# facebook/transform360

Measured on NVIDIA H100. Metric: Mpixels/s 8K equirect->cubemap bicubic (input-plane pixels consumed per second), higher is better.
Workload: dtype u8

## Files before the change

### include/transform360_b200.h

```cpp
#ifndef TRANSFORM360_B200_EXT_H
#define TRANSFORM360_B200_EXT_H

#include "Transform360/VideoFrameTransformHandler.h"

#ifdef __cplusplus
extern "C" {
#endif

typedef struct T360HostPlan T360HostPlan;

T360HostPlan* T360B200_hostPlanCreate(const FrameTransformContext* ctx, int inputWidth, int inputHeight,
                                      int outputWidth, int outputHeight);
void T360B200_hostPlanDestroy(T360HostPlan* plan);
int T360B200_hostPlanInfo(const T360HostPlan* plan, int info[6]);
const float* T360B200_hostPlanMap(const T360HostPlan* plan);
const int32_t* T360B200_hostPlanSamples(const T360HostPlan* plan);
int T360B200_hostPlanGather(T360HostPlan* plan, int info[10], const int32_t** jobs, const int32_t** records,
                            const uint32_t** compact);
int T360B200_dealLanes(int interpolationAlg, int n, const int32_t* phases, int32_t* laneOf, int32_t* copyOf);
int T360B200_weightImage(int interpolationAlg, const uint8_t** image);
int T360B200_hostPlanSegment(const T360HostPlan* plan, int i, int rect[4], int numTaps[2], const float** kx,
                             const float** ky);
int T360B200_remapTable(int interpolationAlg, const int16_t** table);

int T360B200_transformFramePlaneAsync(VideoFrameTransform* transform, const uint8_t* deviceInput,
                                      uint8_t* deviceOutput, int inputWidth, int inputHeight, int inputPitch,
                                      int outputWidth, int outputHeight, int outputPitch,
                                      int transformMatPlaneIndex, void* cudaStream);
int T360B200_transformFrameAsync(VideoFrameTransform* transform, int numPlanes, const uint8_t* const* deviceInputs,
                                 uint8_t* const* deviceOutputs, const int* inputWidths, const int* inputHeights,
                                 const int* inputPitches, const int* outputWidths, const int* outputHeights,
                                 const int* outputPitches, void* cudaStream);
int T360B200_lowPassPlaneAsync(VideoFrameTransform* transform, const uint8_t* deviceInput, uint8_t* deviceOutput,
                               int width, int height, int inputPitch, int outputPitch,
                               int transformMatPlaneIndex, void* cudaStream);
void T360B200_setPinHostPlanes(VideoFrameTransform* transform, int enable);
void T360B200_debugTrace(VideoFrameTransform* transform, int enable);
unsigned long long T360B200_debugTraceRead(VideoFrameTransform* transform, unsigned long long* out, unsigned long long maxWords);
int T360B200_synchronize(VideoFrameTransform* transform);
void* T360B200_stream(VideoFrameTransform* transform);

unsigned long long T360B200_kernelLaunchCount(void);
unsigned long long T360B200_planDeviceBytes(VideoFrameTransform* transform, int transformMatPlaneIndex);
int T360B200_planTileCounts(VideoFrameTransform* transform, int transformMatPlaneIndex, int counts[4]);
int T360B200_deviceCount(void);
const char* T360B200_version(void);

#ifdef __cplusplus
}
#endif
#endif
```

### profiles/trace_frame.py

```python
#!/usr/bin/env python
import sys
from pathlib import Path

import numpy as np
import torch

sys.path.insert(0, str(Path(__file__).resolve().parents[1]))
import transform360_b200 as t360
from bench import CONFIGS
from transform360_b200 import synth
from transform360_b200.stream import FrameTransformer, StreamSpec

KINDS = {0: "class0", 1: "class1", 2: "general", 3: "share-stay", 4: "share", 5: "nop", 7: "seam"}


def main():
    name = sys.argv[1] if len(sys.argv) > 1 else "cfg2"
    cfg = CONFIGS[name]
    dev = torch.device("cuda", 0)
    torch.cuda.set_device(0)
    ctx = t360.make_context(**dict(cfg["ov"], enable_low_pass_filter=0))
    spec = StreamSpec(cfg["inp"][0], cfg["inp"][1], cfg["out"][0], cfg["out"][1])
    ft = FrameTransformer(ctx, spec)
    pitch = lambda w: (w + 255) // 256 * 256
    ring = 5
    d_in = [[synth.noise_plane_torch(*spec.plane_dims(p)[:2], plane=p, frame=f, device=dev, pitch=pitch(spec.plane_dims(p)[0])) for p in range(3)]
            for f in range(ring)]
    d_out = [torch.zeros((spec.plane_dims(p)[3], pitch(spec.plane_dims(p)[2])), dtype=torch.uint8, device=dev) for p in range(3)]
    calls = [ft.frame_call([(t.data_ptr(), t.stride(0)) for t in fr], [(t.data_ptr(), t.stride(0)) for t in d_out]) for fr in d_in]
    stream = torch.cuda.Stream(device=dev)
    torch.cuda.synchronize()
    for i in range(6):
        calls[i % ring](stream.cuda_stream)
    torch.cuda.synchronize()
    ft.vft.debug_trace(True)
    calls[1](stream.cuda_stream)
    torch.cuda.synchronize()
    tr = ft.vft.read_trace().astype(np.int64)
    ft.vft.debug_trace(False)
    if len(sys.argv) > 2:
        np.save(sys.argv[2], tr)
    used = tr[..., 2] > 0
    t_start = tr[..., 0][used].min()
    end = np.where(used, tr[..., 2], 0).max(axis=1) - t_start
    begin = np.where(used, tr[..., 0], 1 << 62).min(axis=1) - t_start
    print(f"groups {tr.shape[0]}, jobs traced {int(used.sum())}, frame {end.max() / 1e3:.1f} us; groups finish at "
          f"min {end.min() / 1e3:.1f} / median {np.median(end) / 1e3:.1f} / max {end.max() / 1e3:.1f} us, start at median {np.median(begin) / 1e3:.1f} us")
    wait, comp, kind = (tr[..., 1] - tr[..., 0])[used], (tr[..., 2] - tr[..., 1])[used], tr[..., 3][used]
    print(f"all jobs: waiting {wait.sum() / 1e3:.0f} group-us, computing {comp.sum() / 1e3:.0f} group-us "
          f"({100 * wait.sum() / (wait.sum() + comp.sum()):.0f} % waiting)")
    for k in sorted(set(kind.tolist())):
        m = kind == k
        print(f"  {KINDS.get(k, k):10s} n={int(m.sum()):5d}  wait mean {wait[m].mean():7.0f} ns (p90 {np.percentile(wait[m], 90):6.0f})  "
              f"compute mean {comp[m].mean():7.0f} ns (p10 {np.percentile(comp[m], 10):6.0f} p90 {np.percentile(comp[m], 90):6.0f})")
    first = tr[:, 0, :]
    print(f"first job of a group: wait {np.mean(first[:, 1] - first[:, 0]) / 1e3:.2f} us")


if __name__ == "__main__":
    main()
```

### transform360_b200/csrc/gather_frame.cu

```cuda
#include "gather_common.cuh"

#include <cuda.h>

#include <algorithm>
#include <cstring>
#include <utility>

namespace t360 {

namespace {

template <class F, int... I>
__device__ __forceinline__ void staticForImpl(F&& f, std::integer_sequence<int, I...>) {
  (f(std::integral_constant<int, I>{}), ...);
}
template <int N, class F>
__device__ __forceinline__ void staticFor(F&& f) {
  staticForImpl(f, std::make_integer_sequence<int, N>{});
}

template <int IMM>
__device__ __forceinline__ uint32_t ldsWordImm(uint32_t addr) {
  uint32_t v;
  asm volatile("ld.shared.u32 %0, [%1+%2];" : "=r"(v) : "r"(addr), "n"(IMM));
  return v;
}
template <int IMM>
__device__ __forceinline__ uint4 ldsVecImm(uint32_t addr) {
  uint4 v;
  asm volatile("ld.shared.v4.u32 {%0, %1, %2, %3}, [%4+%5];" : "=r"(v.x), "=r"(v.y), "=r"(v.z), "=r"(v.w) : "r"(addr), "n"(IMM));
  return v;
}
template <int IMM>
__device__ __forceinline__ uint2 ldsVec2Imm(uint32_t addr) {
  uint2 v;
  asm volatile("ld.shared.v2.u32 {%0, %1}, [%2+%3];" : "=r"(v.x), "=r"(v.y) : "r"(addr), "n"(IMM));
  return v;
}

__device__ __forceinline__ uint32_t smemAddr(const void* p) { return (uint32_t)__cvta_generic_to_shared(p); }

__device__ __forceinline__ void mbarInit(uint64_t* bar, uint32_t arrivals) {
  asm volatile("mbarrier.init.shared::cta.b64 [%0], %1;" ::"r"(smemAddr(bar)), "r"(arrivals));
}
__device__ __forceinline__ void mbarExpectTx(uint64_t* bar, uint32_t bytes) {
  asm volatile("mbarrier.arrive.expect_tx.shared::cta.b64 _, [%0], %1;" ::"r"(smemAddr(bar)), "r"(bytes) : "memory");
}
__device__ __forceinline__ void mbarWait(uint64_t* bar, uint32_t parity) {
  asm volatile(
      "{\n\t.reg .pred p;\n\t"
      "WAIT_%=:\n\t"
      "mbarrier.try_wait.parity.shared::cta.b64 p, [%0], %1;\n\t"
      "@p bra DONE_%=;\n\t"
      "bra WAIT_%=;\n\t"
      "DONE_%=:\n\t}"
      ::"r"(smemAddr(bar)), "r"(parity) : "memory");
}
__device__ __forceinline__ void tmaLoadBox(void* dst, const CUtensorMap* map, int x, int y, uint64_t* bar) {
  asm volatile(
      "cp.async.bulk.tensor.2d.shared::cluster.global.mbarrier::complete_tx::bytes [%0], [%1, {%2, %3}], [%4];"
      ::"r"(smemAddr(dst)), "l"(reinterpret_cast<uint64_t>(map)), "r"(x), "r"(y), "r"(smemAddr(bar)) : "memory");
}
__device__ __forceinline__ void bulkCopyToShared(void* dst, const void* src, uint32_t bytes, uint64_t* bar) {
  asm volatile("cp.async.bulk.shared::cluster.global.mbarrier::complete_tx::bytes [%0], [%1], %2, [%3];"
               ::"r"(smemAddr(dst)), "l"(src), "r"(bytes), "r"(smemAddr(bar)) : "memory");
}
__device__ __forceinline__ void groupBarrier(int group) {
  asm volatile("bar.sync %0, %1;" ::"r"(group + 1), "n"(kGroupThreads) : "memory");
}

template <int K>
struct RowBytes {
  uint32_t b[K == 8 ? 2 : 1];
};

template <int K, int IMM>
__device__ __forceinline__ RowBytes<K> loadRow(uint32_t addr, int sh) {
  RowBytes<K> o;
  const uint32_t q0 = ldsWordImm<IMM>(addr), q1 = ldsWordImm<IMM + 4>(addr);
  o.b[0] = __funnelshift_r(q0, q1, sh);
  if constexpr (K == 8) o.b[1] = __funnelshift_r(q1, ldsWordImm<IMM + 8>(addr), sh);
  return o;
}

template <int K, int VS>
__device__ __forceinline__ int foldRows(const RowBytes<K> (&W)[K], uint32_t slotAddr) {
  int acc = 1 << 14;
  if constexpr (K == 2) {
    const uint2 w = ldsVec2Imm<0>(slotAddr);
    acc = dp2aLo(w.x, W[0].b[0], acc);
    acc = dp2aLo(w.y, W[1].b[0], acc);
  } else if constexpr (K == 4) {
    const uint4 wa = ldsVecImm<0>(slotAddr), wb = ldsVecImm<VS>(slotAddr);
    acc = dp2aLo(wa.x, W[0].b[0], acc); acc = dp2aHi(wa.y, W[0].b[0], acc);
    acc = dp2aLo(wa.z, W[1].b[0], acc); acc = dp2aHi(wa.w, W[1].b[0], acc);
    acc = dp2aLo(wb.x, W[2].b[0], acc); acc = dp2aHi(wb.y, W[2].b[0], acc);
    acc = dp2aLo(wb.z, W[3].b[0], acc); acc = dp2aHi(wb.w, W[3].b[0], acc);
  } else {
    staticFor<8>([&](auto R) {
      constexpr int r = decltype(R)::value;
      const uint4 wt = ldsVecImm<r * VS>(slotAddr);
      acc = dp2aLo(wt.x, W[r].b[0], acc); acc = dp2aHi(wt.y, W[r].b[0], acc);
      acc = dp2aLo(wt.z, W[r].b[1], acc); acc = dp2aHi(wt.w, W[r].b[1], acc);
    });
  }
  return acc;
}
template <int K>
__device__ __forceinline__ uint32_t slotOffset(uint32_t field) { return K == 2 ? field >> 1 : field; }

template <int VS>
__device__ __forceinline__ int foldRowsRotated(const RowBytes<8> (&W)[8], uint32_t wAddr, uint32_t field) {
  static_assert(VS == 16384, "one copy of the table");
  const uint32_t r = ((field >> 4) ^ threadIdx.x) & 7u;
  const uint32_t first = field ^ (r * (uint32_t)kDiagonalStep);
  const bool p0 = (r & 1u) != 0, p1 = (r & 2u) != 0, p2 = (r & 4u) != 0;
  RowBytes<8> A[8], B[8];
#pragma unroll
  for (int i = 0; i < 8; ++i)
#pragma unroll
    for (int h = 0; h < 2; ++h) A[i].b[h] = p0 ? W[i ^ 1].b[h] : W[i].b[h];
#pragma unroll
  for (int i = 0; i < 8; ++i)
#pragma unroll
    for (int h = 0; h < 2; ++h) B[i].b[h] = p1 ? A[i ^ 2].b[h] : A[i].b[h];
  int acc = 1 << 14;
  staticFor<8>([&](auto V) {
    constexpr int v = decltype(V)::value;
    const uint4 wt = ldsVecImm<0>(wAddr + (first ^ (uint32_t)(v * kDiagonalStep)));
    const uint32_t b0 = p2 ? B[v ^ 4].b[0] : B[v].b[0], b1 = p2 ? B[v ^ 4].b[1] : B[v].b[1];
    acc = dp2aLo(wt.x, b0, acc); acc = dp2aHi(wt.y, b0, acc);
    acc = dp2aLo(wt.z, b1, acc); acc = dp2aHi(wt.w, b1, acc);
  });
  return acc;
}
template <int K, int VS>
__device__ __forceinline__ int foldPixel(const RowBytes<K> (&W)[K], uint32_t wAddr, uint32_t field) {
  if constexpr (K == 8) return foldRowsRotated<VS>(W, wAddr, field);
  else return foldRows<K, VS>(W, wAddr + slotOffset<K>(field));
}
__device__ __forceinline__ int biasedToByte(int acc) { return min(max(acc >> 15, 0), 255); }


__device__ __forceinline__ uint32_t packBytes(int hi, int lo) {
  uint32_t r;
  asm("cvt.pack.sat.u8.s32.b32 %0, %1, %2, %3;" : "=r"(r) : "r"(hi), "r"(lo), "r"(0));
  return r;
}

template <int K, int PITCH, int VS, int ROWS, bool ZERO>
__device__ __forceinline__ void computeShareJob(uint8_t* dst, int dstPitch, uint32_t stageAddr, const uint4 (&rec)[ROWS / 8],
                                                uint32_t header, uint32_t wAddr) {
  static_assert(PITCH % 4 == 0 && (K == 4 || K == 8) && ROWS % 8 == 0, "");
  uint32_t base = stageAddr + (header & 0x7ffcu);
  const int sh = (int)(header << 3);
  RowBytes<K> W[K];
  staticFor<K>([&](auto R) { W[decltype(R)::value] = loadRow<K, decltype(R)::value * PITCH>(base, sh); });
  int accPrev = 0;
  staticFor<ROWS>([&](auto J) {
    constexpr int j = decltype(J)::value;
    const uint4& block = rec[j >> 3];
    const uint32_t word = ((j >> 1) & 3) == 0 ? block.x : (((j >> 1) & 3) == 1 ? block.y : (((j >> 1) & 3) == 2 ? block.z : block.w));
    const uint32_t r = (j & 1) ? word >> 16 : word;
    if constexpr (j > 0 && !ZERO) {
      const bool two = (r & 1u) != 0;
      const RowBytes<K> below = loadRow<K, (j - 1 + K) * PITCH>(base, sh);
      RowBytes<K> below2 = below;
      if (two) below2 = loadRow<K, (j + K) * PITCH>(base, sh);
#pragma unroll
      for (int q = 0; q + 2 < K; ++q)
#pragma unroll
        for (int i = 0; i < (K == 8 ? 2 : 1); ++i) W[q].b[i] = two ? W[q + 2].b[i] : W[q + 1].b[i];
#pragma unroll
      for (int i = 0; i < (K == 8 ? 2 : 1); ++i) W[K - 2].b[i] = two ? below.b[i] : W[K - 1].b[i];
      W[K - 1] = below2;
      if (two) base += PITCH;
    }
    if constexpr (j > 0 && ZERO) {
      const uint32_t d = r & 3u;
      RowBytes<K> below = W[K - 1], below2 = W[K - 1];
      if (d != 0) below = loadRow<K, K * PITCH>(base, sh);
      if (d == 2) below2 = loadRow<K, (K + 1) * PITCH>(base, sh);
#pragma unroll
      for (int q = 0; q + 2 < K; ++q)
#pragma unroll
        for (int i = 0; i < (K == 8 ? 2 : 1); ++i) W[q].b[i] = d == 0 ? W[q].b[i] : (d == 1 ? W[q + 1].b[i] : W[q + 2].b[i]);
#pragma unroll
      for (int i = 0; i < (K == 8 ? 2 : 1); ++i) {
        W[K - 2].b[i] = d == 0 ? W[K - 2].b[i] : (d == 1 ? W[K - 1].b[i] : below.b[i]);
        W[K - 1].b[i] = d == 0 ? W[K - 1].b[i] : (d == 1 ? below.b[i] : below2.b[i]);
      }
      base += d * PITCH;
    }
    const int acc = foldPixel<K, VS>(W, wAddr, r & kSlotFieldMask) >> 15;
    if constexpr (j & 1) {
      const uint32_t pair = packBytes(acc, accPrev);
      dst[(size_t)(j - 1) * dstPitch] = (uint8_t)pair;
      dst[(size_t)j * dstPitch] = (uint8_t)(pair >> 8);
    } else {
      accPrev = acc;
    }
  });
}

template <int K, int PITCH, int VS>
__device__ __forceinline__ void computeTileJob(const PlaneView& pv, uint32_t stageAddr, int outX, int outY, const uint4& rec,
                                               uint32_t wAddr, int warp) {
  static_assert(PITCH % 4 == 0, "");
  const int y0 = outY + warp * kTilePatchH;
  const int dstPitch = pv.dstPitch, dstW = pv.dstW, dstH = pv.dstH;
  uint8_t* const dstRow = pv.dst + (size_t)y0 * dstPitch + outX;
  const uint32_t words[4] = {rec.x, rec.y, rec.z, rec.w};
  staticFor<kRowsPerPatchStep>([&](auto J) {
    constexpr int j = decltype(J)::value;
    const uint32_t w = words[j];
    const int col = kTilePatchW * j + ((int)(w >> 16) & (kTilePatchW - 1)), row = (int)(w >> 19) & (kTilePatchH - 1);
    if (!(w & kRecordSkip) && outX + col < dstW && y0 + row < dstH) {
      const uint32_t rowAddr = stageAddr + (w & 0x7ffcu);
      const int sh = (int)(w << 3);
      RowBytes<K> W[K];
      staticFor<K>([&](auto R) { W[decltype(R)::value] = loadRow<K, decltype(R)::value * PITCH>(rowAddr, sh); });
      const int acc = foldPixel<K, VS>(W, wAddr, (w >> 17) & kSlotFieldMask);
      dstRow[(size_t)row * dstPitch + col] = (uint8_t)biasedToByte(acc);
    }
  });
}

template <int K, int VS>
__device__ __forceinline__ void computeGeneralJob(const PlaneView& pv, int outX, int outY, const unsigned char* wsmem, uint32_t wAddr,
                                                  int lane, int warp) {
  SrcView sv;
  sv.bytes = pv.src;
  sv.misalign = (int)(reinterpret_cast<uintptr_t>(pv.src) & 3);
  sv.words = reinterpret_cast<const uint32_t*>(pv.src - sv.misalign);
  sv.w = pv.srcW; sv.h = pv.srcH; sv.pitch = pv.srcPitch;
  const int y0 = outY + warp * kRowsPerThread;
  if (outX + lane >= pv.dstW) return;
  const int2* segment = pv.samples + ((size_t)(y0 / gatherTileH(K)) * pv.tilesPerRow + outX / kGatherTileW) * gatherTileH(K) * kGatherTileW +
                        (y0 % gatherTileH(K)) * kGatherTileW + lane;
  int2 full[kRowsPerThread];
#pragma unroll
  for (int j = 0; j < kRowsPerThread; ++j) full[j] = y0 + j < pv.dstH ? loadPlan(segment + j * kGatherTileW) : make_int2(0, 0);
  constexpr int kBatch = K == 8 ? 2 : 4;
#pragma unroll
  for (int jb = 0; jb < kRowsPerThread; jb += kBatch) {
    RowBytes<K> W[kBatch][K];
    bool interior[kBatch];
#pragma unroll
    for (int b = 0; b < kBatch; ++b) {
      const int col0 = recordCol0(full[jb + b].x), row0 = full[jb + b].y >> 10;
      interior[b] = y0 + jb + b < pv.dstH && col0 >= 0 && row0 >= 0 && col0 + (K == 2 ? 8 : K + 4) <= sv.w && row0 + K <= sv.h;
#pragma unroll
      for (int r = 0; r < K; ++r) {
        W[b][r].b[0] = 0;
        if constexpr (K == 8) W[b][r].b[1] = 0;
        if (interior[b]) {
          const int off = (row0 + r) * sv.pitch + col0 + sv.misalign;
          const uint32_t* q = sv.words + (off >> 2);
          const int sh = (off & 3) * 8;
          const uint32_t q0 = __ldg(q), q1 = __ldg(q + 1);
          W[b][r].b[0] = __funnelshift_r(q0, q1, sh);
          if constexpr (K == 8) W[b][r].b[1] = __funnelshift_r(q1, __ldg(q + 2), sh);
        }
      }
    }
#pragma unroll
    for (int b = 0; b < kBatch; ++b) {
      const int j = jb + b;
      if (y0 + j >= pv.dstH) continue;
      int v;
      if (interior[b]) v = biasedToByte(foldPixel<K, VS>(W[b], wAddr, (uint32_t)weightSlotOf(K, full[j].y & 1023) << 4));
      else v = gatherPixel<K, false, VS, weightDiagonal(K)>(sv, wsmem, recordCol0(full[j].x), full[j].y);
      pv.dst[(size_t)(y0 + j) * pv.dstPitch + outX + recordColumn(full[j].x)] = (uint8_t)v;
    }
  }
}

struct FrameTensorMaps {
  CUtensorMap map[kMaxFramePlanes][kNumBoxClasses][kBoxVariants];
};

__device__ __forceinline__ void mbarArrive(uint64_t* bar) {
  asm volatile("mbarrier.arrive.shared::cta.b64 _, [%0];" ::"r"(smemAddr(bar)) : "memory");
}
__device__ __forceinline__ uint4 ldsVec(uint32_t addr) {
  uint4 v;
  asm volatile("ld.shared.v4.u32 {%0, %1, %2, %3}, [%4];" : "=r"(v.x), "=r"(v.y), "=r"(v.z), "=r"(v.w) : "r"(addr));
  return v;
}
__device__ __forceinline__ uint32_t ldsWord(uint32_t addr) {
  uint32_t v;
  asm volatile("ld.shared.u32 %0, [%1];" : "=r"(v) : "r"(addr));
  return v;
}

template <int K, int COPIES, int GROUPS>
struct FrameLayout {
  static constexpr int kStages = gatherStages(K);
  static constexpr int kWeights = weightImageBytes(K, COPIES);
  static constexpr int kStage = stageBytesOf(K), kRec = stageRecordBytes(K);
  static constexpr int kGroupBytes = kStages * (kStage + kRec);
  static constexpr int kPlanes = kWeights + GROUPS * kGroupBytes;
  static constexpr int kBars = kPlanes + 256;
  static constexpr int kTotal = kBars + GROUPS * kStages * 16 + 16;
  static_assert(kTotal <= 232448, "227 KB of shared memory per CTA");
  static_assert(sizeof(PlaneView) * kMaxFramePlanes <= 256, "");
  static_assert(kStage % 128 == 0 && kRec % 128 == 0 && kWeights % 128 == 0, "TMA / bulk-copy destinations");
};

template <int K, int COPIES, int GROUPS>
__global__ void __launch_bounds__(GROUPS * (kGroupWarps + 1) * 32, 1)
gatherFrameKernel(const __grid_constant__ FrameGatherParams p, StagedParams jobs, const __grid_constant__ FrameTensorMaps maps) {
  using L = FrameLayout<K, COPIES, GROUPS>;
  constexpr int VS = weightVectorStride(K, COPIES), kStage = L::kStage, kRec = L::kRec, S = L::kStages;
  constexpr uint32_t kBox0 = stageBoxW(K, 0) * stageBoxH(K, 0), kBox1 = stageBoxW(K, 1) * stageBoxH(K, 1),
                     kBoxShare = stageBoxW(K, 2) * stageBoxH(K, 2);
  static_assert(kBox1 + 64 <= 2 * kStage && kBox0 + 64 <= kStage && kBoxShare + 64 <= kStage, "boxes must fit their stage buffers");
  static_assert(boxVariantRows(K, 0, kBoxVariants - 1) > 0 && boxVariantRows(K, 2, kBoxVariants - 1) > 0, "");
  extern __shared__ __align__(128) unsigned char smem[];
  unsigned char* wsmem = smem;
  PlaneView* planes = reinterpret_cast<PlaneView*>(smem + L::kPlanes);
  uint64_t* barBase = reinterpret_cast<uint64_t*>(smem + L::kBars);
  uint64_t* weightBar = barBase + GROUPS * 2 * S;
  const int warpId = threadIdx.x >> 5, lane = threadIdx.x & 31;
  constexpr int kProducerWarp = GROUPS * kGroupWarps;

  asm volatile("griddepcontrol.launch_dependents;" ::: "memory");
  if (threadIdx.x == 0) {
    for (int g = 0; g < GROUPS; ++g)
      for (int st = 0; st < S; ++st) {
        mbarInit(barBase + g * 2 * S + st, 1);
        mbarInit(barBase + g * 2 * S + S + st, kGroupWarps);
      }
    mbarInit(weightBar, 1);
    asm volatile("fence.mbarrier_init.release.cluster;" ::: "memory");
  }
  if (threadIdx.x < kMaxFramePlanes * (int)(sizeof(PlaneView) / 4))
    reinterpret_cast<uint32_t*>(planes)[threadIdx.x] = reinterpret_cast<const uint32_t*>(p.plane)[threadIdx.x];
  __syncthreads();

  if (warpId >= kProducerWarp) {
    const int g = warpId - kProducerWarp;
    if (g == 0 && lane == 0) {
      mbarExpectTx(weightBar, L::kWeights);
      constexpr int kChunk = L::kWeights / 4;
      for (int i = 0; i < 4; ++i)
        bulkCopyToShared(wsmem + i * kChunk, reinterpret_cast<const unsigned char*>(p.weightImage) + i * kChunk, kChunk, weightBar);
    }
    const int producer = blockIdx.x * GROUPS + g, dynamicBase = gridDim.x * GROUPS * 2 * kClaimBatch;
    auto loadBatch = [&](int base) {
      int4 h = make_int4(0, kJobExit << kJobKindShift, 0, 0);
      if (lane < kClaimBatch && base + lane < jobs.numTiles) h = __ldg(reinterpret_cast<const int4*>(jobs.tiles) + base + lane);
      return h;
    };
    int4 batch = loadBatch(producer * 2 * kClaimBatch);
    int4 batchNext = loadBatch((producer * 2 + 1) * kClaimBatch);
    asm volatile("griddepcontrol.wait;" ::: "memory");
    int claimed = 0;
    if (lane == 0) claimed = atomicAdd(jobs.claimCounter, kClaimBatch);
    unsigned char* groupBase = smem + L::kWeights + g * L::kGroupBytes;
    uint64_t* full = barBase + g * 2 * S;
    uint64_t* empty = full + S;
    int pos = 0;
    uint32_t st = 0, phase = 0;
    auto advance = [&]() { if (++st == S) { st = 0; phase ^= 1; } };
    auto postEmptyJob = [&](int kind) {
      *reinterpret_cast<int4*>(groupBase + S * kStage + st * kRec) = make_int4(0, kind << kJobKindShift, 0, 0);
      mbarArrive(full + st);
    };
    for (;;) {
      if (pos == kClaimBatch) {
        batch = batchNext;
        pos = 0;
        batchNext = loadBatch(dynamicBase + __shfl_sync(0xffffffffu, claimed, 0));
        if (lane == 0) claimed = atomicAdd(jobs.claimCounter, kClaimBatch);
      }
      int4 h;
      h.x = __shfl_sync(0xffffffffu, batch.x, pos); h.y = __shfl_sync(0xffffffffu, batch.y, pos);
      h.z = __shfl_sync(0xffffffffu, batch.z, pos); h.w = __shfl_sync(0xffffffffu, batch.w, pos);
      ++pos;
      const int kind = (h.y >> kJobKindShift) & kJobKindMask;
      mbarWait(empty + st, phase ^ 1);
      const bool twoStages = kind == kJobClass1 || kind == kJobSeam;
      if (twoStages) {
        if (st == S - 1) {
          if (lane == 0) postEmptyJob(kJobNop);
          advance();
          mbarWait(empty + st, phase ^ 1);
        }
        mbarWait(empty + st + 1, phase ^ 1);
      }
      if (lane == 0) {
        unsigned char* rec = groupBase + S * kStage + st * kRec;
        *reinterpret_cast<int4*>(rec) = h;
        if (kind == kJobShare || kind == kJobShareStay || kind == kJobClass0 || kind == kJobClass1 || kind == kJobSeam) {
          const int pl = h.y >> kJobPlaneShift;
          const bool share = boxClassOf(kind) == 2;
          const int cls = boxClassOf(kind), variant = jobBoxVariant(h.z), boxX = jobBoxX(h.z), boxY = jobBoxY(h.z);
          const uint32_t boxBytes = (uint32_t)(stageBoxW(K, cls) * boxVariantRows(K, cls, variant));
          const uint32_t recBytes = share ? shareJobRecordBytes(K) : tileJobRecordBytes(h.x);
          mbarExpectTx(full + st, (kind == kJobSeam ? 2 : 1) * boxBytes + recBytes);
          tmaLoadBox(groupBase + st * kStage, &maps.map[pl][cls][variant], boxX, boxY, full + st);
          if (kind == kJobSeam)
            tmaLoadBox(groupBase + (st + 1) * kStage, &maps.map[pl][0][variant], boxX - planes[pl].srcW, boxY, full + st);
          bulkCopyToShared(rec + 128, planes[pl].records + (unsigned)h.w, recBytes, full + st);
        } else {
          mbarArrive(full + st);
        }
      }
      advance();
      if (twoStages) {
        if (lane == 0) postEmptyJob(kJobNop);
        advance();
      }
      __syncwarp();
      if (kind == kJobExit) break;
    }
    if (lane == 0 && atomicAdd(jobs.claimCounter + 1, 1) == (int)(gridDim.x * GROUPS) - 1) {
      jobs.claimCounter[0] = 0;
      jobs.claimCounter[1] = 0;
      __threadfence();
    }
    return;
  }

  const int group = warpId / kGroupWarps, warp = warpId % kGroupWarps;
  unsigned char* groupBase = smem + L::kWeights + group * L::kGroupBytes;
  const uint32_t boxAddr = smemAddr(groupBase), recAddr = smemAddr(groupBase + S * kStage);
  uint64_t* full = barBase + group * 2 * S;
  uint64_t* empty = full + S;
  const uint32_t wAddr = smemAddr(wsmem);
  mbarWait(weightBar, 0);
  asm volatile("griddepcontrol.wait;" ::: "memory");
  auto now = []() { unsigned long long t; asm volatile("mov.u64 %0, %globaltimer;" : "=l"(t)); return t; };
  unsigned long long* trace = jobs.trace && warp == 0 && lane == 0 ? jobs.trace + (size_t)(blockIdx.x * GROUPS + group) * kTraceJobsPerGroup * 4 : nullptr;
  uint32_t traced = 0;
  for (uint32_t st = 0, phase = 0;;) {
    const unsigned long long t0 = trace ? now() : 0;
    mbarWait(full + st, phase);
    const unsigned long long t1 = trace ? now() : 0;
    const uint32_t rec = recAddr + st * kRec;
    const uint4 h = ldsVec(rec);
    const int kind = ((int)h.y >> kJobKindShift) & kJobKindMask;
    if (kind == kJobExit) break;
    const int outX = (int)h.x & ~kJobQuadMask, outY = (int)h.y & kJobRowMask;
    const PlaneView& pv = planes[(int)h.y >> kJobPlaneShift];
    if (kind == kJobShare || kind == kJobShareStay) {
      if constexpr (K >= 4) {
        const uint32_t mine = rec + 128 + warp * shareWarpRecordBytes(K);
        uint4 r[shareRows(K) / 8];
#pragma unroll
        for (int b = 0; b < shareRows(K) / 8; ++b) r[b] = ldsVec(mine + b * 512 + lane * 16);
        const uint32_t header = ldsWord(mine + shareRows(K) / 8 * 512 + lane * 4);
        uint8_t* dst = pv.dst + (size_t)(outY + (warp >> 1) * shareRows(K)) * pv.dstPitch + (outX + (warp & 1) * 32 + (int)(header >> kRecordColumnShift));
        if (kind == kJobShare) computeShareJob<K, stageBoxW(K, 2), VS, shareRows(K), false>(dst, pv.dstPitch, boxAddr + st * kStage, r, header, wAddr);
        else computeShareJob<K, stageBoxW(K, 2), VS, shareRows(K), true>(dst, pv.dstPitch, boxAddr + st * kStage, r, header, wAddr);
      }
    } else if (kind == kJobClass0) {
      uint4 r;
      const int quad = ((int)h.x & kJobQuadMask) - 1;
      if (quad < 0) {
        r = ldsVec(rec + 128 + warp * 512 + lane * 16);
      } else {
        r = make_uint4(kRecordSkip, kRecordSkip, kRecordSkip, kRecordSkip);
        if ((warp >> 2) == (quad >> 1)) {
          const uint2 v = ldsVec2Imm<0>(rec + 128 + (warp & 3) * 256 + lane * 8);
          if (quad & 1) { r.z = v.x; r.w = v.y; } else { r.x = v.x; r.y = v.y; }
        }
      }
      computeTileJob<K, stageBoxW(K, 0), VS>(pv, boxAddr + st * kStage, outX, outY, r, wAddr, warp);
    } else if (kind == kJobClass1) {
      computeTileJob<K, stageBoxW(K, 1), VS>(pv, boxAddr + st * kStage, outX, outY, ldsVec(rec + 128 + warp * 512 + lane * 16), wAddr, warp);
    } else if (kind == kJobSeam) {
      {
        uint4* a = reinterpret_cast<uint4*>(groupBase + st * kStage);
        const uint4* b = reinterpret_cast<const uint4*>(groupBase + (st + 1) * kStage);
        for (int i = warp * 32 + lane; i < (int)(kBox0 / 16); i += kGroupThreads) {
          uint4 x = a[i];
          const uint4 y = b[i];
          x.x |= y.x; x.y |= y.y; x.z |= y.z; x.w |= y.w;
          a[i] = x;
        }
        asm volatile("fence.proxy.async.shared::cta;" ::: "memory");
      }
      groupBarrier(group);
      computeTileJob<K, stageBoxW(K, 0), VS>(pv, boxAddr + st * kStage, outX, outY, ldsVec(rec + 128 + warp * 512 + lane * 16), wAddr, warp);
    } else if (kind == kJobGeneral) {
      computeGeneralJob<K, VS>(pv, outX, outY, wsmem, wAddr, lane, warp);
    }
    __syncwarp();
    if (lane == 0) mbarArrive(empty + st);
    if (trace && traced < kTraceJobsPerGroup) {
      trace[traced * 4 + 0] = t0; trace[traced * 4 + 1] = t1; trace[traced * 4 + 2] = now(); trace[traced * 4 + 3] = kind;
      ++traced;
    }
    if (++st == S) { st = 0; phase ^= 1; }
  }
}

template <int K, int COPIES, int GROUPS>
cudaError_t prepareFrameK(LaunchCfg& cfg) {
  static DeviceLaunchCfg cfgs;
  constexpr int threads = GROUPS * (kGroupWarps + 1) * 32, smemBytes = FrameLayout<K, COPIES, GROUPS>::kTotal;
  return prepare<gatherFrameKernel<K, COPIES, GROUPS>>(cfgs, threads, smemBytes, cfg);
}

template <int K, int COPIES, int GROUPS>
cudaError_t launchFrameK(const FrameGatherParams& p, const StagedParams& jobs, const FrameTensorMaps& maps, int numSMs,
                         cudaStream_t stream, bool programmatic) {
  constexpr int threads = GROUPS * (kGroupWarps + 1) * 32, smemBytes = FrameLayout<K, COPIES, GROUPS>::kTotal;
  LaunchCfg cfg;
  cudaError_t err = prepareFrameK<K, COPIES, GROUPS>(cfg);
  if (err != cudaSuccess) return err;
  const int grid = std::min(numSMs * cfg.perSM, (jobs.numTiles + GROUPS * 2 * kClaimBatch - 1) / (GROUPS * 2 * kClaimBatch));
  cudaLaunchConfig_t lc{};
  lc.gridDim = dim3(grid);
  lc.blockDim = dim3(threads);
  lc.dynamicSmemBytes = smemBytes;
  lc.stream = stream;
  cudaLaunchAttribute attr{};
  attr.id = cudaLaunchAttributeProgrammaticStreamSerialization;
  attr.val.programmaticStreamSerializationAllowed = 1;
  lc.attrs = &attr;
  lc.numAttrs = programmatic ? 1 : 0;
  err = cudaLaunchKernelEx(&lc, gatherFrameKernel<K, COPIES, GROUPS>, p, jobs, maps);
  gLaunches.fetch_add(1, std::memory_order_relaxed);
  return err;
}

}

cudaError_t prepareGatherFrame(int kernelSize) {
  LaunchCfg cfg;
  switch (kernelSize) {
    case 2: return prepareFrameK<2, weightCopies(2), gatherGroups(2)>(cfg);
    case 4: return prepareFrameK<4, weightCopies(4), gatherGroups(4)>(cfg);
    case 8: return prepareFrameK<8, weightCopies(8), gatherGroups(8)>(cfg);
    default: return cudaErrorInvalidValue;
  }
}

cudaError_t launchGatherFrame(const FrameGatherParams& p, const StagedParams& jobs, const void* tensorMaps, int numSMs,
                              cudaStream_t stream, bool programmatic) {
  if (jobs.numTiles <= 0) return cudaSuccess;
  if (p.numPlanes < 1 || p.numPlanes > kMaxFramePlanes) return cudaErrorInvalidValue;
  FrameTensorMaps maps;
  std::memcpy(&maps, tensorMaps, sizeof(CUtensorMap) * kNumBoxClasses * kBoxVariants * p.numPlanes);
  for (int i = p.numPlanes; i < kMaxFramePlanes; ++i)
    for (int c = 0; c < kNumBoxClasses; ++c)
      for (int v = 0; v < kBoxVariants; ++v) maps.map[i][c][v] = maps.map[0][c][v];
  switch (p.kernelSize) {
    case 2: return launchFrameK<2, weightCopies(2), gatherGroups(2)>(p, jobs, maps, numSMs, stream, programmatic);
    case 4: return launchFrameK<4, weightCopies(4), gatherGroups(4)>(p, jobs, maps, numSMs, stream, programmatic);
    case 8: return launchFrameK<8, weightCopies(8), gatherGroups(8)>(p, jobs, maps, numSMs, stream, programmatic);
    default: return cudaErrorInvalidValue;
  }
}

}
```

### transform360_b200/csrc/gather_plan.cpp

```cpp
#include "gather_plan.h"

#include <algorithm>
#include <climits>
#include <cstdint>
#include <cstring>
#include <thread>

namespace t360 {
namespace {

template <class F>
void parallelRanges(int n, size_t workPerItem, F fn) {
  unsigned nt = std::thread::hardware_concurrency();
  if (nt == 0) nt = 1;
  if (nt > 32) nt = 32;
  if (static_cast<size_t>(n) * workPerItem < (1u << 16)) nt = 1;
  const int chunk = (n + static_cast<int>(nt) - 1) / static_cast<int>(nt);
  std::vector<std::thread> pool;
  for (unsigned t = 1; t < nt; ++t) {
    const int b = static_cast<int>(t) * chunk, e = std::min(n, b + chunk);
    if (b < e) pool.emplace_back(fn, b, e);
  }
  fn(0, std::min(n, chunk));
  for (auto& th : pool) th.join();
}

struct GroupMatcher {
  int n, copies, cap;
  const int* base;
  int groupOf[32], load[8];
  bool visited[8];

  bool place(int i) {
    for (int c = 0; c < copies; ++c) {
      const int g = (base[i] + c) & 7;
      if (visited[g]) continue;
      visited[g] = true;
      if (load[g] < cap) {
        ++load[g];
        groupOf[i] = g;
        return true;
      }
      for (int j = 0; j < n; ++j) {
        if (j == i || groupOf[j] != g) continue;
        groupOf[j] = -1;
        if (place(j)) {
          groupOf[i] = g;
          return true;
        }
        groupOf[j] = g;
      }
    }
    return false;
  }
  bool run() {
    std::fill(groupOf, groupOf + 32, -1);
    std::fill(load, load + 8, 0);
    for (int i = 0; i < n; ++i) {
      std::fill(visited, visited + 8, false);
      if (!place(i)) return false;
    }
    return true;
  }
  void balance() {
    for (bool improved = true; improved;) {
      improved = false;
      for (int src = 0; src < 8 && !improved; ++src) {
        int from[8], via[8], queue[8], head = 0, tail = 0;
        std::fill(from, from + 8, -1);
        from[src] = src;
        queue[tail++] = src;
        while (head < tail && !improved) {
          const int g = queue[head++];
          for (int j = 0; j < n && !improved; ++j) {
            if (groupOf[j] != g) continue;
            for (int c = 0; c < copies; ++c) {
              const int t = (base[j] + c) & 7;
              if (from[t] >= 0) continue;
              from[t] = g;
              via[t] = j;
              queue[tail++] = t;
              if (load[t] + 2 <= load[src]) {
                for (int cur = t; cur != src; cur = from[cur]) groupOf[via[cur]] = cur;
                ++load[t];
                --load[src];
                improved = true;
                break;
              }
            }
          }
        }
      }
    }
  }
};

void buildFullRecords(const HostPlan& h, std::vector<int2>& out, int tilesPerRow, int tileH) {
  const int k = h.kernelSize;
  constexpr int kRows = 4;
  parallelRanges((h.mapH + kRows - 1) / kRows, static_cast<size_t>(h.mapW) * kRows, [&](int blockBegin, int blockEnd) {
  for (int yb = blockBegin * kRows; yb < blockEnd * kRows; yb += kRows) {
    for (int x0 = 0; x0 < h.mapW; x0 += 32) {
      const int n = std::min(32, h.mapW - x0);
      int laneOf[32], copyOf[32], slot[32];
      const SamplePoint* first = &h.samples[static_cast<size_t>(yb) * h.mapW];
      for (int i = 0; i < n; ++i) slot[i] = k >= 2 ? weightSlotOf(k, first[x0 + i].rowPhase & 1023) : 0;
      if (k >= 2) dealLanes(k, 1, n, slot, laneOf, copyOf);
      else for (int i = 0; i < n; ++i) laneOf[i] = i;
      for (int y = yb; y < std::min(h.mapH, yb + kRows); ++y) {
        const SamplePoint* row = &h.samples[static_cast<size_t>(y) * h.mapW];
        const size_t tile = static_cast<size_t>(y / tileH) * tilesPerRow + x0 / 32;
        int2* dst = &out[(tile * tileH + y % tileH) * 32];
        for (int c = 0; c < n; ++c) {
          const SamplePoint& sp = row[x0 + c];
          dst[laneOf[c]] = int2{static_cast<int>((static_cast<unsigned>(sp.col0) & ((1u << kRecordColumnShift) - 1)) |
                                                 (static_cast<unsigned>(c) << kRecordColumnShift)),
                                sp.rowPhase};
        }
      }
    }
  }
  });
}

struct TileClass {
  int kind = -1;
  int boxX = 0, boxY = 0, boxRows = 0;
  bool shareStart = false;
  bool quads = false;
  int quadBoxX[4] = {}, quadBoxY[4] = {}, quadBoxRows[4] = {};
};

struct Extent {
  int minC = INT32_MAX, maxC = INT32_MIN, minR = INT32_MAX, maxR = INT32_MIN;
};
Extent extentOf(const HostPlan& h, int x0, int y0, int x1, int y1) {
  Extent e;
  for (int y = y0; y < y1; ++y) {
    const SamplePoint* row = &h.samples[static_cast<size_t>(y) * h.mapW];
    for (int x = x0; x < x1; ++x) {
      const int c = row[x].col0, r = row[x].rowPhase >> 10;
      e.minC = std::min(e.minC, c); e.maxC = std::max(e.maxC, c);
      e.minR = std::min(e.minR, r); e.maxR = std::max(e.maxR, r);
    }
  }
  return e;
}

bool shareBlock(const HostPlan& h, int x0, int y0, TileClass& out) {
  const int k = h.kernelSize, kShareH = shareH(k);
  if (k < 4 || x0 + kShareW > h.mapW || y0 + kShareH > h.mapH) return false;
  bool stays = false;
  for (int y = y0 + 1; y < y0 + kShareH; ++y) {
    const SamplePoint* a = &h.samples[static_cast<size_t>(y - 1) * h.mapW + x0];
    const SamplePoint* b = a + h.mapW;
    for (int x = 0; x < kShareW; ++x) {
      const int d = (b[x].rowPhase >> 10) - (a[x].rowPhase >> 10);
      if (b[x].col0 != a[x].col0 || d < 0 || d > 2) return false;
      stays = stays || d == 0;
    }
  }
  const Extent e = extentOf(h, x0, y0, x0 + kShareW, y0 + kShareH);
  if (e.minC < 0 || e.minR < 0 || e.maxC + k > h.inW || e.maxR + k > h.inH) return false;
  const int boxX = e.minC & ~15;
  if (e.maxC + k - boxX > stageBoxW(k, 2) || e.maxR + k - e.minR > stageBoxH(k, 2)) return false;
  out.kind = stays ? kJobShareStay : kJobShare;
  out.boxX = boxX;
  out.boxY = e.minR;
  out.boxRows = e.maxR + k - e.minR;
  out.shareStart = true;
  return true;
}

int boxClassFor(const HostPlan& h, int x0, int y0, int x1, int y1, int maxClass, int* boxX, int* boxY, int* boxRows) {
  const int k = h.kernelSize;
  const Extent e = extentOf(h, x0, y0, x1, y1);
  if (e.minC < 0 || e.minR < 0 || e.maxC + k > h.inW || e.maxR + k > h.inH) return -1;
  *boxX = e.minC & ~15;
  *boxY = e.minR;
  *boxRows = e.maxR + k - e.minR;
  for (int cls = 0; cls <= maxClass; ++cls)
    if (e.maxC + k - *boxX <= stageBoxW(k, cls) && e.maxR + k - e.minR <= stageBoxH(k, cls)) return cls;
  return -1;
}

void classifyTile(const HostPlan& h, int x0, int y0, bool seamPossible, TileClass& out) {
  const int k = h.kernelSize;
  const int x1 = std::min(h.mapW, x0 + kGatherTileW), y1 = std::min(h.mapH, y0 + kFrameTileH);
  const int cls = boxClassFor(h, x0, y0, x1, y1, 1, &out.boxX, &out.boxY, &out.boxRows);
  if (cls == 0) {
    out.kind = kJobClass0;
    return;
  }
  if (x1 - x0 == kGatherTileW && y1 - y0 == kFrameTileH) {
    bool all = true;
    for (int q = 0; q < 4 && all; ++q) {
      const int qx = x0 + 16 * (q & 1), qy = y0 + 16 * (q >> 1);
      all = boxClassFor(h, qx, qy, qx + 16, qy + 16, 0, &out.quadBoxX[q], &out.quadBoxY[q], &out.quadBoxRows[q]) == 0;
    }
    if (all) {
      out.kind = kJobClass0;
      out.quads = true;
      return;
    }
  }
  if (cls == 1) {
    out.kind = kJobClass1;
    return;
  }
  const Extent e = extentOf(h, x0, y0, x1, y1);
  if (seamPossible && e.minR >= 0 && e.maxR + k <= h.inH && e.maxR + k - e.minR <= stageBoxH(k, 0)) {
    const int W = h.inW, half = W / 2;
    int lo = INT32_MAX, hi = INT32_MIN;
    for (int y = y0; y < y1; ++y)
      for (int x = x0; x < x1; ++x) {
        int cw = h.samples[static_cast<size_t>(y) * h.mapW + x].col0 % W;
        if (cw < 0) cw += W;
        const int rot = cw + half >= W ? cw + half - W : cw + half;
        lo = std::min(lo, rot); hi = std::max(hi, rot);
      }
    const int first = lo - half < 0 ? lo - half + W : lo - half;
    const int bx = first & ~15;
    if (hi - lo + (first - bx) + k <= stageBoxW(k, 0) && bx + stageBoxW(k, 0) > W) {
      out.kind = kJobSeam;
      out.boxX = bx;
      out.boxY = e.minR;
      out.boxRows = e.maxR + k - e.minR;
      return;
    }
  }
  out.kind = kJobGeneral;
  out.boxX = out.boxY = out.boxRows = 0;
}

inline uint32_t slotField(int k, int phase, int copy) { return static_cast<uint32_t>(weightSlotField(k, phase, copy)); }

void writeShareRecords(const HostPlan& h, const GatherJob& job, uint32_t* out) {
  const int k = h.kernelSize, copies = weightCopies(k), kShareRows = shareRows(k), kShareH = shareH(k);
  const int x0 = job.outX, y0 = job.outY & kJobRowMask, boxX = jobBoxX(job.boxXY), boxY = jobBoxY(job.boxXY);
  const int pitch = stageBoxW(k, 2);
  const bool stay = ((job.outY >> kJobKindShift) & kJobKindMask) == kJobShareStay;
  for (int wx = 0; wx < kShareW / 32; ++wx) {
    for (int wy = 0; wy < kShareH / kShareRows; ++wy) {
      int slot[32], laneOf[32], copyOf[32];
      const SamplePoint* first = &h.samples[static_cast<size_t>(y0 + wy * kShareRows) * h.mapW + x0 + wx * 32];
      for (int i = 0; i < 32; ++i) slot[i] = weightSlotOf(k, first[i].rowPhase & 1023);
      dealLanes(k, copies, 32, slot, laneOf, copyOf);
      const int w = wy * (kShareW / 32) + wx;
      uint32_t* words = out + static_cast<size_t>(w) * (shareWarpRecordBytes(k) / 4);
      uint32_t* headers = words + kShareRows / 8 * 32 * 4;
      for (int c = 0; c < 32; ++c) {
        const int lane = laneOf[c], x = x0 + wx * 32 + c, ya = y0 + wy * kShareRows;
        const SamplePoint* col = &h.samples[static_cast<size_t>(ya) * h.mapW + x];
        const int off = ((col->rowPhase >> 10) - boxY) * pitch + (col->col0 - boxX);
        headers[lane] = static_cast<uint32_t>(off) | (static_cast<uint32_t>(c) << kRecordColumnShift);
        for (int j = 0; j < kShareRows; ++j) {
          const SamplePoint& sp = col[static_cast<size_t>(j) * h.mapW];
          const int first = stay ? 0 : 1;
          const int d = j == 0 ? first : (sp.rowPhase >> 10) - (col[static_cast<size_t>(j - 1) * h.mapW].rowPhase >> 10);
          const uint32_t rec = slotField(k, sp.rowPhase & 1023, copyOf[c]) | static_cast<uint32_t>(d - first);
          uint32_t& word = words[(j >> 3) * 32 * 4 + lane * 4 + ((j >> 1) & 3)];
          word = (j & 1) ? (word | (rec << 16)) : rec;
        }
      }
    }
  }
}

void writeTileRecords(const HostPlan& h, const GatherJob& job, uint32_t* out) {
  const int k = h.kernelSize, copies = weightCopies(k);
  const int kind = (job.outY >> kJobKindShift) & kJobKindMask;
  const int x0 = job.outX & ~kJobQuadMask, y0 = job.outY & kJobRowMask, boxX = jobBoxX(job.boxXY), boxY = jobBoxY(job.boxXY);
  const int pitch = stageBoxW(k, boxClassOf(kind));
  const int quad = (job.outX & kJobQuadMask) - 1;
  const int lx0 = quad < 0 ? x0 : x0 + 16 * (quad & 1), ly0 = quad < 0 ? y0 : y0 + 16 * (quad >> 1);
  const int lx1 = quad < 0 ? x0 + kGatherTileW : lx0 + 16, ly1 = quad < 0 ? y0 + kFrameTileH : ly0 + 16;
  for (int w = 0; w < kGroupWarps; ++w)
    for (int j = 0; j < kRowsPerPatchStep; ++j) {
      if (quad >= 0 && ((w >> 2) != (quad >> 1) || (j >> 1) != (quad & 1))) continue;
      uint32_t* words = quad < 0 ? out + static_cast<size_t>(w) * 32 * 4 : out + static_cast<size_t>(w & 3) * 32 * 2;
      const int stride = quad < 0 ? 4 : 2, word = quad < 0 ? j : (j & 1);
      int slot[32], laneOf[32], copyOf[32], posOf[32], n = 0;
      bool present[32] = {};
      for (int pos = 0; pos < 32; ++pos) {
        const int x = x0 + kTilePatchW * j + (pos & (kTilePatchW - 1)), y = y0 + kTilePatchH * w + pos / kTilePatchW;
        if (x >= h.mapW || y >= h.mapH || x < lx0 || x >= lx1 || y < ly0 || y >= ly1) continue;
        present[pos] = true;
        posOf[n] = pos;
        slot[n++] = weightSlotOf(k, h.samples[static_cast<size_t>(y) * h.mapW + x].rowPhase & 1023);
      }
      dealLanes(k, copies, n, slot, laneOf, copyOf);
      int lane = n;
      for (int pos = 0; pos < 32; ++pos)
        if (!present[pos]) words[(lane++) * stride + word] = (static_cast<uint32_t>(pos) << 16) | kRecordSkip;
      for (int i = 0; i < n; ++i) {
        const int pos = posOf[i];
        const int x = x0 + kTilePatchW * j + (pos & (kTilePatchW - 1)), y = y0 + kTilePatchH * w + pos / kTilePatchW;
        const SamplePoint& sp = h.samples[static_cast<size_t>(y) * h.mapW + x];
        int col0 = sp.col0;
        if (kind == kJobSeam) {
          int cw = col0 % h.inW;
          if (cw < 0) cw += h.inW;
          col0 = boxX + (cw - boxX + h.inW) % h.inW;
        }
        const int off = ((sp.rowPhase >> 10) - boxY) * pitch + (col0 - boxX);
        words[laneOf[i] * stride + word] = static_cast<uint32_t>(off) | (static_cast<uint32_t>(pos) << 16) |
                                           (slotField(k, sp.rowPhase & 1023, copyOf[i]) << 17);
      }
    }
}

}

struct PassDealer {
  int groups, passes, lanes;
  int h[4], share[16][4], fill[4];
  bool seen[4];

  bool put(int g) {
    for (int q = 0; q < passes; ++q) {
      if (seen[q] || share[g][q] >= h[q]) continue;
      seen[q] = true;
      if (fill[q] < lanes) {
        ++share[g][q];
        ++fill[q];
        return true;
      }
      for (int other = 0; other < groups; ++other) {
        if (other == g || share[other][q] == 0) continue;
        --share[other][q];
        if (put(other)) {
          ++share[g][q];
          return true;
        }
        ++share[other][q];
      }
    }
    return false;
  }
  bool deal(const int* load) {
    std::memset(share, 0, sizeof(share));
    std::fill(fill, fill + 4, 0);
    for (int g = 0; g < groups; ++g)
      for (int i = 0; i < load[g]; ++i) {
        std::fill(seen, seen + 4, false);
        if (!put(g)) return false;
      }
    return true;
  }
};

int dealLanes(int k, int copies, int n, const int* slot, int* laneOf, int* copyOf) {
  const int groups = weightBankGroups(k), lanesPerPass = weightLanesPerPass(k), passes = 32 / lanesPerPass;
  for (int i = 0; i < n; ++i) { laneOf[i] = i; copyOf[i] = 0; }
  if (n < 32) return 0;
  int group[32];
  if (copies > 1 && groups == 8) {
    int base[32];
    for (int i = 0; i < n; ++i) base[i] = slot[i] & 7;
    GroupMatcher m{n, copies, 0, base, {}, {}, {}};
    for (m.cap = 4; m.cap <= 32; ++m.cap)
      if (m.run()) break;
    m.balance();
    for (int i = 0; i < n; ++i) {
      group[i] = m.groupOf[i];
      copyOf[i] = (m.groupOf[i] - base[i]) & 7;
    }
  } else {
    for (int i = 0; i < n; ++i) group[i] = slot[i] & (groups - 1);
  }
  int load[16] = {};
  for (int i = 0; i < n; ++i) ++load[group[i]];
  int share[16][4] = {}, height[4] = {};
  {
    int fullest = 0;
    for (int g = 0; g < groups; ++g) fullest = std::max(fullest, load[g]);
    PassDealer d{groups, passes, lanesPerPass, {}, {}, {}, {}};
    bool done = false;
    for (int total = std::max(passes, fullest); !done; ++total) {
      int h[4] = {1, 1, 1, 1};
      auto tryHeights = [&]() {
        std::copy(h, h + 4, d.h);
        if (!d.deal(load)) return false;
        std::memcpy(share, d.share, sizeof(share));
        std::copy(h, h + 4, height);
        return true;
      };
      if (passes == 2) {
        for (h[1] = total / 2; h[1] >= 1 && !done; --h[1]) { h[0] = total - h[1]; done = tryHeights(); }
      } else {
        for (h[3] = total / 4; h[3] >= 1 && !done; --h[3])
          for (h[2] = (total - h[3]) / 3; h[2] >= h[3] && !done; --h[2])
            for (h[1] = (total - h[3] - h[2]) / 2; h[1] >= h[2] && !done; --h[1]) {
              h[0] = total - h[3] - h[2] - h[1];
              done = tryHeights();
            }
      }
    }
  }
  int nextLane[4];
  for (int q = 0; q < passes; ++q) nextLane[q] = q * lanesPerPass;
  for (int g = 0; g < groups; ++g) {
    int q = 0;
    for (int i = 0; i < n; ++i) {
      if (group[i] != g) continue;
      while (share[g][q] == 0) ++q;
      --share[g][q];
      laneOf[i] = nextLane[q]++;
    }
  }
  int wavefronts = 0;
  for (int q = 0; q < passes; ++q) wavefronts += height[q];
  return wavefronts;
}

void spreadGeneralJobs(std::vector<GatherJob>& jobs) {
  std::vector<GatherJob> general, staged;
  for (const GatherJob& j : jobs)
    (((j.outY >> kJobKindShift) & kJobKindMask) == kJobGeneral ? general : staged).push_back(j);
  if (general.empty() || staged.empty()) return;
  const size_t span = staged.size() / 2 + 1;
  jobs.clear();
  size_t g = 0;
  for (size_t i = 0; i < staged.size(); ++i) {
    while (g < general.size() && g * span / general.size() <= i) jobs.push_back(general[g++]);
    jobs.push_back(staged[i]);
  }
  while (g < general.size()) jobs.push_back(general[g++]);
}

std::vector<uint8_t> buildWeightImage(int k, const int16_t* table) {
  const int copies = weightCopies(k);
  std::vector<uint8_t> img(static_cast<size_t>(weightImageBytes(k, copies)), 0);
  for (int phase = 0; phase < 1024; ++phase) {
    const int slot = weightSlotOf(k, phase);
    const int16_t* cell = table + static_cast<size_t>(phase) * k * k;
    if (k == 2) {
      std::memcpy(&img[static_cast<size_t>(slot) * 8], cell, 8);
      continue;
    }
    for (int c = 0; c < copies; ++c)
      for (int v = 0; v < k * k / 8; ++v)
        std::memcpy(&img[static_cast<size_t>(weightVectorOffset(k, copies, (weightSlotInCopy(slot, c) << 4) | (c << 14), v))], cell + v * 8, 16);
  }
  return img;
}

void buildGatherPlan(const HostPlan& h, bool stageTiles, GatherPlan& g) {
  g = GatherPlan{};
  const int k = h.kernelSize;
  if (k <= 0) return;
  g.tileH = gatherTileH(k);
  g.tilesPerRow = (h.mapW + kGatherTileW - 1) / kGatherTileW;
  g.tileRows = (h.mapH + g.tileH - 1) / g.tileH;
  g.records.assign(static_cast<size_t>(g.tilesPerRow) * g.tileRows * g.tileH * kGatherTileW, int2{0, 0});
  buildFullRecords(h, g.records, g.tilesPerRow, g.tileH);
  if (!stageTiles) return;

  const int tilesX = g.tilesPerRow, tilesY = (h.mapH + kFrameTileH - 1) / kFrameTileH;
  const bool seamPossible = h.inW % 16 == 0 && h.inW >= 4 * stageBoxW(k, 0);
  std::vector<TileClass> cls(static_cast<size_t>(tilesX) * tilesY);
  const int blockRows = shareH(k) / kFrameTileH;
  parallelRanges((tilesY + blockRows - 1) / blockRows, static_cast<size_t>(h.mapW) * shareH(k), [&](int byBegin, int byEnd) {
    for (int by = byBegin; by < byEnd; ++by)
      for (int tx = 0; tx < tilesX; tx += 2) {
        TileClass* c = &cls[static_cast<size_t>(by) * blockRows * tilesX + tx];
        if (shareBlock(h, tx * 32, by * shareH(k), c[0])) continue;
        for (int ty = by * blockRows; ty < std::min(tilesY, (by + 1) * blockRows); ++ty)
          for (int t = tx; t < std::min(tilesX, tx + 2); ++t)
            classifyTile(h, t * 32, ty * kFrameTileH, seamPossible, cls[static_cast<size_t>(ty) * tilesX + t]);
      }
  });
  const int order[7] = {kJobGeneral, kJobSeam, kJobClass1, kJobShareStay, kJobShare, kJobClass0, kJobClass0};
  size_t offset = 0;
  for (int step = 0; step < 7; ++step)
    for (int ty = 0; ty < tilesY; ++ty)
      for (int tx = 0; tx < tilesX; ++tx) {
        const int kind = order[step];
        const TileClass& c = cls[static_cast<size_t>(ty) * tilesX + tx];
        if (c.kind != kind || (kind == kJobClass0 && c.quads != (step == 6))) continue;
        for (int q = 0; q < (c.quads ? 4 : 1); ++q) {
          GatherJob job{tx * 32, ty * kFrameTileH | (kind << kJobKindShift),
                        kind == kJobGeneral ? 0 : jobBoxField(c.boxX, c.boxY, boxVariantFor(k, boxClassOf(kind), c.boxRows)), 0};
          if (c.quads) {
            job.outX |= q + 1;
            job.boxXY = jobBoxField(c.quadBoxX[q], c.quadBoxY[q], boxVariantFor(k, 0, c.quadBoxRows[q]));
          }
          if (kind != kJobGeneral) {
            job.recordOffset = static_cast<int>(offset / 16);
            offset += boxClassOf(kind) == 2 ? shareJobRecordBytes(k) : tileJobRecordBytes(job.outX);
          }
          g.jobs.push_back(job);
        }
        switch (kind) {
          case kJobGeneral: ++g.numGeneral; break;
          case kJobSeam: ++g.numSeam; break;
          case kJobShare: case kJobShareStay: ++g.numShare; break;
          default: g.numStaged[kind] += c.quads ? 4 : 1; break;
        }
      }
  g.compact.assign(offset / 4, 0u);
  g.jobNeedRows.assign(g.jobs.size(), h.inH);
  parallelRanges(static_cast<int>(g.jobs.size()), 2048, [&](int begin, int end) {
    for (int i = begin; i < end; ++i) {
      const GatherJob& job = g.jobs[i];
      {
        int rect[4];
        jobOutputRect(job, k, rect);
        const Extent e = extentOf(h, rect[0], rect[1], std::min(rect[2], h.mapW), std::min(rect[3], h.mapH));
        if (e.minR >= 0 && e.maxR + k <= h.inH) g.jobNeedRows[i] = e.maxR + k;
      }
      const int kind = (job.outY >> kJobKindShift) & kJobKindMask;
      if (kind == kJobGeneral) continue;
      uint32_t* out = g.compact.data() + static_cast<size_t>(job.recordOffset) * 4;
      if (boxClassOf(kind) == 2) writeShareRecords(h, job, out);
      else writeTileRecords(h, job, out);
    }
  });
}

}
```

### transform360_b200/csrc/gather_plan.h

```cpp
#pragma once

#include <cstdint>
#include <vector>

#include "host_plan.h"
#include "kernels.cuh"

namespace t360 {

struct GatherPlan {
  int tilesPerRow = 0, tileRows = 0, tileH = 0;
  std::vector<int2> records;
  std::vector<GatherJob> jobs;
  std::vector<uint32_t> compact;
  std::vector<int> jobNeedRows;
  int numStaged[2] = {}, numSeam = 0, numGeneral = 0, numShare = 0;
  int totalStaged() const { return numSeam + numShare + numStaged[0] + numStaged[1]; }
};

void buildGatherPlan(const HostPlan& h, bool stageTiles, GatherPlan& g);

inline void jobOutputRect(const GatherJob& job, int k, int rect[4]) {
  const int kind = (job.outY >> kJobKindShift) & kJobKindMask, quad = (job.outX & kJobQuadMask) - 1;
  rect[0] = job.outX & ~kJobQuadMask;
  rect[1] = job.outY & kJobRowMask;
  if (quad >= 0) { rect[0] += 16 * (quad & 1); rect[1] += 16 * (quad >> 1); }
  const bool share = kind == kJobShare || kind == kJobShareStay;
  rect[2] = rect[0] + (quad >= 0 ? 16 : (share ? kShareW : kGatherTileW));
  rect[3] = rect[1] + (quad >= 0 ? 16 : (share ? shareH(k) : kFrameTileH));
}

void spreadGeneralJobs(std::vector<GatherJob>& jobs);


int dealLanes(int k, int copies, int n, const int* slot, int* laneOf, int* copyOf);

std::vector<uint8_t> buildWeightImage(int k, const int16_t* table);

}
```

### transform360_b200/csrc/kernels.cuh

```cuda
#pragma once

#include <cuda_runtime.h>

#include <cstdint>

namespace t360 {

struct GatherParams {
  const uint8_t* src;
  int srcW, srcH, srcPitch;
  uint8_t* dst;
  int dstW, dstH, dstPitch;
  const int2* samples;
  int tilesPerRow;
  const int16_t* weights;
  int kernelSize;
  int transparent;
};

struct GatherJob {
  int outX, outY;
  int boxXY;
  int recordOffset;
};
constexpr int kBoxVariants = 3;
__host__ __device__ constexpr int jobBoxField(int boxX, int boxY, int variant) { return boxX | (boxY << 16) | variant; }
__host__ __device__ constexpr int jobBoxX(int boxXY) { return boxXY & 0xfff0; }
__host__ __device__ constexpr int jobBoxY(int boxXY) { return (int)((unsigned)boxXY >> 16); }
__host__ __device__ constexpr int jobBoxVariant(int boxXY) { return boxXY & 15; }
using StagedTile = GatherJob;
constexpr int kJobClass0 = 0, kJobClass1 = 1, kJobGeneral = 2, kJobShareStay = 3, kJobShare = 4, kJobNop = 5, kJobExit = 6, kJobSeam = 7;
constexpr int kJobQuadMask = 7;
constexpr uint32_t kRecordSkip = 0x8000u;
constexpr int kJobKindShift = 24, kJobRowMask = (1 << kJobKindShift) - 1;
constexpr int kJobPlaneShift = 28, kJobKindMask = (1 << (kJobPlaneShift - kJobKindShift)) - 1;

constexpr int kGroupThreads = 256, kGroupWarps = kGroupThreads / 32;
__host__ __device__ constexpr int gatherGroups(int k) { return k == 8 ? 2 : 3; }
#ifndef T360_CLAIM_BATCH
#define T360_CLAIM_BATCH 1
#endif
constexpr int kClaimBatch = T360_CLAIM_BATCH;
constexpr int kGatherTileW = 32, kFrameTileH = 32;
constexpr int kTilePatchW = 8, kTilePatchH = 4, kRowsPerPatchStep = 4;
constexpr int kShareW = 64;
__host__ __device__ constexpr int shareRows(int ) { return 8; }
__host__ __device__ constexpr int shareH(int k) { return 4 * shareRows(k); }
constexpr int kNumBoxClasses = 3;
__host__ __device__ constexpr int boxClassOf(int kind) { return (kind == kJobShare || kind == kJobShareStay) ? 2 : (kind == kJobClass1 ? 1 : 0); }
__host__ __device__ constexpr int stageBoxW(int , int cls) { return cls == 2 ? 192 : (cls == 0 ? 208 : 240); }
__host__ __device__ constexpr int stageBoxH(int k, int cls) {
  return k == 8 ? (cls == 2 ? 80 : (cls == 0 ? 72 : 128)) : (cls == 2 ? 72 : (cls == 0 ? 64 : 96));
}
__host__ __device__ constexpr int boxVariantRows(int k, int cls, int v) {
  return cls == 1 || v == 0 ? stageBoxH(k, cls) : (cls == 2 ? stageBoxH(k, cls) - 8 * v : stageBoxH(k, cls) - 8 - 8 * v);
}
__host__ __device__ constexpr int boxVariantFor(int k, int cls, int rows) {
  int v = 0;
  while (v + 1 < kBoxVariants && cls != 1 && boxVariantRows(k, cls, v + 1) >= rows) ++v;
  return v;
}
__host__ __device__ constexpr int gatherStages(int ) { return 2; }
__host__ __device__ constexpr int stageBytesOf(int k) {
  const int a = stageBoxW(k, 2) * stageBoxH(k, 2), b = stageBoxW(k, 0) * stageBoxH(k, 0);
  return ((a > b ? a : b) + 64 + 127) & ~127;
}

__host__ __device__ constexpr int weightSlotOf(int k, int phase) {
  (void)k;
  return (phase & ~31) | ((phase & 1) << 4) | ((phase & 31) >> 1);
}
__host__ __device__ constexpr int weightCopies(int k) { return k == 4 ? 2 : 1; }
__host__ __device__ constexpr int weightVectorStride(int k, int copies) { return (k == 2 ? 8192 : 16384) * copies; }
__host__ __device__ constexpr int weightImageBytes(int k, int copies) { return k == 2 ? 8192 * copies : (k * k / 8) * 16384 * copies; }
__host__ __device__ constexpr int weightSlotInCopy(int slot, int copy) { return copy ? ((slot & ~7) | ((slot + copy) & 7)) : slot; }
__host__ __device__ constexpr int weightSlotField(int k, int phase, int copy) {
  return (weightSlotInCopy(weightSlotOf(k, phase), copy) << 4) | (copy << 14);
}
constexpr int kSlotFieldMask = 0x7FF0;
constexpr int kDiagonalStep = 0x4010;
__host__ __device__ constexpr bool weightDiagonal(int k) { return k == 8; }
__host__ __device__ constexpr int weightVectorOffset(int k, int copies, int slotFieldValue, int vector) {
  return weightDiagonal(k) ? (slotFieldValue ^ (vector * kDiagonalStep)) : slotFieldValue + vector * weightVectorStride(k, copies);
}
__host__ __device__ constexpr int weightBankGroups(int k) { return k == 2 ? 16 : 8; }
__host__ __device__ constexpr int weightLanesPerPass(int k) { return k == 2 ? 16 : 8; }

__host__ __device__ constexpr int shareWarpRecordBytes(int k) { return shareRows(k) / 8 * 32 * 16 + 32 * 4; }
__host__ __device__ constexpr int shareJobRecordBytes(int k) { return kGroupWarps * shareWarpRecordBytes(k); }
constexpr int kTileJobRecordBytes = kGroupWarps * 32 * 16;
constexpr int kQuadJobRecordBytes = kGroupWarps / 2 * 32 * 8;
__host__ __device__ constexpr int tileJobRecordBytes(int outXField) { return (outXField & kJobQuadMask) ? kQuadJobRecordBytes : kTileJobRecordBytes; }
__host__ __device__ constexpr int stageRecordBytes(int k) {
  return 128 + (shareJobRecordBytes(k) > kTileJobRecordBytes ? shareJobRecordBytes(k) : kTileJobRecordBytes);
}
constexpr int kRecordColumnShift = 27;

constexpr int kMaxFramePlanes = 3;
struct PlaneView {
  const uint8_t* src;
  uint8_t* dst;
  const int2* samples;
  const uint4* records;
  int srcW, srcH, srcPitch;
  int dstW, dstH, dstPitch;
  int tilesPerRow;
  int reserved;
};
struct FrameGatherParams {
  PlaneView plane[kMaxFramePlanes];
  const uint4* weightImage;
  int kernelSize, numPlanes;
};

__host__ __device__ constexpr int gatherThreads(int k) { return k == 8 ? 512 : 256; }
__host__ __device__ constexpr int gatherTileH(int k) { return gatherThreads(k) / 32 * 4; }

struct StagedParams {
  const GatherJob* tiles;
  int numTiles;
  int* claimCounter;
  unsigned long long* trace;
};
constexpr int kTraceJobsPerGroup = 64;

struct BlurJob {
  int x0, y0, w, h;
  int kxOffset, kxCount, kyOffset, kyCount;
};

struct BlurParams {
  const uint8_t* src;
  uint8_t* dst;
  int width, height, srcPitch, dstPitch;
  const BlurJob* jobs;
  int numJobs;
  const float* taps;
  int tileSmemBytes;
};

struct StripJob {
  int x0, y0, w, h;
  int kxOffset, kxChunks, kxCount, kyOffset;
  int edge;
};

struct StripParams {
  const uint8_t* src;
  uint8_t* dst;
  int width, height, srcPitch, dstPitch;
  const StripJob* jobs;
  int numJobs;
  const float* taps;
};

struct AreaParams {
  const uint8_t* src;
  uint8_t* dst;
  int srcW, srcH, srcPitch, dstW, dstH, dstPitch;
  int cellW, cellH;
  const int2* xTaps;
  const int* xFirst;
  const int2* yTaps;
  const int* yFirst;
  const int2* xLinear;
  const int2* yLinear;
  int xMax;
};
cudaError_t launchAreaResize(const AreaParams& p, cudaStream_t stream);

struct FrameStripParams {
  struct Plane {
    const uint8_t* src;
    uint8_t* dst;
    int width, height, srcPitch, dstPitch;
  } plane[kMaxFramePlanes];
  const StripJob* jobs;
  int numJobs;
  const float* taps;
};
constexpr int kStripPlaneShift = 8;
cudaError_t launchBlurFrameStrips(const FrameStripParams& p, int hy, cudaStream_t stream);

constexpr int kStripLanePx = 8, kStripW = 32 * kStripLanePx, kStripMaxHy = 3;

constexpr int kBlurTileW = 64, kBlurTileH = 32;
constexpr int kBlurMaxSmem = 96 * 1024;

cudaError_t launchGather(const GatherParams& p, int numSMs, cudaStream_t stream);
cudaError_t launchGatherFrame(const FrameGatherParams& p, const StagedParams& jobs, const void* tensorMaps, int numSMs,
                              cudaStream_t stream, bool programmatic = true);
cudaError_t prepareGatherFrame(int kernelSize);
cudaError_t launchBlurStrips(const StripParams& p, int hy, cudaStream_t stream);
cudaError_t launchBlur(const BlurParams& p, cudaStream_t stream);
cudaError_t launchBlurDirect(const BlurParams& p, cudaStream_t stream);
unsigned long long kernelLaunchCount();
void countKernelLaunches(long long n);

inline int blurTileSmem(int w, int h, int nkx, int nky) {
  const int hx = nkx / 2, hy = nky / 2;
  const int rows = h + 2 * hy;
  const int srcStride = (w + 2 * hx + 3) & ~3;
  return rows * srcStride + rows * w * 4;
}

}
```

### transform360_b200/csrc/video_frame_transform.cpp

```cpp
#include <cuda.h>
#include <cuda_runtime.h>

#include <algorithm>
#include <climits>
#include <cstdio>
#include <cstdlib>
#include <cstring>
#include <map>
#include <memory>
#include <mutex>
#include <new>
#include <stdexcept>
#include <vector>

#include "host_plan.h"
#include "gather_plan.h"
#include "kernels.cuh"
#include "transform360_b200.h"

#define T360_API extern "C" __attribute__((visibility("default")))

namespace {

using t360::BlurJob;
using t360::GatherJob;
using t360::HostPlan;
using t360::StripJob;

struct CudaFail {
  cudaError_t err;
  const char* what;
};

#define CU(call)                                       \
  do {                                                 \
    cudaError_t e__ = (call);                          \
    if (e__ != cudaSuccess) throw CudaFail{e__, #call}; \
  } while (0)

template <typename T>
struct DeviceBuffer {
  T* ptr = nullptr;
  size_t count = 0;
  DeviceBuffer() = default;
  DeviceBuffer(const DeviceBuffer&) = delete;
  DeviceBuffer& operator=(const DeviceBuffer&) = delete;
  DeviceBuffer(DeviceBuffer&& o) noexcept : ptr(o.ptr), count(o.count) { o.ptr = nullptr; o.count = 0; }
  DeviceBuffer& operator=(DeviceBuffer&& o) noexcept {
    if (this != &o) { release(); ptr = o.ptr; count = o.count; o.ptr = nullptr; o.count = 0; }
    return *this;
  }
  ~DeviceBuffer() { release(); }
  void release() {
    if (ptr) cudaFree(ptr);
    ptr = nullptr;
    count = 0;
  }
  void reserve(size_t n) {
    if (n <= count) return;
    release();
    CU(cudaMalloc(reinterpret_cast<void**>(&ptr), n * sizeof(T)));
    count = n;
  }
  size_t bytes() const { return count * sizeof(T); }
};

struct DevicePlan {
  int inW = 0, inH = 0, outW = 0, outH = 0, mapW = 0, mapH = 0;
  int kernelSize = 0;
  bool transparent = false, lowPass = false;
  DeviceBuffer<int2> samples;
  DeviceBuffer<uint32_t> records;
  int tilesPerRow = 0;
  DeviceBuffer<GatherJob> gatherJobs;
  std::vector<GatherJob> hostJobs;
  std::vector<int> jobNeedRows;
  int numJobs = 0, numStaged[2] = {}, numSeam = 0, numShare = 0, numFallback = 0;
  int totalStaged() const { return numSeam + numShare + numStaged[0] + numStaged[1]; }
  struct BlurSet {
    DeviceBuffer<StripJob> stripJobs[t360::kStripMaxHy];
    int numStripJobs[t360::kStripMaxHy] = {};
    DeviceBuffer<BlurJob> tileJobs, directJobs;
    int numTileJobs = 0, numDirectJobs = 0, tileSmem = 0;
    DeviceBuffer<float> taps;
    bool needsClear = false;
    std::vector<StripJob> hostStrips[t360::kStripMaxHy];
    std::vector<float> hostTaps;
  };
  BlurSet blur;
  std::vector<t360::LowPassSegment> segments;
  std::vector<float> planTaps;
  mutable std::map<std::pair<int, int>, BlurSet> otherBlurs;
  struct Resize {
    int cellW = 0, cellH = 0, xMax = 0;
    DeviceBuffer<int2> xTaps, yTaps, xLinear, yLinear;
    DeviceBuffer<int> xFirst, yFirst;
  };
  bool resizeNeeded = false;
  mutable std::map<std::pair<int, int>, Resize> resizes;
  size_t deviceBytes() const {
    return samples.bytes() + records.bytes() + gatherJobs.bytes() + blur.stripJobs[0].bytes() + blur.stripJobs[1].bytes() + blur.stripJobs[2].bytes() +
           blur.tileJobs.bytes() + blur.directJobs.bytes() + blur.taps.bytes();
  }
};

using EncodeTiledFn = CUresult (*)(CUtensorMap*, CUtensorMapDataType, cuuint32_t, void*, const cuuint64_t*, const cuuint64_t*,
                                   const cuuint32_t*, const cuuint32_t*, CUtensorMapInterleave, CUtensorMapSwizzle,
                                   CUtensorMapL2promotion, CUtensorMapFloatOOBfill);

EncodeTiledFn tensorMapEncoder() {
  static EncodeTiledFn fn = [] {
    void* p = nullptr;
    cudaDriverEntryPointQueryResult q{};
    if (cudaGetDriverEntryPoint("cuTensorMapEncodeTiled", &p, cudaEnableDefault, &q) != cudaSuccess || q != cudaDriverEntryPointSuccess) {
      cudaGetLastError();
      p = nullptr;
    }
    return reinterpret_cast<EncodeTiledFn>(p);
  }();
  return fn;
}

bool encodePlaneMap(CUtensorMap* map, const uint8_t* base, int w, int h, int pitch, int k, int cls, int variant) {
  EncodeTiledFn enc = tensorMapEncoder();
  if (!enc) return false;
  if ((reinterpret_cast<uintptr_t>(base) & 15) || (pitch & 15)) return false;
  const cuuint64_t dims[2] = {static_cast<cuuint64_t>(w), static_cast<cuuint64_t>(h)};
  const cuuint64_t strides[1] = {static_cast<cuuint64_t>(pitch)};
  const cuuint32_t box[2] = {static_cast<cuuint32_t>(t360::stageBoxW(k, cls)), static_cast<cuuint32_t>(t360::boxVariantRows(k, cls, variant))};
  const cuuint32_t elem[2] = {1, 1};
  return enc(map, CU_TENSOR_MAP_DATA_TYPE_UINT8, 2, const_cast<uint8_t*>(base), dims, strides, box, elem,
             CU_TENSOR_MAP_INTERLEAVE_NONE, CU_TENSOR_MAP_SWIZZLE_NONE, CU_TENSOR_MAP_L2_PROMOTION_L2_128B,
             CU_TENSOR_MAP_FLOAT_OOB_FILL_NONE) == CUDA_SUCCESS;
}

constexpr int kPlaneLanes = 3;
static_assert(kPlaneLanes == t360::kMaxFramePlanes, "the frame kernel takes one PlaneView per lane");
struct PlaneMaps {
  const uint8_t* base = nullptr;
  int w = 0, h = 0, pitch = 0, k = 0;
  CUtensorMap maps[t360::kNumBoxClasses][t360::kBoxVariants];
};
struct PlaneLane {
  static constexpr int kMapCache = 32;
  PlaneMaps mapCache[kMapCache];
  int mapCacheNext = 0;
  cudaStream_t main = nullptr;
  cudaEvent_t done = nullptr;
  DeviceBuffer<uint8_t> blurred;
  DeviceBuffer<uint8_t> scaled;
  DeviceBuffer<int> claimCounter;
};

struct GatherWork {
  const DevicePlan* plan = nullptr;
  t360::PlaneView view{};
  bool staged = false;
  CUtensorMap maps[t360::kNumBoxClasses][t360::kBoxVariants];
  uint8_t* finalOut = nullptr;
  int finalPitch = 0, finalW = 0, finalH = 0, imagePlane = 0;
  const void* resizeTables = nullptr;
};

struct FrameJobList {
  DeviceBuffer<GatherJob> tiles;
  int numTiles = 0, numPlanes = 0;
  unsigned long long generation = ~0ull;
  DeviceBuffer<int> claimCounter;
};

struct WavePlan {
  struct Rect { int x, y, w, h; };
  int chunks = 0;
  const void* plan = nullptr;
  unsigned long long generation = ~0ull;
  std::vector<int> chunkRowEnd, waveStart;
  DeviceBuffer<GatherJob> jobs;
  std::vector<std::vector<Rect>> rects;
};

struct StreamSlot {
  PlaneLane lanes[kPlaneLanes];
  DeviceBuffer<int> frameClaim;
  cudaEvent_t fork = nullptr;
};

struct FrameBlurList {
  DeviceBuffer<StripJob> jobs[t360::kStripMaxHy];
  int numJobs[t360::kStripMaxHy] = {};
  DeviceBuffer<float> taps;
  int numPlanes = 0;
  unsigned long long generation = ~0ull;
};

constexpr int kPitchAlign = 256;
inline int alignedPitch(int w) { return (w + kPitchAlign - 1) / kPitchAlign * kPitchAlign; }

}

class VideoFrameTransform {
 public:
  explicit VideoFrameTransform(FrameTransformContext* ctx) {
    std::memcpy(&ctx_, ctx, sizeof(ctx_));
    const char* e = std::getenv("T360B200_PIN_HOST_PLANES");
    pinHostPlanes_ = e && *e && *e != '0';
    if (const char* m = std::getenv("T360B200_PIPELINE_MIN_BYTES")) pipelineMinBytes_ = std::atoll(m);
    if (const char* m = std::getenv("T360B200_PIPELINE_CHUNKS")) pipelineChunks_ = std::atoi(m);
    if (const char* m = std::getenv("T360B200_PIPELINE_BLOCKS")) pipelineBlocks_ = std::atoi(m);
    if (const char* m = std::getenv("T360B200_PIPELINE_IN_STREAMS")) pipelineInStreams_ = std::atoi(m);
  }
  void setPinHostPlanes(bool on) { pinHostPlanes_ = on; }

  ~VideoFrameTransform() {
    if (deviceReady_) {
      cudaSetDevice(device_);
      plans_.clear();
      for (auto& w : weights_) w.release();
      for (auto& w : weightImages_) w.release();
      stagingIn_.release(); stagingOut_.release();
      for (HostRange& r : hostRanges_)
        if (r.pinned) cudaHostUnregister(reinterpret_cast<void*>(r.base));
      for (auto& kv : slots_) {
        for (PlaneLane& l : kv.second->lanes) {
          l.blurred.release();
          l.scaled.release();
          l.claimCounter.release();
          if (l.main) cudaStreamDestroy(l.main);
          if (l.done) cudaEventDestroy(l.done);
        }
        kv.second->frameClaim.release();
        if (kv.second->fork) cudaEventDestroy(kv.second->fork);
      }
      frameJobs_.tiles.release();
      for (auto& b : frameBlur_.jobs) b.release();
      frameBlur_.taps.release();
      trace_.release();
      frameJobs_.claimCounter.release();
      for (cudaEvent_t e : chunkIn_) cudaEventDestroy(e);
      for (cudaEvent_t e : waveDone_) cudaEventDestroy(e);
      for (WavePlan& w : wavePlans_) w.jobs.release();
      for (PlaneGraph& g : planeGraphs_) cudaGraphExecDestroy(g.exec);
      for (cudaEvent_t e : {graphFork_, graphJoinIn_, graphJoinOut_}) if (e) cudaEventDestroy(e);
      if (copyIn_) cudaStreamDestroy(copyIn_);
      if (copyIn2_) cudaStreamDestroy(copyIn2_);
      if (copyOut_) cudaStreamDestroy(copyOut_);
      if (stream_) cudaStreamDestroy(stream_);
    }
  }

  bool generateMapForPlane(int inW, int inH, int outW, int outH, int planIndex) {
    try {
      HostPlan host;
      if (!t360::buildHostPlan(ctx_, inW, inH, outW, outH, host)) return false;
      const DeviceRestore restoreDevice = ensureDevice();
      std::lock_guard<std::mutex> lock(mu_);
      plans_[planIndex] = upload(host);
      ++planGeneration_;
      return true;
    } catch (const CudaFail& f) {
      std::printf("Could not generate map for plane %d. Error: CUDA %s (%s) in %s\n", planIndex,
                  cudaGetErrorName(f.err), cudaGetErrorString(f.err), f.what);
    } catch (const std::exception& ex) {
      std::printf("Could not generate map for plane %d. Error: %s\n", planIndex, ex.what());
    }
    return false;
  }

  bool transformFramePlane(uint8_t* in, uint8_t* out, int inW, int inH, int inPitch, int outW, int outH, int outPitch,
                           int planIndex, int imagePlaneIndex) {
    try {
      if (!in || !out || inW <= 0 || inH <= 0 || outW <= 0 || outH <= 0 || inPitch < inW || outPitch < outW) {
        std::printf("Could not transform the plane %d. Error: invalid plane description\n", imagePlaneIndex);
        return false;
      }
      const DeviceRestore restoreDevice = ensureDevice();
      const DevicePlan* plan = findPlan(planIndex, imagePlaneIndex);
      if (!plan) return false;
      {
        std::lock_guard<std::mutex> hostLock(hostCallMu_);
        if (replayPlaneGraph(*plan, in, out, inW, inH, inPitch, outW, outH, outPitch)) return true;
      }
      const bool inOnDevice = isDevicePointer(in), outOnDevice = isDevicePointer(out);
      if (plan->kernelSize == 0) {
        std::printf("Could not find interpolation algorithm for plane %d", imagePlaneIndex);
        return true;
      }
      std::lock_guard<std::mutex> hostLock(hostCallMu_);
      if (!inOnDevice && !outOnDevice && pipelineEligible(*plan, inW, inH, outW, outH))
        return transformHostPlanePipelined(*plan, in, out, inW, inH, inPitch, outW, outH, outPitch, planIndex, imagePlaneIndex);
      const uint8_t* dIn = in;
      uint8_t* dOut = out;
      int dInPitch = inPitch, dOutPitch = outPitch;
      if (!inOnDevice) {
        pinIfRecurring(in, static_cast<size_t>(inPitch) * (inH - 1) + inW);
        dInPitch = alignedPitch(inW);
        stagingIn_.reserve(static_cast<size_t>(dInPitch) * inH + 64);
        CU(cudaMemcpy2DAsync(stagingIn_.ptr, dInPitch, in, inPitch, inW, inH, cudaMemcpyHostToDevice, stream_));
        dIn = stagingIn_.ptr;
      }
      if (!outOnDevice) {
        pinIfRecurring(out, static_cast<size_t>(outPitch) * (outH - 1) + outW);
        dOutPitch = alignedPitch(outW);
        stagingOut_.reserve(static_cast<size_t>(dOutPitch) * outH + 64);
        dOut = stagingOut_.ptr;
        if (plan->transparent) {
          if (planIndex) CU(cudaMemset2DAsync(dOut, dOutPitch, 128, outW, outH, stream_));
          else CU(cudaMemcpy2DAsync(dOut, dOutPitch, out, outPitch, outW, outH, cudaMemcpyHostToDevice, stream_));
        }
      } else if (plan->transparent && planIndex) {
        CU(cudaMemset2DAsync(dOut, dOutPitch, 128, outW, outH, stream_));
      }
      if (!enqueue(*plan, dIn, dOut, inW, inH, dInPitch, outW, outH, dOutPitch, stream_, imagePlaneIndex, slotFor(stream_).lanes[0])) return false;
      if (!outOnDevice)
        CU(cudaMemcpy2DAsync(out, outPitch, dOut, dOutPitch, outW, outH, cudaMemcpyDeviceToHost, stream_));
      CU(cudaStreamSynchronize(stream_));
      return true;
    } catch (const CudaFail& f) {
      std::printf("Could not transform the plane %d. Error: CUDA %s (%s) in %s\n", imagePlaneIndex,
                  cudaGetErrorName(f.err), cudaGetErrorString(f.err), f.what);
      cudaGetLastError();
    } catch (const std::exception& ex) {
      std::printf("Could not transform the plane %d. Error: %s\n", imagePlaneIndex, ex.what());
    }
    return false;
  }

  bool pipelineEligible(const DevicePlan& plan, int inW, int inH, int outW, int outH) const {
    return plan.totalStaged() > 0 && !plan.transparent && !plan.lowPass && inW == plan.inW && inH == plan.inH &&
           outW == plan.mapW && outH == plan.mapH && static_cast<long long>(inW) * inH >= pipelineMinBytes_ && inH >= 64;
  }

  WavePlan& wavePlanFor(const DevicePlan& plan, int planIndex, int chunks) {
    WavePlan& w = wavePlans_[planIndex ? 1 : 0];
    if (w.plan == &plan && w.chunks == chunks && w.generation == planGeneration_) return w;
    w.chunks = chunks;
    w.plan = &plan;
    w.generation = planGeneration_;
    const int rowsPer = ((plan.inH + chunks - 1) / chunks + 7) & ~7;
    w.chunkRowEnd.assign(chunks, plan.inH);
    for (int c = 0; c < chunks; ++c) w.chunkRowEnd[c] = std::min(plan.inH, (c + 1) * rowsPer);
    auto waveOf = [&](int needRows) {
      int c = 0;
      while (c + 1 < chunks && w.chunkRowEnd[c] < needRows) ++c;
      return c;
    };
    std::vector<std::vector<GatherJob>> byWave(chunks);
    int blocks = 1;
    for (int nb : {4, 3, 2})
      if (plan.mapW % (nb * t360::kShareW) == 0 && nb <= pipelineBlocks_) { blocks = nb; break; }
    const int blockW = plan.mapW / blocks, bands = (plan.mapH + 31) / 32;
    std::vector<int> complete(static_cast<size_t>(bands) * blocks, 0);
    for (size_t i = 0; i < plan.hostJobs.size(); ++i) {
      const int c = waveOf(plan.jobNeedRows[i]);
      byWave[c].push_back(plan.hostJobs[i]);
      int rect[4];
      t360::jobOutputRect(plan.hostJobs[i], plan.kernelSize, rect);
      for (int band = rect[1] / 32; band <= (std::min(rect[3], plan.mapH) - 1) / 32; ++band) {
        int& slot = complete[static_cast<size_t>(band) * blocks + rect[0] / blockW];
        slot = std::max(slot, c);
      }
    }
    std::vector<GatherJob> all;
    w.waveStart.assign(chunks + 1, 0);
    for (int c = 0; c < chunks; ++c) {
      t360::spreadGeneralJobs(byWave[c]);
      w.waveStart[c] = static_cast<int>(all.size());
      all.insert(all.end(), byWave[c].begin(), byWave[c].end());
    }
    w.waveStart[chunks] = static_cast<int>(all.size());
    w.jobs.reserve(all.size());
    CU(cudaMemcpy(w.jobs.ptr, all.data(), all.size() * sizeof(GatherJob), cudaMemcpyHostToDevice));
    w.rects.assign(chunks, {});
    for (int b = 0; b < blocks; ++b)
      for (int band = 0; band < bands;) {
        const int c = complete[static_cast<size_t>(band) * blocks + b];
        int end = band + 1;
        while (end < bands && complete[static_cast<size_t>(end) * blocks + b] == c) ++end;
        w.rects[c].push_back(WavePlan::Rect{b * blockW, band * 32, blockW, std::min(plan.mapH, end * 32) - band * 32});
        band = end;
      }
    return w;
  }

  static bool isPinnedHost(const void* p) {
    cudaPointerAttributes a{};
    if (cudaPointerGetAttributes(&a, p) != cudaSuccess) {
      cudaGetLastError();
      return false;
    }
    return a.type == cudaMemoryTypeHost;
  }

  bool replayPlaneGraph(const DevicePlan& plan, const uint8_t* in, const uint8_t* out, int inW, int inH, int inPitch, int outW, int outH,
                        int outPitch) {
    for (PlaneGraph& c : planeGraphs_) {
      if (c.plan != &plan || c.in != in || c.out != out || c.inPitch != inPitch || c.outPitch != outPitch || c.generation != planGeneration_ ||
          c.stagingIn != stagingIn_.ptr || c.stagingOut != stagingOut_.ptr || c.inW != inW || c.inH != inH || c.outW != outW || c.outH != outH)
        continue;
      c.lastUse = ++graphClock_;
      CU(cudaGraphLaunch(c.exec, stream_));
      t360::countKernelLaunches(c.kernels);
      CU(cudaStreamSynchronize(stream_));
      return true;
    }
    return false;
  }

  bool transformHostPlanePipelined(const DevicePlan& plan, uint8_t* in, uint8_t* out, int inW, int inH, int inPitch, int outW, int outH,
                                   int outPitch, int planIndex, int imagePlaneIndex) {
    const long long bytes = static_cast<long long>(inW) * inH;
    const int chunks = pipelineChunks_ > 1 ? std::min(pipelineChunks_, 32)
                                           : static_cast<int>(std::min<long long>(8, std::max<long long>(2, bytes / (3ll << 20))));
    WavePlan& w = wavePlanFor(plan, planIndex, chunks);
    if (!copyIn_) {
      CU(cudaStreamCreateWithFlags(&copyIn_, cudaStreamNonBlocking));
      CU(cudaStreamCreateWithFlags(&copyIn2_, cudaStreamNonBlocking));
      CU(cudaStreamCreateWithFlags(&copyOut_, cudaStreamNonBlocking));
      for (cudaEvent_t* e : {&graphFork_, &graphJoinIn_, &graphJoinOut_}) CU(cudaEventCreateWithFlags(e, cudaEventDisableTiming));
    }
    while (static_cast<int>(chunkIn_.size()) < chunks) {
      cudaEvent_t a = nullptr, b = nullptr;
      CU(cudaEventCreateWithFlags(&a, cudaEventDisableTiming));
      chunkIn_.push_back(a);
      CU(cudaEventCreateWithFlags(&b, cudaEventDisableTiming));
      waveDone_.push_back(b);
    }
    pinIfRecurring(in, static_cast<size_t>(inPitch) * (inH - 1) + inW);
    pinIfRecurring(out, static_cast<size_t>(outPitch) * (outH - 1) + outW);
    const int dInPitch = alignedPitch(inW), dOutPitch = alignedPitch(outW);
    stagingIn_.reserve(static_cast<size_t>(dInPitch) * inH + 64);
    stagingOut_.reserve(static_cast<size_t>(dOutPitch) * outH + 64);
    PlaneLane& hostLane = slotFor(stream_).lanes[0];
    GatherWork work;
    if (!prepareGather(plan, stagingIn_.ptr, stagingOut_.ptr, inW, inH, dInPitch, outW, outH, dOutPitch, stream_, imagePlaneIndex, hostLane, work))
      return false;
    if (!work.staged) {
      CU(cudaMemcpy2DAsync(stagingIn_.ptr, dInPitch, in, inPitch, inW, inH, cudaMemcpyHostToDevice, stream_));
      gatherPlane(work, hostLane, stream_);
      CU(cudaMemcpy2DAsync(out, outPitch, stagingOut_.ptr, dOutPitch, outW, outH, cudaMemcpyDeviceToHost, stream_));
      CU(cudaStreamSynchronize(stream_));
      return true;
    }
    armScheduler(hostLane.claimCounter, stream_);
    CU(t360::prepareGatherFrame(plan.kernelSize));
    auto issue = [&](bool forkJoin) {
      if (forkJoin) {
        CU(cudaEventRecord(graphFork_, stream_));
        CU(cudaStreamWaitEvent(copyIn_, graphFork_, 0));
        if (pipelineInStreams_ > 1) CU(cudaStreamWaitEvent(copyIn2_, graphFork_, 0));
        CU(cudaStreamWaitEvent(copyOut_, graphFork_, 0));
      }
      t360::FrameGatherParams fp{};
      fp.plane[0] = work.view;
      fp.weightImage = reinterpret_cast<const uint4*>(weightImages_[plan.kernelSize].ptr);
      fp.kernelSize = plan.kernelSize;
      fp.numPlanes = 1;
      for (int c = 0; c < chunks; ++c) {
        const int r0 = c ? w.chunkRowEnd[c - 1] : 0, r1 = w.chunkRowEnd[c];
        cudaStream_t inStream = (pipelineInStreams_ > 1 && (c & 1)) ? copyIn2_ : copyIn_;
        if (r1 > r0)
          CU(cudaMemcpy2DAsync(stagingIn_.ptr + static_cast<size_t>(r0) * dInPitch, dInPitch, in + static_cast<size_t>(r0) * inPitch, inPitch, inW,
                               r1 - r0, cudaMemcpyHostToDevice, inStream));
        CU(cudaEventRecord(chunkIn_[c], inStream));
        CU(cudaStreamWaitEvent(stream_, chunkIn_[c], 0));
        const int n = w.waveStart[c + 1] - w.waveStart[c];
        if (n > 0) {
          t360::StagedParams jobs{w.jobs.ptr + w.waveStart[c], n, hostLane.claimCounter.ptr, nullptr};
          CU(t360::launchGatherFrame(fp, jobs, work.maps, numSMs_, stream_, false));
        }
        if (!w.rects[c].empty()) {
          CU(cudaEventRecord(waveDone_[c], stream_));
          CU(cudaStreamWaitEvent(copyOut_, waveDone_[c], 0));
          for (const WavePlan::Rect& r : w.rects[c])
            CU(cudaMemcpy2DAsync(out + static_cast<size_t>(r.y) * outPitch + r.x, outPitch,
                                 stagingOut_.ptr + static_cast<size_t>(r.y) * dOutPitch + r.x, dOutPitch, r.w, r.h, cudaMemcpyDeviceToHost, copyOut_));
        }
      }
      if (forkJoin) {
        if (pipelineInStreams_ > 1) {
          CU(cudaEventRecord(graphJoinIn_, copyIn2_));
          CU(cudaStreamWaitEvent(copyIn_, graphJoinIn_, 0));
        }
        CU(cudaEventRecord(graphJoinIn_, copyIn_));
        CU(cudaEventRecord(graphJoinOut_, copyOut_));
        CU(cudaStreamWaitEvent(stream_, graphJoinIn_, 0));
        CU(cudaStreamWaitEvent(stream_, graphJoinOut_, 0));
      }
    };
    if (std::getenv("T360B200_PIPELINE_TIMING")) {
      std::vector<cudaEvent_t> ev(3 * chunks + 1);
      for (cudaEvent_t& e : ev) CU(cudaEventCreate(&e));
      CU(cudaStreamSynchronize(stream_));
      CU(cudaEventRecord(ev[3 * chunks], stream_));
      CU(cudaStreamWaitEvent(copyIn_, ev[3 * chunks], 0));
      CU(cudaStreamWaitEvent(copyOut_, ev[3 * chunks], 0));
      t360::FrameGatherParams fp{};
      fp.plane[0] = work.view;
      fp.weightImage = reinterpret_cast<const uint4*>(weightImages_[plan.kernelSize].ptr);
      fp.kernelSize = plan.kernelSize;
      fp.numPlanes = 1;
      for (int c = 0; c < chunks; ++c) {
        const int r0 = c ? w.chunkRowEnd[c - 1] : 0, r1 = w.chunkRowEnd[c];
        CU(cudaMemcpy2DAsync(stagingIn_.ptr + static_cast<size_t>(r0) * dInPitch, dInPitch, in + static_cast<size_t>(r0) * inPitch, inPitch, inW,
                             r1 - r0, cudaMemcpyHostToDevice, copyIn_));
        CU(cudaEventRecord(ev[3 * c], copyIn_));
        CU(cudaStreamWaitEvent(stream_, ev[3 * c], 0));
        const int n = w.waveStart[c + 1] - w.waveStart[c];
        if (n > 0) {
          t360::StagedParams jobs{w.jobs.ptr + w.waveStart[c], n, hostLane.claimCounter.ptr, nullptr};
          CU(t360::launchGatherFrame(fp, jobs, work.maps, numSMs_, stream_, false));
        }
        CU(cudaEventRecord(ev[3 * c + 1], stream_));
        CU(cudaStreamWaitEvent(copyOut_, ev[3 * c + 1], 0));
        for (const WavePlan::Rect& r : w.rects[c])
          CU(cudaMemcpy2DAsync(out + static_cast<size_t>(r.y) * outPitch + r.x, outPitch, stagingOut_.ptr + static_cast<size_t>(r.y) * dOutPitch + r.x,
                               dOutPitch, r.w, r.h, cudaMemcpyDeviceToHost, copyOut_));
        CU(cudaEventRecord(ev[3 * c + 2], copyOut_));
      }
      CU(cudaStreamSynchronize(stream_));
      CU(cudaStreamSynchronize(copyOut_));
      std::printf("streamed plane %d (%dx%d -> %dx%d, %d chunks): chunk | H2D done | wave done (jobs) | D2H done (rects, bytes) [us]\n", imagePlaneIndex, inW,
                  inH, outW, outH, chunks);
      for (int c = 0; c < chunks; ++c) {
        float a = 0, b = 0, d = 0;
        cudaEventElapsedTime(&a, ev[3 * chunks], ev[3 * c]);
        cudaEventElapsedTime(&b, ev[3 * chunks], ev[3 * c + 1]);
        cudaEventElapsedTime(&d, ev[3 * chunks], ev[3 * c + 2]);
        long long bytes = 0;
        for (const WavePlan::Rect& r : w.rects[c]) bytes += static_cast<long long>(r.w) * r.h;
        std::printf("  %2d | %7.1f | %7.1f (%5d) | %7.1f (%2zu, %lld)\n", c, a * 1e3, b * 1e3, w.waveStart[c + 1] - w.waveStart[c], d * 1e3,
                    w.rects[c].size(), bytes);
      }
      for (cudaEvent_t e : ev) cudaEventDestroy(e);
      return true;
    }
    if (isPinnedHost(in) && isPinnedHost(out)) {
      PlaneGraph* g = nullptr;
      for (size_t i = 0; i < planeGraphs_.size();) {
        PlaneGraph& c = planeGraphs_[i];
        if (c.stagingIn != stagingIn_.ptr || c.stagingOut != stagingOut_.ptr || c.generation != planGeneration_) {
          cudaGraphExecDestroy(c.exec);
          planeGraphs_.erase(planeGraphs_.begin() + static_cast<long>(i));
          continue;
        }
        if (c.plan == &plan && c.in == in && c.out == out && c.inPitch == inPitch && c.outPitch == outPitch) g = &c;
        ++i;
      }
      if (!g) {
        if (planeGraphs_.size() >= 24) {
          auto oldest = std::min_element(planeGraphs_.begin(), planeGraphs_.end(), [](const PlaneGraph& a, const PlaneGraph& b) { return a.lastUse < b.lastUse; });
          cudaGraphExecDestroy(oldest->exec);
          planeGraphs_.erase(oldest);
        }
        CU(cudaStreamSynchronize(stream_));
        cudaGraph_t graph = nullptr;
        CU(cudaStreamBeginCapture(stream_, cudaStreamCaptureModeThreadLocal));
        try {
          issue(true);
        } catch (...) {
          cudaStreamEndCapture(stream_, &graph);
          if (graph) cudaGraphDestroy(graph);
          throw;
        }
        CU(cudaStreamEndCapture(stream_, &graph));
        cudaGraphExec_t exec = nullptr;
        const cudaError_t e = cudaGraphInstantiate(&exec, graph, 0);
        cudaGraphDestroy(graph);
        if (e != cudaSuccess) throw CudaFail{e, "cudaGraphInstantiate"};
        int kernels = 0;
        for (int c = 0; c < chunks; ++c) kernels += w.waveStart[c + 1] > w.waveStart[c];
        planeGraphs_.push_back(PlaneGraph{&plan, planGeneration_, in, out, inPitch, outPitch, stagingIn_.ptr, stagingOut_.ptr, inW, inH, outW, outH,
                                          kernels, exec, 0});
        g = &planeGraphs_.back();
        t360::countKernelLaunches(-kernels);
      }
      g->lastUse = ++graphClock_;
      CU(cudaGraphLaunch(g->exec, stream_));
      t360::countKernelLaunches(g->kernels);
      CU(cudaStreamSynchronize(stream_));
      return true;
    }
    issue(false);
    CU(cudaStreamSynchronize(stream_));
    CU(cudaStreamSynchronize(copyOut_));
    if (pipelineInStreams_ > 1) CU(cudaStreamSynchronize(copyIn2_));
    return true;
  }

  bool transformDevice(const uint8_t* dIn, uint8_t* dOut, int inW, int inH, int inPitch, int outW, int outH,
                       int outPitch, int planIndex, cudaStream_t stream) {
    try {
      const DeviceRestore restoreDevice = ensureDevice();
      const DevicePlan* plan = findPlan(planIndex, planIndex);
      if (!plan) return false;
      cudaStream_t s = stream ? stream : stream_;
      if (plan->transparent && planIndex) CU(cudaMemset2DAsync(dOut, outPitch, 128, outW, outH, s));
      return enqueue(*plan, dIn, dOut, inW, inH, inPitch, outW, outH, outPitch, s, planIndex, slotFor(s).lanes[0]);
    } catch (const CudaFail& f) {
      std::printf("Could not transform the plane %d. Error: CUDA %s (%s) in %s\n", planIndex, cudaGetErrorName(f.err),
                  cudaGetErrorString(f.err), f.what);
      cudaGetLastError();
    } catch (const std::exception& ex) {
      std::printf("Could not transform the plane %d. Error: %s\n", planIndex, ex.what());
    }
    return false;
  }

  bool transformFrameDevice(int numPlanes, const uint8_t* const* dIn, uint8_t* const* dOut, const int* inW, const int* inH,
                            const int* inPitch, const int* outW, const int* outH, const int* outPitch, cudaStream_t stream) {
    try {
      if (numPlanes < 1 || numPlanes > kPlaneLanes) {
        std::printf("Could not transform the frame. Error: %d planes (1..%d supported)\n", numPlanes, kPlaneLanes);
        return false;
      }
      const DeviceRestore restoreDevice = ensureDevice();
      cudaStream_t s = stream ? stream : stream_;
      StreamSlot& slot = slotFor(s);
      PlaneLane* lanes_ = slot.lanes;
      cudaEvent_t frameFork_ = slot.fork;
      const DevicePlan* plans[kPlaneLanes];
      bool sideWork = false;
      bool anyTransparent = false;
      for (int p = 0; p < numPlanes; ++p) {
        if (!(plans[p] = findPlan(p ? 1 : 0, p))) return false;
        if (p) sideWork = sideWork || plans[p]->lowPass || plans[p]->transparent;
        anyTransparent = anyTransparent || plans[p]->transparent;
      }
      const bool mergedBlur = !anyTransparent && blurFrame(plans, numPlanes, dIn, inW, inH, inPitch, lanes_, s);
      if (mergedBlur) sideWork = false;
      const bool fork = numPlanes > 1 && sideWork;
      if (fork) CU(cudaEventRecord(frameFork_, s));
      GatherWork work[kPlaneLanes];
      bool allStaged = true;
      for (int p = numPlanes - 1; p >= 0; --p) {
        cudaStream_t ps = (p && fork) ? lanes_[p].main : s;
        if (p && fork) CU(cudaStreamWaitEvent(ps, frameFork_, 0));
        if (plans[p]->transparent && p) CU(cudaMemset2DAsync(dOut[p], outPitch[p], 128, outW[p], outH[p], ps));
        if (!prepareGather(*plans[p], dIn[p], dOut[p], inW[p], inH[p], inPitch[p], outW[p], outH[p], outPitch[p], ps, p, lanes_[p], work[p], mergedBlur))
          return false;
        allStaged = allStaged && work[p].staged;
      }
      if (allStaged && numPlanes > 1) {
        if (fork)
          for (int p = 1; p < numPlanes; ++p) {
            CU(cudaEventRecord(lanes_[p].done, lanes_[p].main));
            CU(cudaStreamWaitEvent(s, lanes_[p].done, 0));
          }
        gatherFrame(work, numPlanes, s, slot);
        for (int p = 0; p < numPlanes; ++p) finishGather(work[p], s);
        return true;
      }
      if (numPlanes > 1 && !fork) CU(cudaEventRecord(frameFork_, s));
      for (int p = numPlanes - 1; p >= 0; --p) {
        cudaStream_t ps = p ? lanes_[p].main : s;
        if (p && !fork) CU(cudaStreamWaitEvent(ps, frameFork_, 0));
        if (work[p].plan->kernelSize) {
          gatherPlane(work[p], lanes_[p], ps);
          finishGather(work[p], ps);
        }
        if (p) CU(cudaEventRecord(lanes_[p].done, ps));
      }
      for (int p = 1; p < numPlanes; ++p) CU(cudaStreamWaitEvent(s, lanes_[p].done, 0));
      return true;
    } catch (const CudaFail& f) {
      std::printf("Could not transform the frame. Error: CUDA %s (%s) in %s\n", cudaGetErrorName(f.err), cudaGetErrorString(f.err), f.what);
      cudaGetLastError();
    } catch (const std::exception& ex) {
      std::printf("Could not transform the frame. Error: %s\n", ex.what());
    }
    return false;
  }

  bool lowPassDevice(const uint8_t* dIn, uint8_t* dOut, int w, int h, int inPitch, int outPitch, int planIndex,
                     cudaStream_t stream) {
    try {
      const DeviceRestore restoreDevice = ensureDevice();
      const DevicePlan* plan = findPlan(planIndex, planIndex);
      if (!plan) return false;
      if (!plan->lowPass) {
        std::printf("Could not filter plane %d. Error: plan has no low-pass stage\n", planIndex);
        return false;
      }
      runLowPass(*plan, dIn, dOut, w, h, inPitch, outPitch, stream ? stream : stream_);
      return true;
    } catch (const CudaFail& f) {
      std::printf("Could not filter plane %d. Error: CUDA %s (%s) in %s\n", planIndex, cudaGetErrorName(f.err),
                  cudaGetErrorString(f.err), f.what);
      cudaGetLastError();
    }
    return false;
  }

  void enableTrace(bool on) { traceEnabled_ = on; }
  size_t readTrace(unsigned long long* out, size_t maxWords) {
    if (!trace_.ptr) return 0;
    if (!out) return trace_.count;
    const size_t n = std::min(maxWords, trace_.count);
    if (cudaMemcpy(out, trace_.ptr, n * sizeof(unsigned long long), cudaMemcpyDeviceToHost) != cudaSuccess) return 0;
    return n;
  }

  bool synchronize() {
    if (!deviceReady_) return true;
    return cudaStreamSynchronize(stream_) == cudaSuccess;
  }
  cudaStream_t stream() {
    try { const DeviceRestore restoreDevice = ensureDevice(); } catch (...) { return nullptr; }
    return stream_;
  }
  bool tileCounts(int planIndex, int counts[4]) {
    std::lock_guard<std::mutex> lock(mu_);
    auto it = plans_.find(planIndex);
    if (it == plans_.end()) return false;
    counts[0] = it->second.totalStaged(); counts[1] = it->second.numFallback;
    counts[2] = it->second.blur.numStripJobs[0] + it->second.blur.numStripJobs[1] + it->second.blur.numStripJobs[2];
    counts[3] = it->second.blur.numTileJobs + it->second.blur.numDirectJobs;
    return true;
  }
  size_t planBytes(int planIndex) {
    std::lock_guard<std::mutex> lock(mu_);
    auto it = plans_.find(planIndex);
    return it == plans_.end() ? 0 : it->second.deviceBytes();
  }

 private:
  StreamSlot& slotFor(cudaStream_t s) {
    std::lock_guard<std::mutex> lock(slotMu_);
    std::unique_ptr<StreamSlot>& slot = slots_[s];
    if (!slot) {
      slot.reset(new StreamSlot);
      for (int i = 0; i < kPlaneLanes; ++i) {
        PlaneLane& l = slot->lanes[i];
        if (i > 0) CU(cudaStreamCreateWithFlags(&l.main, cudaStreamNonBlocking));
        CU(cudaEventCreateWithFlags(&l.done, cudaEventDisableTiming));
      }
      CU(cudaEventCreateWithFlags(&slot->fork, cudaEventDisableTiming));
    }
    return *slot;
  }

  struct DeviceRestore {
    int previous = -1;
    DeviceRestore() = default;
    DeviceRestore(const DeviceRestore&) = delete;
    DeviceRestore& operator=(const DeviceRestore&) = delete;
    DeviceRestore(DeviceRestore&& o) noexcept : previous(o.previous) { o.previous = -1; }
    ~DeviceRestore() { if (previous >= 0) cudaSetDevice(previous); }
  };
  DeviceRestore ensureDevice() {
    DeviceRestore guard;
    if (deviceReady_) {
      int current = device_;
      CU(cudaGetDevice(&current));
      if (current != device_) {
        CU(cudaSetDevice(device_));
        guard.previous = current;
      }
      return guard;
    }
    int n = 0;
    cudaError_t e = cudaGetDeviceCount(&n);
    if (e != cudaSuccess || n <= 0) throw CudaFail{e != cudaSuccess ? e : cudaErrorNoDevice, "cudaGetDeviceCount (no CUDA device: this library has no CPU fallback)"};
    CU(cudaGetDevice(&device_));
    cudaDeviceProp prop{};
    CU(cudaGetDeviceProperties(&prop, device_));
    numSMs_ = prop.multiProcessorCount;
    CU(cudaStreamCreateWithFlags(&stream_, cudaStreamNonBlocking));
    deviceReady_ = true;
    return guard;
  }

  void pinIfRecurring(const void* ptr, size_t bytes) {
    if (!pinHostPlanes_ || !ptr || !bytes) return;
    cudaPointerAttributes a{};
    if (cudaPointerGetAttributes(&a, ptr) != cudaSuccess) { cudaGetLastError(); return; }
    if (a.type != cudaMemoryTypeUnregistered) return;
    const uintptr_t page = 4096, lo = reinterpret_cast<uintptr_t>(ptr) & ~(page - 1);
    const size_t len = ((reinterpret_cast<uintptr_t>(ptr) + bytes + page - 1) & ~(page - 1)) - lo;
    for (HostRange& r : hostRanges_) {
      if (r.base != lo || r.bytes != len) continue;
      if (!r.pinned && ++r.seen >= 2) {
        if (cudaHostRegister(reinterpret_cast<void*>(lo), len, cudaHostRegisterDefault) == cudaSuccess) r.pinned = true;
        else { cudaGetLastError(); r.seen = -1000000; }
      }
      return;
    }
    if (hostRanges_.size() < 64) hostRanges_.push_back(HostRange{lo, len, 1, false});
  }

  static bool isDevicePointer(const void* p) {
    cudaPointerAttributes a{};
    if (cudaPointerGetAttributes(&a, p) != cudaSuccess) {
      cudaGetLastError();
      return false;
    }
    return a.type == cudaMemoryTypeDevice || a.type == cudaMemoryTypeManaged;
  }

  const DevicePlan* findPlan(int planIndex, int imagePlaneIndex) {
    std::lock_guard<std::mutex> lock(mu_);
    auto it = plans_.find(planIndex);
    if (it == plans_.end()) {
      std::printf("Could not transform the plane %d. Error: no map was generated for index %d\n", imagePlaneIndex, planIndex);
      return nullptr;
    }
    return &it->second;
  }

  const int16_t* deviceWeights(int interpolationAlg) {
    const int16_t* host = nullptr;
    const int k = t360::remapTable(interpolationAlg, &host);
    if (k < 2) return nullptr;
    auto& buf = weights_[k];
    if (!buf.ptr) {
      buf.reserve(static_cast<size_t>(1024) * k * k);
      CU(cudaMemcpy(buf.ptr, host, buf.bytes(), cudaMemcpyHostToDevice));
      const std::vector<uint8_t> image = t360::buildWeightImage(k, host);
      weightImages_[k].reserve(image.size());
      CU(cudaMemcpy(weightImages_[k].ptr, image.data(), image.size(), cudaMemcpyHostToDevice));
    }
    return buf.ptr;
  }

  DevicePlan upload(const HostPlan& h) {
    DevicePlan d;
    d.inW = h.inW; d.inH = h.inH; d.outW = h.outW; d.outH = h.outH; d.mapW = h.mapW; d.mapH = h.mapH;
    d.kernelSize = h.kernelSize;
    d.transparent = h.transparentBorder;
    if (d.kernelSize > 0) {
      deviceWeights(ctx_.interpolation_alg);
      t360::GatherPlan g;
      t360::buildGatherPlan(h, d.kernelSize >= 2 && !d.transparent, g);
      d.tilesPerRow = g.tilesPerRow;
      d.samples.reserve(g.records.size());
      CU(cudaMemcpy(d.samples.ptr, g.records.data(), g.records.size() * sizeof(int2), cudaMemcpyHostToDevice));
      d.numFallback = g.numGeneral;
      d.numSeam = g.numSeam;
      d.numShare = g.numShare;
      for (int c = 0; c < 2; ++c) d.numStaged[c] = g.numStaged[c];
      d.numJobs = static_cast<int>(g.jobs.size());
      if (!g.jobs.empty()) {
        std::vector<GatherJob> launchOrder = g.jobs;
        t360::spreadGeneralJobs(launchOrder);
        d.gatherJobs.reserve(launchOrder.size());
        CU(cudaMemcpy(d.gatherJobs.ptr, launchOrder.data(), launchOrder.size() * sizeof(GatherJob), cudaMemcpyHostToDevice));
      }
      if (!g.compact.empty()) {
        d.records.reserve(g.compact.size());
        CU(cudaMemcpy(d.records.ptr, g.compact.data(), g.compact.size() * sizeof(uint32_t), cudaMemcpyHostToDevice));
      }
      d.hostJobs = std::move(g.jobs);
      d.jobNeedRows = std::move(g.jobNeedRows);
    }
    d.lowPass = ctx_.enable_low_pass_filter != 0;
    if (d.lowPass) {
      d.segments = h.segments;
      d.planTaps = h.taps;
      buildBlurJobs(d.segments, d.planTaps, h.inW, h.inH, d.blur);
    }
    d.resizeNeeded = h.resize.needed;
    if (d.resizeNeeded) resizeFor(d, d.outW, d.outH);
    return d;
  }

  const DevicePlan::Resize& resizeFor(const DevicePlan& plan, int outW, int outH) {
    std::lock_guard<std::mutex> lock(lazyMu_);
    auto it = plan.resizes.find({outW, outH});
    if (it != plan.resizes.end()) return it->second;
    t360::AreaResizePlan r;
    t360::buildAreaResize(plan.mapW, plan.mapH, outW, outH, r);
    DevicePlan::Resize& d = plan.resizes[{outW, outH}];
    auto upload2 = [](const std::vector<int2>& v, DeviceBuffer<int2>& buf) {
      buf.reserve(std::max<size_t>(v.size(), 1));
      if (!v.empty()) CU(cudaMemcpy(buf.ptr, v.data(), v.size() * sizeof(int2), cudaMemcpyHostToDevice));
    };
    if (r.enlarge) {
      d.cellW = d.cellH = -1;
      d.xMax = r.lx.dmax;
      auto pack = [](const t360::AreaLinearAxis& a) {
        std::vector<int2> v(a.ofs.size());
        for (size_t i = 0; i < a.ofs.size(); ++i)
          v[i] = int2{a.ofs[i], static_cast<int>(static_cast<uint16_t>(a.coef[2 * i]) | (static_cast<uint32_t>(static_cast<uint16_t>(a.coef[2 * i + 1])) << 16))};
        return v;
      };
      upload2(pack(r.lx), d.xLinear);
      upload2(pack(r.ly), d.yLinear);
    } else if (r.cellW > 0) {
      d.cellW = r.cellW; d.cellH = r.cellH;
    } else {
      auto uploadAxis = [&](const t360::AreaAxis& a, DeviceBuffer<int2>& taps, DeviceBuffer<int>& first) {
        std::vector<int2> packed(a.taps.size());
        for (size_t i = 0; i < a.taps.size(); ++i) {
          int bits;
          std::memcpy(&bits, &a.taps[i].alpha, sizeof(bits));
          packed[i] = int2{a.taps[i].src, bits};
        }
        upload2(packed, taps);
        first.reserve(a.first.size());
        CU(cudaMemcpy(first.ptr, a.first.data(), a.first.size() * sizeof(int), cudaMemcpyHostToDevice));
      };
      uploadAxis(r.x, d.xTaps, d.xFirst);
      uploadAxis(r.y, d.yTaps, d.yFirst);
    }
    return d;
  }

  void buildBlurJobs(const std::vector<t360::LowPassSegment>& segments, const std::vector<float>& planTaps, int planeW, int planeH,
                     DevicePlan::BlurSet& d) {
    struct { const std::vector<t360::LowPassSegment>& segments; const std::vector<float>& taps; int inW, inH; } h{segments, planTaps, planeW, planeH};
    std::vector<BlurJob> tiles, direct;
    std::vector<StripJob> strips[t360::kStripMaxHy];
    std::vector<float> taps = h.taps;
    int offX[2] = {0, 0}, offY[2] = {0, 0}, passes = 1;
    if (ctx_.input_stereo_format == STEREO_FORMAT_LR) { passes = 2; offX[1] = static_cast<int>(0.5 * h.inW); }
    else if (ctx_.input_stereo_format == STEREO_FORMAT_TB) { passes = 2; offY[1] = static_cast<int>(0.5 * h.inH); }
    std::vector<uint8_t> covered(static_cast<size_t>(h.inW) * h.inH, 0);
    int tileSmem = 0;
    const long long stripsPerRow = (h.inW + t360::kStripW - 1) / t360::kStripW;
    const long long wanted = static_cast<long long>(h.inH) * stripsPerRow / 5000;
    const int rowsBudget = wanted >= 32 ? 32 : (wanted >= 16 ? 16 : 8);

    auto sameTaps = [&](int offA, int nA, int offB, int nB) {
      return nA == nB && (offA == offB || std::memcmp(&h.taps[offA], &h.taps[offB], sizeof(float) * nA) == 0);
    };
    std::map<std::pair<int, int>, std::pair<int, int>> paddedKx;
    auto padKx = [&](int off, int n) {
      auto it = paddedKx.find({off, n});
      if (it != paddedKx.end()) return it->second;
      while (taps.size() % 4) taps.push_back(0.f);
      const int at = static_cast<int>(taps.size()), chunks = (n + 3) / 4;
      for (int i = 0; i < chunks * 4; ++i) taps.push_back(i < n ? h.taps[off + i] : 0.f);
      return paddedKx[{off, n}] = std::make_pair(at, chunks);
    };
    std::map<int, int> paddedKy1;
    auto padKy = [&](int off, int n) {
      if (n != 1) return off;
      auto it = paddedKy1.find(off);
      if (it != paddedKy1.end()) return it->second;
      const int at = static_cast<int>(taps.size());
      taps.push_back(0.f); taps.push_back(h.taps[off]); taps.push_back(0.f);
      return paddedKy1[off] = at;
    };

    for (int pass = 0; pass < passes; ++pass) {
      auto fits = [&](const t360::LowPassSegment& g) {
        const int l = g.left + offX[pass], t = g.top + offY[pass];
        return l >= 0 && t >= 0 && g.width > 0 && g.height > 0 && l + g.width <= h.inW && t + g.height <= h.inH;
      };
      size_t i = 0;
      while (i < h.segments.size()) {
        t360::LowPassSegment s = h.segments[i];
        size_t j = i + 1;
        if (!fits(s)) { i = j; continue; }
        while (j < h.segments.size()) {
          const t360::LowPassSegment& n = h.segments[j];
          if (n.top != s.top || n.height != s.height || n.left != s.left + s.width || !fits(n) ||
              !sameTaps(n.kxOffset, n.kxCount, s.kxOffset, s.kxCount) || !sameTaps(n.kyOffset, n.kyCount, s.kyOffset, s.kyCount))
            break;
          s.width += n.width;
          ++j;
        }
        i = j;
        const int left = s.left + offX[pass], top = s.top + offY[pass];
        for (int y = 0; y < s.height; ++y) std::memset(&covered[static_cast<size_t>(top + y) * h.inW + left], 1, s.width);
        const int hy = s.kyCount / 2;
        if (hy <= t360::kStripMaxHy && (s.kyCount & 1) && (s.kxCount & 1)) {
          const auto kx = padKx(s.kxOffset, s.kxCount);
          const int kyOff = padKy(s.kyOffset, s.kyCount), hx = s.kxCount / 2;
          const int rows = std::min(rowsBudget, kx.second <= 3 ? 32 : (kx.second <= 8 ? 16 : 8));
          for (int ty = 0; ty < s.height; ty += rows)
            for (int tx = 0; tx < s.width; tx += t360::kStripW) {
              StripJob j{left + tx, top + ty, std::min(t360::kStripW, s.width - tx), std::min(rows, s.height - ty),
                         kx.first, kx.second, s.kxCount, kyOff, 0};
              const int firstByte = j.x0 - hx, lastByte = j.x0 + t360::kStripW - t360::kStripLanePx - hx + 4 * (kx.second + 3) + 7;
              j.edge = (firstByte - 4 < 0 || lastByte >= h.inW) ? 1 : 0;
              strips[std::max(hy, 1) - 1].push_back(j);
            }
        } else {
          for (int ty = 0; ty < s.height; ty += t360::kBlurTileH)
            for (int tx = 0; tx < s.width; tx += t360::kBlurTileW) {
              BlurJob j{left + tx, top + ty, std::min(t360::kBlurTileW, s.width - tx), std::min(t360::kBlurTileH, s.height - ty),
                        s.kxOffset, s.kxCount, s.kyOffset, s.kyCount};
              const long long need = static_cast<long long>(t360::blurTileSmem(j.w, j.h, j.kxCount, j.kyCount));
              if (need <= t360::kBlurMaxSmem) {
                tiles.push_back(j);
                tileSmem = std::max(tileSmem, static_cast<int>(need));
              } else {
                direct.push_back(j);
              }
            }
        }
      }
    }
    d.needsClear = std::find(covered.begin(), covered.end(), 0) != covered.end();
    for (int c = 0; c < t360::kStripMaxHy; ++c) {
      std::stable_sort(strips[c].begin(), strips[c].end(), [](const StripJob& a, const StripJob& b) {
        return static_cast<long long>(a.kxChunks + 2) * a.h * (1 + 3 * a.edge) > static_cast<long long>(b.kxChunks + 2) * b.h * (1 + 3 * b.edge);
      });
      d.numStripJobs[c] = static_cast<int>(strips[c].size());
      d.hostStrips[c] = strips[c];
      if (strips[c].empty()) continue;
      d.stripJobs[c].reserve(strips[c].size());
      CU(cudaMemcpy(d.stripJobs[c].ptr, strips[c].data(), strips[c].size() * sizeof(StripJob), cudaMemcpyHostToDevice));
    }
    d.numTileJobs = static_cast<int>(tiles.size());
    d.numDirectJobs = static_cast<int>(direct.size());
    d.tileSmem = tileSmem;
    if (!tiles.empty()) {
      d.tileJobs.reserve(tiles.size());
      CU(cudaMemcpy(d.tileJobs.ptr, tiles.data(), tiles.size() * sizeof(BlurJob), cudaMemcpyHostToDevice));
    }
    if (!direct.empty()) {
      d.directJobs.reserve(direct.size());
      CU(cudaMemcpy(d.directJobs.ptr, direct.data(), direct.size() * sizeof(BlurJob), cudaMemcpyHostToDevice));
    }
    d.hostTaps = taps;
    if (!taps.empty()) {
      d.taps.reserve(taps.size());
      CU(cudaMemcpy(d.taps.ptr, taps.data(), taps.size() * sizeof(float), cudaMemcpyHostToDevice));
    }
  }

  const DevicePlan::BlurSet& blurFor(const DevicePlan& plan, int w, int h) {
    if (w == plan.inW && h == plan.inH) return plan.blur;
    std::lock_guard<std::mutex> lock(lazyMu_);
    auto it = plan.otherBlurs.find({w, h});
    if (it != plan.otherBlurs.end()) return it->second;
    DevicePlan::BlurSet& set = plan.otherBlurs[{w, h}];
    buildBlurJobs(plan.segments, plan.planTaps, w, h, set);
    return set;
  }

  void runLowPass(const DevicePlan& plan, const uint8_t* dIn, uint8_t* dOut, int w, int h, int inPitch, int outPitch,
                  cudaStream_t s) {
    const DevicePlan::BlurSet& b = blurFor(plan, w, h);
    if (b.needsClear) CU(cudaMemset2DAsync(dOut, outPitch, 0, w, h, s));
    for (int c = 0; c < t360::kStripMaxHy; ++c) {
      if (!b.numStripJobs[c]) continue;
      t360::StripParams sp{dIn, dOut, w, h, inPitch, outPitch, b.stripJobs[c].ptr, b.numStripJobs[c], b.taps.ptr};
      CU(t360::launchBlurStrips(sp, c + 1, s));
    }
    t360::BlurParams bp{dIn, dOut, w, h, inPitch, outPitch, b.tileJobs.ptr, b.numTileJobs, b.taps.ptr, b.tileSmem};
    if (b.numTileJobs) CU(t360::launchBlur(bp, s));
    if (b.numDirectJobs) {
      bp.jobs = b.directJobs.ptr;
      bp.numJobs = b.numDirectJobs;
      CU(t360::launchBlurDirect(bp, s));
    }
  }

  static bool planeMaps(PlaneLane& lane, const uint8_t* src, int w, int h, int pitch, int k,
                        CUtensorMap (&out)[t360::kNumBoxClasses][t360::kBoxVariants]) {
    for (const PlaneMaps& e : lane.mapCache)
      if (e.base == src && e.w == w && e.h == h && e.pitch == pitch && e.k == k) {
        std::memcpy(out, e.maps, sizeof(e.maps));
        return true;
      }
    PlaneMaps fresh;
    for (int c = 0; c < t360::kNumBoxClasses; ++c)
      for (int v = 0; v < t360::kBoxVariants; ++v) {
        if (v > 0 && t360::boxVariantRows(k, c, v) == t360::boxVariantRows(k, c, 0)) {
          fresh.maps[c][v] = fresh.maps[c][0];
          continue;
        }
        if (!encodePlaneMap(&fresh.maps[c][v], src, w, h, pitch, k, c, v)) return false;
      }
    fresh.base = src; fresh.w = w; fresh.h = h; fresh.pitch = pitch; fresh.k = k;
    lane.mapCache[lane.mapCacheNext] = fresh;
    lane.mapCacheNext = (lane.mapCacheNext + 1) % PlaneLane::kMapCache;
    std::memcpy(out, fresh.maps, sizeof(fresh.maps));
    return true;
  }

  bool enqueue(const DevicePlan& plan, const uint8_t* dIn, uint8_t* dOut, int inW, int inH, int inPitch, int outW,
               int outH, int outPitch, cudaStream_t s, int imagePlaneIndex, PlaneLane& lane) {
    GatherWork w;
    if (!prepareGather(plan, dIn, dOut, inW, inH, inPitch, outW, outH, outPitch, s, imagePlaneIndex, lane, w)) return false;
    if (plan.kernelSize == 0) return true;
    gatherPlane(w, lane, s);
    finishGather(w, s);
    return true;
  }

  bool prepareGather(const DevicePlan& plan, const uint8_t* dIn, uint8_t* dOut, int inW, int inH, int inPitch, int outW,
                     int outH, int outPitch, cudaStream_t s, int imagePlaneIndex, PlaneLane& lane, GatherWork& w, bool blurDone = false) {
    w.plan = &plan;
    w.imagePlane = imagePlaneIndex;
    if (plan.kernelSize == 0) {
      std::printf("Could not find interpolation algorithm for plane %d", imagePlaneIndex);
      return true;
    }
    w.finalOut = dOut;
    w.finalPitch = outPitch;
    w.finalW = outW;
    w.finalH = outH;
    w.resizeTables = nullptr;
    if (outW != plan.mapW || outH != plan.mapH) {
      w.resizeTables = &resizeFor(plan, outW, outH);
      const int sp = alignedPitch(plan.mapW);
      lane.scaled.reserve(static_cast<size_t>(sp) * plan.mapH + 64);
      if (plan.transparent) CU(cudaMemset2DAsync(lane.scaled.ptr, sp, planIndexOf(plan) ? 128 : 0, plan.mapW, plan.mapH, s));
      dOut = lane.scaled.ptr;
      outPitch = sp;
      outW = plan.mapW;
      outH = plan.mapH;
    }
    const uint8_t* src = dIn;
    int srcPitch = inPitch;
    if (plan.lowPass) {
      const int bp = alignedPitch(inW);
      lane.blurred.reserve(static_cast<size_t>(bp) * inH + 64);
      if (!blurDone) runLowPass(plan, dIn, lane.blurred.ptr, inW, inH, inPitch, bp, s);
      src = lane.blurred.ptr;
      srcPitch = bp;
    }
    w.view = t360::PlaneView{src, dOut, plan.samples.ptr, reinterpret_cast<const uint4*>(plan.records.ptr), inW, inH, srcPitch,
                             outW, outH, outPitch, plan.tilesPerRow, 0};
    w.staged = plan.totalStaged() > 0 && !plan.transparent && inW == plan.inW && inH == plan.inH;
    if (w.staged) w.staged = planeMaps(lane, src, inW, inH, srcPitch, plan.kernelSize, w.maps);
    return true;
  }

  static void armScheduler(DeviceBuffer<int>& counter, cudaStream_t s) {
    if (counter.ptr) return;
    counter.reserve(2);
    CU(cudaMemsetAsync(counter.ptr, 0, 2 * sizeof(int), s));
  }

  void gatherPlane(const GatherWork& w, PlaneLane& lane, cudaStream_t s) {
    const DevicePlan& plan = *w.plan;
    if (w.staged) {
      armScheduler(lane.claimCounter, s);
      t360::FrameGatherParams fp{};
      fp.plane[0] = w.view;
      fp.weightImage = reinterpret_cast<const uint4*>(weightImages_[plan.kernelSize].ptr);
      fp.kernelSize = plan.kernelSize;
      fp.numPlanes = 1;
      t360::StagedParams jobs{plan.gatherJobs.ptr, plan.numJobs, lane.claimCounter.ptr, nullptr};
      CU(t360::launchGatherFrame(fp, jobs, w.maps, numSMs_, s));
    } else {
      const t360::PlaneView& v = w.view;
      t360::GatherParams gp{v.src, v.srcW, v.srcH, v.srcPitch, v.dst, v.dstW, v.dstH, v.dstPitch, v.samples, v.tilesPerRow,
                            weights_[plan.kernelSize].ptr, plan.kernelSize, plan.transparent ? 1 : 0};
      CU(t360::launchGather(gp, numSMs_, s));
    }
  }

  bool blurFrame(const DevicePlan* const* plans, int numPlanes, const uint8_t* const* dIn, const int* inW, const int* inH, const int* inPitch,
                 PlaneLane* lanes, cudaStream_t s) {
    if (numPlanes < 2) return false;
    for (int p = 0; p < numPlanes; ++p) {
      const DevicePlan& plan = *plans[p];
      if (!plan.lowPass || inW[p] != plan.inW || inH[p] != plan.inH || plan.blur.numTileJobs || plan.blur.numDirectJobs || plan.blur.needsClear)
        return false;
    }
    FrameBlurList& f = frameBlur_;
    {
      std::lock_guard<std::mutex> lock(frameJobsMu_);
      if (f.generation != planGeneration_ || f.numPlanes != numPlanes) {
        std::vector<StripJob> merged[t360::kStripMaxHy];
        std::vector<float> taps;
        for (int p = 0; p < numPlanes; ++p) {
          const DevicePlan::BlurSet& b = plans[p]->blur;
          while (taps.size() % 4) taps.push_back(0.f);
          const int base = static_cast<int>(taps.size());
          taps.insert(taps.end(), b.hostTaps.begin(), b.hostTaps.end());
          for (int c = 0; c < t360::kStripMaxHy; ++c)
            for (StripJob j : b.hostStrips[c]) {
              j.kxOffset += base;
              j.kyOffset += base;
              j.edge |= p << t360::kStripPlaneShift;
              merged[c].push_back(j);
            }
        }
        CU(cudaDeviceSynchronize());
        for (int c = 0; c < t360::kStripMaxHy; ++c) {
          std::stable_sort(merged[c].begin(), merged[c].end(), [](const StripJob& a, const StripJob& b) {
            return static_cast<long long>(a.kxChunks + 2) * a.h * (1 + 3 * (a.edge & 1)) > static_cast<long long>(b.kxChunks + 2) * b.h * (1 + 3 * (b.edge & 1));
          });
          f.numJobs[c] = static_cast<int>(merged[c].size());
          if (merged[c].empty()) continue;
          f.jobs[c].reserve(merged[c].size());
          CU(cudaMemcpy(f.jobs[c].ptr, merged[c].data(), merged[c].size() * sizeof(StripJob), cudaMemcpyHostToDevice));
        }
        f.taps.reserve(std::max<size_t>(taps.size(), 4));
        CU(cudaMemcpy(f.taps.ptr, taps.data(), taps.size() * sizeof(float), cudaMemcpyHostToDevice));
        f.numPlanes = numPlanes;
        f.generation = planGeneration_;
      }
    }
    t360::FrameStripParams fp{};
    for (int p = 0; p < numPlanes; ++p) {
      const int bp = alignedPitch(inW[p]);
      lanes[p].blurred.reserve(static_cast<size_t>(bp) * inH[p] + 64);
      fp.plane[p] = {dIn[p], lanes[p].blurred.ptr, inW[p], inH[p], inPitch[p], bp};
    }
    fp.taps = f.taps.ptr;
    for (int c = 0; c < t360::kStripMaxHy; ++c) {
      if (!f.numJobs[c]) continue;
      fp.jobs = f.jobs[c].ptr;
      fp.numJobs = f.numJobs[c];
      CU(t360::launchBlurFrameStrips(fp, c + 1, s));
    }
    return true;
  }

  void gatherFrame(const GatherWork* work, int numPlanes, cudaStream_t s, StreamSlot& slot) {
    FrameJobList& f = frameJobs_;
    std::unique_lock<std::mutex> listLock(frameJobsMu_);
    if (f.generation != planGeneration_ || f.numPlanes != numPlanes) {
      std::vector<GatherJob> merged;
      const int order[7] = {t360::kJobGeneral, t360::kJobSeam, t360::kJobClass1, t360::kJobShareStay, t360::kJobShare, t360::kJobClass0, t360::kJobClass0};
      for (int step = 0; step < 7; ++step)
        for (int p = 0; p < numPlanes; ++p)
          for (GatherJob t : work[p].plan->hostJobs) {
            const int kind = order[step];
            if (((t.outY >> t360::kJobKindShift) & t360::kJobKindMask) != kind) continue;
            if (kind == t360::kJobClass0 && ((t.outX & t360::kJobQuadMask) != 0) != (step == 6)) continue;
            t.outY |= p << t360::kJobPlaneShift;
            merged.push_back(t);
          }
      t360::spreadGeneralJobs(merged);
      CU(cudaDeviceSynchronize());
      f.tiles.reserve(merged.size());
      CU(cudaMemcpy(f.tiles.ptr, merged.data(), merged.size() * sizeof(GatherJob), cudaMemcpyHostToDevice));
      f.numTiles = static_cast<int>(merged.size());
      f.numPlanes = numPlanes;
      f.generation = planGeneration_;
    }
    listLock.unlock();
    armScheduler(slot.frameClaim, s);
    t360::FrameGatherParams fp{};
    CUtensorMap maps[kPlaneLanes][t360::kNumBoxClasses][t360::kBoxVariants];
    for (int p = 0; p < numPlanes; ++p) {
      fp.plane[p] = work[p].view;
      std::memcpy(maps[p], work[p].maps, sizeof(work[p].maps));
    }
    fp.weightImage = reinterpret_cast<const uint4*>(weightImages_[work[0].plan->kernelSize].ptr);
    fp.kernelSize = work[0].plan->kernelSize;
    fp.numPlanes = numPlanes;
    if (traceEnabled_) {
      trace_.reserve(static_cast<size_t>(numSMs_) * t360::gatherGroups(work[0].plan->kernelSize) * t360::kTraceJobsPerGroup * 4);
      CU(cudaMemsetAsync(trace_.ptr, 0, trace_.bytes(), s));
    }
    t360::StagedParams jobs{f.tiles.ptr, f.numTiles, slot.frameClaim.ptr, traceEnabled_ ? trace_.ptr : nullptr};
    CU(t360::launchGatherFrame(fp, jobs, maps, numSMs_, s));
  }

  void finishGather(const GatherWork& w, cudaStream_t s) {
    const DevicePlan& plan = *w.plan;
    if (!w.resizeTables) return;
    const DevicePlan::Resize& r = *static_cast<const DevicePlan::Resize*>(w.resizeTables);
    t360::AreaParams ap{w.view.dst, w.finalOut, plan.mapW, plan.mapH, w.view.dstPitch, w.finalW, w.finalH, w.finalPitch,
                        r.cellW, r.cellH, r.xTaps.ptr, r.xFirst.ptr, r.yTaps.ptr, r.yFirst.ptr, r.xLinear.ptr, r.yLinear.ptr, r.xMax};
    CU(t360::launchAreaResize(ap, s));
  }

  int planIndexOf(const DevicePlan& plan) {
    std::lock_guard<std::mutex> lock(mu_);
    for (auto& kv : plans_)
      if (&kv.second == &plan) return kv.first;
    return 0;
  }

  FrameTransformContext ctx_;
  std::mutex mu_;
  std::mutex lazyMu_;
  std::map<int, DevicePlan> plans_;
  DeviceBuffer<int16_t> weights_[9];
  DeviceBuffer<uint8_t> weightImages_[9];
  DeviceBuffer<uint8_t> stagingIn_, stagingOut_;
  std::mutex hostCallMu_;
  cudaStream_t copyIn_ = nullptr, copyIn2_ = nullptr, copyOut_ = nullptr;
  std::vector<cudaEvent_t> chunkIn_, waveDone_;
  WavePlan wavePlans_[2];
  long long pipelineMinBytes_ = 6ll << 20;
  int pipelineChunks_ = 0, pipelineBlocks_ = 0;
  int pipelineInStreams_ = 1;
  struct PlaneGraph {
    const void* plan; unsigned long long generation; const void* in; const void* out; int inPitch, outPitch;
    const void* stagingIn; const void* stagingOut;
    int inW, inH, outW, outH;
    int kernels;
    cudaGraphExec_t exec; unsigned long long lastUse;
  };
  std::vector<PlaneGraph> planeGraphs_;
  unsigned long long graphClock_ = 0;
  cudaEvent_t graphFork_ = nullptr, graphJoinIn_ = nullptr, graphJoinOut_ = nullptr;
  struct HostRange { uintptr_t base; size_t bytes; int seen; bool pinned; };
  std::vector<HostRange> hostRanges_;
  bool pinHostPlanes_ = false;
  std::mutex slotMu_;
  std::map<cudaStream_t, std::unique_ptr<StreamSlot>> slots_;
  FrameJobList frameJobs_;
  FrameBlurList frameBlur_;
  std::mutex frameJobsMu_;
  DeviceBuffer<unsigned long long> trace_;
  bool traceEnabled_ = false;
  unsigned long long planGeneration_ = 0;
  cudaStream_t stream_ = nullptr;
  int device_ = 0, numSMs_ = 0;
  bool deviceReady_ = false;
};

T360_API VideoFrameTransform* VideoFrameTransform_new(FrameTransformContext* ctx) {
  if (!ctx) return nullptr;
  return new (std::nothrow) VideoFrameTransform(ctx);
}

T360_API void VideoFrameTransform_delete(VideoFrameTransform* transform) { delete transform; }

T360_API int VideoFrameTransform_generateMapForPlane(VideoFrameTransform* transform, int inputWidth, int inputHeight,
                                                     int outputWidth, int outputHeight, int transformMatPlaneIndex) {
  if (!transform) return 0;
  return transform->generateMapForPlane(inputWidth, inputHeight, outputWidth, outputHeight, transformMatPlaneIndex);
}

T360_API int VideoFrameTransform_transformFramePlane(VideoFrameTransform* transform, uint8_t* inputData,
                                                     uint8_t* outputData, int inputWidth, int inputHeight,
                                                     int inputWidthWithPadding, int outputWidth, int outputHeight,
                                                     int outputWidthWithPadding, int transformMatPlaneIndex,
                                                     int imagePlaneIndex) {
  if (!transform) return 0;
  return transform->transformFramePlane(inputData, outputData, inputWidth, inputHeight, inputWidthWithPadding,
                                        outputWidth, outputHeight, outputWidthWithPadding, transformMatPlaneIndex,
                                        imagePlaneIndex);
}

struct T360HostPlan {
  HostPlan plan;
  t360::GatherPlan gather;
  bool gatherBuilt = false;
};

T360_API T360HostPlan* T360B200_hostPlanCreate(const FrameTransformContext* ctx, int inW, int inH, int outW, int outH) {
  if (!ctx) return nullptr;
  std::unique_ptr<T360HostPlan> p(new (std::nothrow) T360HostPlan);
  if (!p) return nullptr;
  try {
    if (!t360::buildHostPlan(*ctx, inW, inH, outW, outH, p->plan)) return nullptr;
  } catch (const std::exception& ex) {
    std::printf("Could not build the host plan. Error: %s\n", ex.what());
    return nullptr;
  }
  return p.release();
}
T360_API void T360B200_hostPlanDestroy(T360HostPlan* plan) { delete plan; }
T360_API int T360B200_hostPlanInfo(const T360HostPlan* plan, int info[6]) {
  if (!plan || !info) return 0;
  info[0] = plan->plan.mapW; info[1] = plan->plan.mapH;
  info[2] = static_cast<int>(plan->plan.segments.size());
  info[3] = static_cast<int>(plan->plan.taps.size());
  info[4] = plan->plan.kernelSize;
  info[5] = 0;
  return 1;
}
T360_API const float* T360B200_hostPlanMap(const T360HostPlan* plan) { return plan ? plan->plan.map.data() : nullptr; }
T360_API const int32_t* T360B200_hostPlanSamples(const T360HostPlan* plan) {
  return plan && !plan->plan.samples.empty() ? reinterpret_cast<const int32_t*>(plan->plan.samples.data()) : nullptr;
}
T360_API int T360B200_hostPlanGather(T360HostPlan* plan, int info[10], const int32_t** jobs, const int32_t** records,
                                     const uint32_t** compact) {
  if (!plan || !info || plan->plan.kernelSize <= 0) return 0;
  try {
    if (!plan->gatherBuilt) {
      t360::buildGatherPlan(plan->plan, plan->plan.kernelSize >= 2 && !plan->plan.transparentBorder, plan->gather);
      plan->gatherBuilt = true;
    }
  } catch (const std::exception& ex) {
    std::printf("Could not build the gather plan. Error: %s\n", ex.what());
    return 0;
  }
  const t360::GatherPlan& g = plan->gather;
  info[0] = g.tilesPerRow; info[1] = g.tileRows; info[2] = g.tileH; info[3] = static_cast<int>(g.jobs.size());
  info[4] = g.numStaged[0]; info[5] = g.numStaged[1]; info[6] = g.numSeam; info[7] = g.numGeneral;
  info[8] = g.numShare; info[9] = static_cast<int>(g.compact.size());
  if (jobs) *jobs = g.jobs.empty() ? nullptr : reinterpret_cast<const int32_t*>(g.jobs.data());
  if (records) *records = reinterpret_cast<const int32_t*>(g.records.data());
  if (compact) *compact = g.compact.empty() ? nullptr : g.compact.data();
  return 1;
}
T360_API int T360B200_hostPlanSegment(const T360HostPlan* plan, int i, int rect[4], int numTaps[2], const float** kx,
                                      const float** ky) {
  if (!plan || i < 0 || i >= static_cast<int>(plan->plan.segments.size())) return 0;
  const t360::LowPassSegment& s = plan->plan.segments[i];
  rect[0] = s.left; rect[1] = s.top; rect[2] = s.width; rect[3] = s.height;
  numTaps[0] = s.kxCount; numTaps[1] = s.kyCount;
  if (kx) *kx = plan->plan.taps.data() + s.kxOffset;
  if (ky) *ky = plan->plan.taps.data() + s.kyOffset;
  return 1;
}
T360_API int T360B200_remapTable(int interpolationAlg, const int16_t** table) { return t360::remapTable(interpolationAlg, table); }
T360_API int T360B200_dealLanes(int interpolationAlg, int n, const int32_t* phases, int32_t* laneOf, int32_t* copyOf) {
  const int16_t* table = nullptr;
  const int k = t360::remapTable(interpolationAlg, &table);
  if (k < 2 || n < 0 || n > 32 || !phases || !laneOf || !copyOf) return -1;
  int slot[32], lane[32], copy[32];
  for (int i = 0; i < n; ++i) slot[i] = t360::weightSlotOf(k, phases[i] & 1023);
  const int wavefronts = t360::dealLanes(k, t360::weightCopies(k), n, slot, lane, copy);
  for (int i = 0; i < n; ++i) { laneOf[i] = lane[i]; copyOf[i] = copy[i]; }
  return wavefronts;
}

T360_API int T360B200_weightImage(int interpolationAlg, const uint8_t** image) {
  static std::mutex mu;
  static std::map<int, std::vector<uint8_t>> images;
  const int16_t* table = nullptr;
  const int k = t360::remapTable(interpolationAlg, &table);
  if (k < 2 || !image) return 0;
  std::lock_guard<std::mutex> lock(mu);
  auto it = images.find(k);
  if (it == images.end()) it = images.emplace(k, t360::buildWeightImage(k, table)).first;
  *image = it->second.data();
  return static_cast<int>(it->second.size());
}

T360_API int T360B200_transformFramePlaneAsync(VideoFrameTransform* t, const uint8_t* dIn, uint8_t* dOut, int inW, int inH,
                                               int inPitch, int outW, int outH, int outPitch, int planIndex, void* stream) {
  if (!t || !dIn || !dOut) return 0;
  return t->transformDevice(dIn, dOut, inW, inH, inPitch, outW, outH, outPitch, planIndex, static_cast<cudaStream_t>(stream));
}
T360_API int T360B200_transformFrameAsync(VideoFrameTransform* t, int numPlanes, const uint8_t* const* dIn, uint8_t* const* dOut,
                                          const int* inW, const int* inH, const int* inPitch, const int* outW, const int* outH,
                                          const int* outPitch, void* stream) {
  if (!t || !dIn || !dOut || !inW || !inH || !inPitch || !outW || !outH || !outPitch) return 0;
  return t->transformFrameDevice(numPlanes, dIn, dOut, inW, inH, inPitch, outW, outH, outPitch, static_cast<cudaStream_t>(stream));
}
T360_API int T360B200_lowPassPlaneAsync(VideoFrameTransform* t, const uint8_t* dIn, uint8_t* dOut, int w, int h, int inPitch,
                                        int outPitch, int planIndex, void* stream) {
  if (!t || !dIn || !dOut) return 0;
  try {
    return t->lowPassDevice(dIn, dOut, w, h, inPitch, outPitch, planIndex, static_cast<cudaStream_t>(stream));
  } catch (const std::exception& ex) {
    std::printf("Could not filter plane %d. Error: %s\n", planIndex, ex.what());
    return 0;
  }
}
T360_API void T360B200_setPinHostPlanes(VideoFrameTransform* t, int enable) { if (t) t->setPinHostPlanes(enable != 0); }
T360_API void T360B200_debugTrace(VideoFrameTransform* t, int enable) { if (t) t->enableTrace(enable != 0); }
T360_API unsigned long long T360B200_debugTraceRead(VideoFrameTransform* t, unsigned long long* out, unsigned long long maxWords) {
  return t ? t->readTrace(out, maxWords) : 0;
}
T360_API int T360B200_synchronize(VideoFrameTransform* t) { return t ? t->synchronize() : 0; }
T360_API void* T360B200_stream(VideoFrameTransform* t) { return t ? t->stream() : nullptr; }
T360_API unsigned long long T360B200_kernelLaunchCount(void) { return t360::kernelLaunchCount(); }
T360_API unsigned long long T360B200_planDeviceBytes(VideoFrameTransform* t, int planIndex) { return t ? t->planBytes(planIndex) : 0; }
T360_API int T360B200_planTileCounts(VideoFrameTransform* t, int planIndex, int counts[4]) {
  return t && counts ? t->tileCounts(planIndex, counts) : 0;
}
T360_API int T360B200_deviceCount(void) {
  int n = 0;
  if (cudaGetDeviceCount(&n) != cudaSuccess) {
    cudaGetLastError();
    return 0;
  }
  return n;
}
T360_API const char* T360B200_version(void) { return "transform360-b200 0.1 (sm_90a)"; }
```

### transform360_b200/handler.py

```python
from __future__ import annotations

import ctypes as C
import os
from pathlib import Path

import numpy as np

PKG = Path(__file__).resolve().parent
LIB_PATH = PKG / "lib" / "libTransform360.so"

LAYOUT_CUBEMAP_32, LAYOUT_CUBEMAP_23_OFFCENTER, LAYOUT_FLAT_FIXED, LAYOUT_EQUIRECT = 0, 1, 2, 3
LAYOUT_BARREL, LAYOUT_BARREL_SPLIT, LAYOUT_EAC_32, LAYOUT_N = 4, 5, 6, 7
STEREO_FORMAT_TB, STEREO_FORMAT_LR, STEREO_FORMAT_MONO, STEREO_FORMAT_GUESS, STEREO_FORMAT_N = 0, 1, 2, 3, 4
NEAREST, LINEAR, CUBIC, LANCZOS4 = 0, 1, 2, 4


class FrameTransformContext(C.Structure):
    _fields_ = [
        ("input_layout", C.c_int), ("output_layout", C.c_int),
        ("input_stereo_format", C.c_int), ("output_stereo_format", C.c_int),
        ("vflip", C.c_int), ("input_expand_coef", C.c_float), ("expand_coef", C.c_float),
        ("interpolation_alg", C.c_int), ("width_scale_factor", C.c_float),
        ("height_scale_factor", C.c_float), ("fixed_yaw", C.c_float), ("fixed_pitch", C.c_float),
        ("fixed_roll", C.c_float), ("fixed_hfov", C.c_float), ("fixed_vfov", C.c_float),
        ("fixed_cube_offcenter_x", C.c_float), ("fixed_cube_offcenter_y", C.c_float),
        ("fixed_cube_offcenter_z", C.c_float), ("is_horizontal_offset", C.c_int),
        ("enable_low_pass_filter", C.c_int), ("kernel_height_scale_factor", C.c_float),
        ("min_kernel_half_height", C.c_float), ("max_kernel_half_height", C.c_float),
        ("enable_multi_threading", C.c_int), ("num_vertical_segments", C.c_int),
        ("num_horizontal_segments", C.c_int), ("adjust_kernel", C.c_int),
        ("kernel_adjust_factor", C.c_float),
    ]


FILTER_DEFAULTS = dict(
    input_layout=LAYOUT_EQUIRECT, output_layout=LAYOUT_CUBEMAP_32, input_stereo_format=STEREO_FORMAT_MONO,
    output_stereo_format=STEREO_FORMAT_MONO, vflip=0, input_expand_coef=1.01, expand_coef=1.01,
    interpolation_alg=CUBIC, width_scale_factor=1.0, height_scale_factor=1.0, fixed_yaw=0.0, fixed_pitch=0.0,
    fixed_roll=0.0, fixed_hfov=120.0, fixed_vfov=110.0, fixed_cube_offcenter_x=0.0, fixed_cube_offcenter_y=0.0,
    fixed_cube_offcenter_z=0.0, is_horizontal_offset=0, enable_low_pass_filter=1, kernel_height_scale_factor=1.0,
    min_kernel_half_height=1.0, max_kernel_half_height=10000.0, enable_multi_threading=1, num_vertical_segments=5,
    num_horizontal_segments=1, adjust_kernel=1, kernel_adjust_factor=1.0)


def make_context(**overrides) -> FrameTransformContext:
    vals = dict(FILTER_DEFAULTS)
    for k in overrides:
        if k not in vals:
            raise AttributeError(f"FrameTransformContext has no field {k!r}")
    vals.update(overrides)
    return FrameTransformContext(**vals)


_lib = None


def load(path: os.PathLike | None = None):
    global _lib
    if _lib is not None and path is None:
        return _lib
    p = Path(path) if path else Path(os.environ.get("T360B200_LIB") or LIB_PATH)
    if not p.exists():
        raise FileNotFoundError(f"{p} not found: build it with `python -m transform360_b200.build` (needs nvcc); "
                                "transform360_b200 has no CPU fallback")
    L = C.CDLL(str(p), mode=os.RTLD_LOCAL)
    vp, ci = C.c_void_p, C.c_int
    L.VideoFrameTransform_new.restype = vp
    L.VideoFrameTransform_new.argtypes = [C.POINTER(FrameTransformContext)]
    L.VideoFrameTransform_delete.restype = None
    L.VideoFrameTransform_delete.argtypes = [vp]
    L.VideoFrameTransform_generateMapForPlane.restype = ci
    L.VideoFrameTransform_generateMapForPlane.argtypes = [vp] + [ci] * 5
    L.VideoFrameTransform_transformFramePlane.restype = ci
    L.VideoFrameTransform_transformFramePlane.argtypes = [vp, vp, vp] + [ci] * 8
    L.T360B200_hostPlanCreate.restype = vp
    L.T360B200_hostPlanCreate.argtypes = [C.POINTER(FrameTransformContext)] + [ci] * 4
    L.T360B200_hostPlanDestroy.restype = None
    L.T360B200_hostPlanDestroy.argtypes = [vp]
    L.T360B200_hostPlanInfo.restype = ci
    L.T360B200_hostPlanInfo.argtypes = [vp, C.POINTER(ci)]
    L.T360B200_hostPlanMap.restype = vp
    L.T360B200_hostPlanMap.argtypes = [vp]
    L.T360B200_hostPlanSamples.restype = vp
    L.T360B200_hostPlanSamples.argtypes = [vp]
    L.T360B200_hostPlanSegment.restype = ci
    L.T360B200_hostPlanSegment.argtypes = [vp, ci, C.POINTER(ci), C.POINTER(ci), C.POINTER(vp), C.POINTER(vp)]
    L.T360B200_hostPlanGather.restype = ci
    L.T360B200_hostPlanGather.argtypes = [vp, C.POINTER(ci), C.POINTER(vp), C.POINTER(vp), C.POINTER(vp)]
    L.T360B200_weightImage.restype = ci
    L.T360B200_weightImage.argtypes = [ci, C.POINTER(vp)]
    L.T360B200_remapTable.restype = ci
    L.T360B200_remapTable.argtypes = [ci, C.POINTER(vp)]
    L.T360B200_transformFramePlaneAsync.restype = ci
    L.T360B200_transformFramePlaneAsync.argtypes = [vp, vp, vp] + [ci] * 7 + [vp]
    L.T360B200_transformFrameAsync.restype = ci
    L.T360B200_transformFrameAsync.argtypes = [vp, ci, vp, vp] + [vp] * 6 + [vp]
    L.T360B200_lowPassPlaneAsync.restype = ci
    L.T360B200_lowPassPlaneAsync.argtypes = [vp, vp, vp] + [ci] * 5 + [vp]
    L.T360B200_setPinHostPlanes.restype = None
    L.T360B200_setPinHostPlanes.argtypes = [vp, ci]
    L.T360B200_debugTrace.restype = None
    L.T360B200_debugTrace.argtypes = [vp, ci]
    L.T360B200_debugTraceRead.restype = C.c_ulonglong
    L.T360B200_debugTraceRead.argtypes = [vp, vp, C.c_ulonglong]
    L.T360B200_synchronize.restype = ci
    L.T360B200_synchronize.argtypes = [vp]
    L.T360B200_stream.restype = vp
    L.T360B200_stream.argtypes = [vp]
    L.T360B200_kernelLaunchCount.restype = C.c_ulonglong
    L.T360B200_planDeviceBytes.restype = C.c_ulonglong
    L.T360B200_planDeviceBytes.argtypes = [vp, ci]
    L.T360B200_planTileCounts.restype = ci
    L.T360B200_planTileCounts.argtypes = [vp, ci, C.POINTER(ci)]
    L.T360B200_deviceCount.restype = ci
    L.T360B200_version.restype = C.c_char_p
    if path is None:
        _lib = L
    return L


EXPORTED_SYMBOLS = [
    "VideoFrameTransform_new", "VideoFrameTransform_delete", "VideoFrameTransform_generateMapForPlane",
    "VideoFrameTransform_transformFramePlane", "T360B200_hostPlanCreate", "T360B200_hostPlanDestroy",
    "T360B200_hostPlanInfo", "T360B200_hostPlanMap", "T360B200_hostPlanSamples", "T360B200_hostPlanSegment",
    "T360B200_hostPlanGather", "T360B200_weightImage", "T360B200_dealLanes",
    "T360B200_remapTable", "T360B200_transformFramePlaneAsync", "T360B200_transformFrameAsync",
    "T360B200_lowPassPlaneAsync",
    "T360B200_setPinHostPlanes", "T360B200_debugTrace", "T360B200_debugTraceRead", "T360B200_synchronize", "T360B200_stream", "T360B200_kernelLaunchCount", "T360B200_planDeviceBytes",
    "T360B200_planTileCounts", "T360B200_deviceCount", "T360B200_version",
]


class VideoFrameTransform:

    def __init__(self, ctx: FrameTransformContext):
        self._lib = load()
        self.ctx = ctx
        self._h = self._lib.VideoFrameTransform_new(C.byref(ctx))
        if not self._h:
            raise MemoryError("VideoFrameTransform_new returned NULL")

    def close(self):
        if getattr(self, "_h", None):
            self._lib.VideoFrameTransform_delete(self._h)
            self._h = None

    __del__ = close

    def __enter__(self):
        return self

    def __exit__(self, *exc):
        self.close()

    def generateMapForPlane(self, inputWidth, inputHeight, outputWidth, outputHeight, transformMatPlaneIndex) -> bool:
        return bool(self._lib.VideoFrameTransform_generateMapForPlane(
            self._h, inputWidth, inputHeight, outputWidth, outputHeight, transformMatPlaneIndex))

    def transformFramePlane(self, inputData, outputData, inputWidth, inputHeight, inputWidthWithPadding,
                            outputWidth, outputHeight, outputWidthWithPadding, transformMatPlaneIndex,
                            imagePlaneIndex) -> bool:
        return bool(self._lib.VideoFrameTransform_transformFramePlane(
            self._h, inputData, outputData, inputWidth, inputHeight, inputWidthWithPadding, outputWidth,
            outputHeight, outputWidthWithPadding, transformMatPlaneIndex, imagePlaneIndex))

    def transform_plane(self, src: np.ndarray, out_w: int, out_h: int, plan_index: int, image_plane: int = 0,
                        out: np.ndarray | None = None) -> np.ndarray:
        assert src.dtype == np.uint8 and src.ndim == 2 and src.strides[1] == 1
        if out is None:
            out = np.zeros((out_h, out_w), np.uint8)
        assert out.dtype == np.uint8 and out.shape == (out_h, out_w) and out.strides[1] == 1
        ok = self.transformFramePlane(src.ctypes.data, out.ctypes.data, src.shape[1], src.shape[0], src.strides[0],
                                      out_w, out_h, out.strides[0], plan_index, image_plane)
        if not ok:
            raise RuntimeError("VideoFrameTransform_transformFramePlane returned 0 (message on stdout)")
        return out

    def transform_plane_async(self, d_in: int, d_out: int, in_w, in_h, in_pitch, out_w, out_h, out_pitch, plan_index,
                              stream: int = 0) -> bool:
        return bool(self._lib.T360B200_transformFramePlaneAsync(self._h, d_in, d_out, in_w, in_h, in_pitch, out_w,
                                                                out_h, out_pitch, plan_index, stream))

    def make_frame_call(self, in_planes, out_planes, dims):
        n = len(in_planes)
        VP, IA = C.c_void_p * n, C.c_int * n
        d_in = VP(*[p[0] for p in in_planes])
        d_out = VP(*[p[0] for p in out_planes])
        arrs = [IA(*[d[0] for d in dims]), IA(*[d[1] for d in dims]), IA(*[p[1] for p in in_planes]),
                IA(*[d[2] for d in dims]), IA(*[d[3] for d in dims]), IA(*[p[1] for p in out_planes])]
        fn, h = self._lib.T360B200_transformFrameAsync, self._h
        ptrs = [C.cast(a, C.c_void_p) for a in arrs]
        pin, pout = C.cast(d_in, C.c_void_p), C.cast(d_out, C.c_void_p)

        def call(stream: int = 0, _keep=(d_in, d_out, arrs)) -> bool:
            return bool(fn(h, n, pin, pout, *ptrs, stream))
        return call

    def low_pass_async(self, d_in: int, d_out: int, w, h, in_pitch, out_pitch, plan_index, stream: int = 0) -> bool:
        return bool(self._lib.T360B200_lowPassPlaneAsync(self._h, d_in, d_out, w, h, in_pitch, out_pitch, plan_index,
                                                         stream))

    def set_pin_host_planes(self, enable: bool) -> None:
        self._lib.T360B200_setPinHostPlanes(self._h, 1 if enable else 0)

    def debug_trace(self, enable: bool) -> None:
        self._lib.T360B200_debugTrace(self._h, 1 if enable else 0)

    def read_trace(self) -> np.ndarray:
        buf = np.zeros(int(self._lib.T360B200_debugTraceRead(self._h, None, 0)), np.uint64)
        n = int(self._lib.T360B200_debugTraceRead(self._h, buf.ctypes.data, buf.size)) if buf.size else 0
        return buf[:n].reshape(-1, 64, 4)

    def synchronize(self) -> bool:
        return bool(self._lib.T360B200_synchronize(self._h))

    @property
    def stream(self) -> int:
        return self._lib.T360B200_stream(self._h) or 0

    def plan_tile_counts(self, plan_index):
        c = (C.c_int * 4)()
        if not self._lib.T360B200_planTileCounts(self._h, plan_index, c):
            raise KeyError(plan_index)
        return tuple(c)

    def plan_device_bytes(self, plan_index) -> int:
        return int(self._lib.T360B200_planDeviceBytes(self._h, plan_index))


class HostPlan:

    def __init__(self, ctx: FrameTransformContext, in_w, in_h, out_w, out_h):
        self._lib = load()
        self._h = self._lib.T360B200_hostPlanCreate(C.byref(ctx), in_w, in_h, out_w, out_h)
        if not self._h:
            raise ValueError("T360B200_hostPlanCreate failed (message on stdout)")
        info = (C.c_int * 6)()
        self._lib.T360B200_hostPlanInfo(self._h, info)
        self.map_w, self.map_h, self.num_segments, self.num_taps, self.kernel_size = info[0], info[1], info[2], info[3], info[4]

    def close(self):
        if getattr(self, "_h", None):
            self._lib.T360B200_hostPlanDestroy(self._h)
            self._h = None

    __del__ = close

    @property
    def map(self) -> np.ndarray:
        p = self._lib.T360B200_hostPlanMap(self._h)
        n = self.map_w * self.map_h * 2
        return np.frombuffer((C.c_float * n).from_address(p), np.float32).reshape(self.map_h, self.map_w, 2).copy()

    @property
    def samples(self) -> np.ndarray:
        p = self._lib.T360B200_hostPlanSamples(self._h)
        n = self.map_w * self.map_h * 2
        return np.frombuffer((C.c_int32 * n).from_address(p), np.int32).reshape(self.map_h, self.map_w, 2).copy()

    def gather_plan(self):
        info = (C.c_int * 10)()
        jobs, recs, comp = C.c_void_p(), C.c_void_p(), C.c_void_p()
        if not self._lib.T360B200_hostPlanGather(self._h, info, C.byref(jobs), C.byref(recs), C.byref(comp)):
            raise ValueError("T360B200_hostPlanGather failed")
        tpr, trows, th, nj = info[0], info[1], info[2], info[3]
        n = tpr * trows * th * 32 * 2
        records = np.frombuffer((C.c_int32 * n).from_address(recs.value), np.int32).reshape(tpr * trows, th, 32, 2).copy()
        j = compact = None
        if nj and jobs.value:
            j = np.frombuffer((C.c_int32 * (nj * 4)).from_address(jobs.value), np.int32).reshape(nj, 4).copy()
        if info[9] and comp.value:
            compact = np.frombuffer((C.c_uint32 * info[9]).from_address(comp.value), np.uint32).copy()
        return dict(tiles_per_row=tpr, tile_rows=trows, tile_h=th, jobs=j, records=records, compact=compact,
                    counts=dict(class0=info[4], class1=info[5], seam=info[6], general=info[7], share=info[8]))

    def segments(self):
        out = []
        rect, nk = (C.c_int * 4)(), (C.c_int * 2)()
        kx, ky = C.c_void_p(), C.c_void_p()
        for i in range(self.num_segments):
            assert self._lib.T360B200_hostPlanSegment(self._h, i, rect, nk, C.byref(kx), C.byref(ky))
            a = np.frombuffer((C.c_float * nk[0]).from_address(kx.value), np.float32).copy()
            b = np.frombuffer((C.c_float * nk[1]).from_address(ky.value), np.float32).copy()
            out.append((rect[0], rect[1], rect[2], rect[3], a, b))
        return out


def remap_table(interpolation_alg: int) -> np.ndarray | None:
    L = load()
    p = C.c_void_p()
    k = L.T360B200_remapTable(interpolation_alg, C.byref(p))
    if k < 2:
        return None
    return np.frombuffer((C.c_int16 * (1024 * k * k)).from_address(p.value), np.int16).reshape(1024, k, k).copy()


def deal_lanes(interpolation_alg: int, phases) -> tuple[int, np.ndarray, np.ndarray]:
    L = load()
    ph = np.ascontiguousarray(phases, np.int32)
    lane, copy = np.zeros(ph.size, np.int32), np.zeros(ph.size, np.int32)
    L.T360B200_dealLanes.restype = C.c_int
    L.T360B200_dealLanes.argtypes = [C.c_int, C.c_int, C.c_void_p, C.c_void_p, C.c_void_p]
    w = L.T360B200_dealLanes(interpolation_alg, ph.size, ph.ctypes.data, lane.ctypes.data, copy.ctypes.data)
    if w < 0:
        raise ValueError("T360B200_dealLanes refused the arguments")
    return int(w), lane, copy


def weight_image(interpolation_alg: int) -> np.ndarray | None:
    L = load()
    p = C.c_void_p()
    n = L.T360B200_weightImage(interpolation_alg, C.byref(p))
    if n <= 0:
        return None
    return np.frombuffer((C.c_uint8 * n).from_address(p.value), np.uint8).copy()


def kernel_launch_count() -> int:
    return int(load().T360B200_kernelLaunchCount())


def device_count() -> int:
    return int(load().T360B200_deviceCount())
```

Baseline: 627,000.

## Replace general fallback tiles with TMA-staged pole-cap and border pixel jobs

Tiles that could not be staged (general jobs near the poles) used to be computed by reading each pixel's source rows straight from global memory. They are now split into two new job kinds. Cap jobs group interior pixels by source row and column into TMA-staged boxes, with per-lane records so the shared-memory stage path can be used. Border jobs carry explicit per-pixel records and use the clamped gather. This moves pole traffic onto the staged pipeline and replaces the special general-job interleaving with a rank-based launch order, at the cost of more host planning and extra record storage.

```diff
diff --git a/include/transform360_b200.h b/include/transform360_b200.h
--- a/include/transform360_b200.h
+++ b/include/transform360_b200.h
@@ -17,6 +17,8 @@
 const int32_t* T360B200_hostPlanSamples(const T360HostPlan* plan);
 int T360B200_hostPlanGather(T360HostPlan* plan, int info[10], const int32_t** jobs, const int32_t** records,
                             const uint32_t** compact);
+int T360B200_hostPlanPoleCaps(T360HostPlan* plan, int info[4], const int32_t** capJobs, const uint32_t** capRecords,
+                              const int32_t** launchJobs);
 int T360B200_dealLanes(int interpolationAlg, int n, const int32_t* phases, int32_t* laneOf, int32_t* copyOf);
 int T360B200_weightImage(int interpolationAlg, const uint8_t** image);
 int T360B200_hostPlanSegment(const T360HostPlan* plan, int i, int rect[4], int numTaps[2], const float** kx,
diff --git a/profiles/trace_frame.py b/profiles/trace_frame.py
--- a/profiles/trace_frame.py
+++ b/profiles/trace_frame.py
@@ -11,7 +11,7 @@
 from transform360_b200 import synth
 from transform360_b200.stream import FrameTransformer, StreamSpec
 
-KINDS = {0: "class0", 1: "class1", 2: "general", 3: "share-stay", 4: "share", 5: "nop", 7: "seam"}
+KINDS = {0: "class0", 1: "class1", 3: "share-stay", 4: "share", 5: "nop", 7: "seam", 8: "pole-cap", 9: "border"}
 
 
 def main():
diff --git a/transform360_b200/csrc/gather_frame.cu b/transform360_b200/csrc/gather_frame.cu
--- a/transform360_b200/csrc/gather_frame.cu
+++ b/transform360_b200/csrc/gather_frame.cu
@@ -226,53 +226,33 @@
   });
 }
 
+template <int K, int PITCH, int VS>
+__device__ __forceinline__ void computeCapJob(const PlaneView& pv, uint32_t stageAddr, uint32_t recAddr, int steps, uint32_t wAddr,
+                                              int warp, int lane) {
+  static_assert(PITCH % 4 == 0, "");
+  for (int s = warp; s < steps; s += kGroupWarps) {
+    const uint2 r = ldsVec2Imm<0>(recAddr + s * kCapStepBytes + lane * 8);
+    if (r.x & kRecordSkip) continue;
+    const uint32_t rowAddr = stageAddr + (r.x & 0x7ffcu);
+    const int sh = (int)(r.x << 3);
+    RowBytes<K> W[K];
+    staticFor<K>([&](auto R) { W[decltype(R)::value] = loadRow<K, decltype(R)::value * PITCH>(rowAddr, sh); });
+    const int acc = foldPixel<K, VS>(W, wAddr, (r.x >> 17) & kSlotFieldMask);
+    pv.dst[(size_t)(r.y >> 16) * pv.dstPitch + (r.y & 0xffffu)] = (uint8_t)biasedToByte(acc);
+  }
+}
+
 template <int K, int VS>
-__device__ __forceinline__ void computeGeneralJob(const PlaneView& pv, int outX, int outY, const unsigned char* wsmem, uint32_t wAddr,
-                                                  int lane, int warp) {
+__device__ __forceinline__ void computeBorderJob(const PlaneView& pv, uint32_t recAddr, int n, const unsigned char* wsmem, int warp, int lane) {
   SrcView sv;
   sv.bytes = pv.src;
   sv.misalign = (int)(reinterpret_cast<uintptr_t>(pv.src) & 3);
   sv.words = reinterpret_cast<const uint32_t*>(pv.src - sv.misalign);
   sv.w = pv.srcW; sv.h = pv.srcH; sv.pitch = pv.srcPitch;
-  const int y0 = outY + warp * kRowsPerThread;
-  if (outX + lane >= pv.dstW) return;
-  const int2* segment = pv.samples + ((size_t)(y0 / gatherTileH(K)) * pv.tilesPerRow + outX / kGatherTileW) * gatherTileH(K) * kGatherTileW +
-                        (y0 % gatherTileH(K)) * kGatherTileW + lane;
-  int2 full[kRowsPerThread];
-#pragma unroll
-  for (int j = 0; j < kRowsPerThread; ++j) full[j] = y0 + j < pv.dstH ? loadPlan(segment + j * kGatherTileW) : make_int2(0, 0);
-  constexpr int kBatch = K == 8 ? 2 : 4;
-#pragma unroll
-  for (int jb = 0; jb < kRowsPerThread; jb += kBatch) {
-    RowBytes<K> W[kBatch][K];
-    bool interior[kBatch];
-#pragma unroll
-    for (int b = 0; b < kBatch; ++b) {
-      const int col0 = recordCol0(full[jb + b].x), row0 = full[jb + b].y >> 10;
-      interior[b] = y0 + jb + b < pv.dstH && col0 >= 0 && row0 >= 0 && col0 + (K == 2 ? 8 : K + 4) <= sv.w && row0 + K <= sv.h;
-#pragma unroll
-      for (int r = 0; r < K; ++r) {
-        W[b][r].b[0] = 0;
-        if constexpr (K == 8) W[b][r].b[1] = 0;
-        if (interior[b]) {
-          const int off = (row0 + r) * sv.pitch + col0 + sv.misalign;
-          const uint32_t* q = sv.words + (off >> 2);
-          const int sh = (off & 3) * 8;
-          const uint32_t q0 = __ldg(q), q1 = __ldg(q + 1);
-          W[b][r].b[0] = __funnelshift_r(q0, q1, sh);
-          if constexpr (K == 8) W[b][r].b[1] = __funnelshift_r(q1, __ldg(q + 2), sh);
-        }
-      }
-    }
-#pragma unroll
-    for (int b = 0; b < kBatch; ++b) {
-      const int j = jb + b;
-      if (y0 + j >= pv.dstH) continue;
-      int v;
-      if (interior[b]) v = biasedToByte(foldPixel<K, VS>(W[b], wAddr, (uint32_t)weightSlotOf(K, full[j].y & 1023) << 4));
-      else v = gatherPixel<K, false, VS, weightDiagonal(K)>(sv, wsmem, recordCol0(full[j].x), full[j].y);
-      pv.dst[(size_t)(y0 + j) * pv.dstPitch + outX + recordColumn(full[j].x)] = (uint8_t)v;
-    }
+  for (int i = warp * 32 + lane; i < n; i += kGroupThreads) {
+    const uint4 r = ldsVecImm<0>(recAddr + i * kBorderPixelBytes);
+    const int v = gatherPixel<K, false, VS, weightDiagonal(K)>(sv, wsmem, (int)r.x, (int)r.y);
+    pv.dst[(size_t)(r.z >> 16) * pv.dstPitch + (r.z & 0xffffu)] = (uint8_t)v;
   }
 }
 
@@ -393,19 +373,22 @@
       if (lane == 0) {
         unsigned char* rec = groupBase + S * kStage + st * kRec;
         *reinterpret_cast<int4*>(rec) = h;
-        if (kind == kJobShare || kind == kJobShareStay || kind == kJobClass0 || kind == kJobClass1 || kind == kJobSeam) {
+        if (kind == kJobExit) {
+          mbarArrive(full + st);
+        } else {
           const int pl = h.y >> kJobPlaneShift;
-          const bool share = boxClassOf(kind) == 2;
-          const int cls = boxClassOf(kind), variant = jobBoxVariant(h.z), boxX = jobBoxX(h.z), boxY = jobBoxY(h.z);
-          const uint32_t boxBytes = (uint32_t)(stageBoxW(K, cls) * boxVariantRows(K, cls, variant));
-          const uint32_t recBytes = share ? shareJobRecordBytes(K) : tileJobRecordBytes(h.x);
-          mbarExpectTx(full + st, (kind == kJobSeam ? 2 : 1) * boxBytes + recBytes);
-          tmaLoadBox(groupBase + st * kStage, &maps.map[pl][cls][variant], boxX, boxY, full + st);
-          if (kind == kJobSeam)
-            tmaLoadBox(groupBase + (st + 1) * kStage, &maps.map[pl][0][variant], boxX - planes[pl].srcW, boxY, full + st);
+          const uint32_t recBytes = (uint32_t)jobRecordBytes(K, kind, h.x);
+          if (kind == kJobBorder) {
+            mbarExpectTx(full + st, recBytes);
+          } else {
+            const int cls = boxClassOf(kind), variant = jobBoxVariant(h.z), boxX = jobBoxX(h.z), boxY = jobBoxY(h.z);
+            const uint32_t boxBytes = (uint32_t)(stageBoxW(K, cls) * boxVariantRows(K, cls, variant));
+            mbarExpectTx(full + st, (kind == kJobSeam ? 2 : 1) * boxBytes + recBytes);
+            tmaLoadBox(groupBase + st * kStage, &maps.map[pl][cls][variant], boxX, boxY, full + st);
+            if (kind == kJobSeam)
+              tmaLoadBox(groupBase + (st + 1) * kStage, &maps.map[pl][0][variant], boxX - planes[pl].srcW, boxY, full + st);
+          }
           bulkCopyToShared(rec + 128, planes[pl].records + (unsigned)h.w, recBytes, full + st);
-        } else {
-          mbarArrive(full + st);
         }
       }
       advance();
@@ -436,9 +419,10 @@
   unsigned long long* trace = jobs.trace && warp == 0 && lane == 0 ? jobs.trace + (size_t)(blockIdx.x * GROUPS + group) * kTraceJobsPerGroup * 4 : nullptr;
   uint32_t traced = 0;
   for (uint32_t st = 0, phase = 0;;) {
-    const unsigned long long t0 = trace ? now() : 0;
+    unsigned long long* const row = trace && traced < kTraceJobsPerGroup ? trace + traced * 4 : nullptr;
+    if (row) row[0] = now();
     mbarWait(full + st, phase);
-    const unsigned long long t1 = trace ? now() : 0;
+    if (row) row[1] = now();
     const uint32_t rec = recAddr + st * kRec;
     const uint4 h = ldsVec(rec);
     const int kind = ((int)h.y >> kJobKindShift) & kJobKindMask;
@@ -485,13 +469,15 @@
       }
       groupBarrier(group);
       computeTileJob<K, stageBoxW(K, 0), VS>(pv, boxAddr + st * kStage, outX, outY, ldsVec(rec + 128 + warp * 512 + lane * 16), wAddr, warp);
-    } else if (kind == kJobGeneral) {
-      computeGeneralJob<K, VS>(pv, outX, outY, wsmem, wAddr, lane, warp);
+    } else if (kind == kJobCap) {
+      computeCapJob<K, stageBoxW(K, 0), VS>(pv, boxAddr + st * kStage, rec + 128, (int)h.x, wAddr, warp, lane);
+    } else if (kind == kJobBorder) {
+      computeBorderJob<K, VS>(pv, rec + 128, (int)h.x, wsmem, warp, lane);
     }
     __syncwarp();
     if (lane == 0) mbarArrive(empty + st);
-    if (trace && traced < kTraceJobsPerGroup) {
-      trace[traced * 4 + 0] = t0; trace[traced * 4 + 1] = t1; trace[traced * 4 + 2] = now(); trace[traced * 4 + 3] = kind;
+    if (row) {
+      row[2] = now(); row[3] = kind;
       ++traced;
     }
     if (++st == S) { st = 0; phase ^= 1; }
diff --git a/transform360_b200/csrc/gather_plan.cpp b/transform360_b200/csrc/gather_plan.cpp
--- a/transform360_b200/csrc/gather_plan.cpp
+++ b/transform360_b200/csrc/gather_plan.cpp
@@ -4,7 +4,9 @@
 #include <climits>
 #include <cstdint>
 #include <cstring>
+#include <stdexcept>
 #include <thread>
+#include <utility>
 
 namespace t360 {
 namespace {
@@ -310,6 +312,124 @@
     }
 }
 
+JobRect tileRect(const GatherJob& job, int k) {
+  const int kind = (job.outY >> kJobKindShift) & kJobKindMask, quad = (job.outX & kJobQuadMask) - 1;
+  JobRect r;
+  r.x0 = job.outX & ~kJobQuadMask;
+  r.y0 = job.outY & kJobRowMask;
+  if (quad >= 0) { r.x0 += 16 * (quad & 1); r.y0 += 16 * (quad >> 1); }
+  const bool share = kind == kJobShare || kind == kJobShareStay;
+  r.x1 = r.x0 + (quad >= 0 ? 16 : (share ? kShareW : kGatherTileW));
+  r.y1 = r.y0 + (quad >= 0 ? 16 : (share ? shareH(k) : kFrameTileH));
+  return r;
+}
+
+struct PixelJob {
+  GatherJob job;
+  std::vector<uint32_t> words;
+  JobRect rect;
+  int needRows;
+};
+
+struct CapPixel {
+  int x, y, col0, rowPhase;
+  int row() const { return rowPhase >> 10; }
+};
+
+PixelJob capJob(const HostPlan& h, const CapPixel* px, int n) {
+  const int k = h.kernelSize, copies = weightCopies(k), pitch = stageBoxW(k, 0);
+  PixelJob j;
+  int minC = INT32_MAX, minR = INT32_MAX, maxR = INT32_MIN;
+  j.rect = JobRect{INT32_MAX, INT32_MAX, INT32_MIN, INT32_MIN};
+  for (int i = 0; i < n; ++i) {
+    minC = std::min(minC, px[i].col0);
+    minR = std::min(minR, px[i].row());
+    maxR = std::max(maxR, px[i].row());
+    j.rect = JobRect{std::min(j.rect.x0, px[i].x), std::min(j.rect.y0, px[i].y), std::max(j.rect.x1, px[i].x + 1), std::max(j.rect.y1, px[i].y + 1)};
+  }
+  const int boxX = minC & ~15, boxY = minR, steps = (n + 31) / 32;
+  j.job = GatherJob{steps, kJobCap << kJobKindShift, jobBoxField(boxX, boxY, boxVariantFor(k, 0, maxR + k - minR)), 0};
+  j.needRows = maxR + k;
+  j.words.assign(static_cast<size_t>(steps) * kCapStepBytes / 4, 0u);
+  for (int s = 0; s < steps; ++s) {
+    const CapPixel* step = px + 32 * s;
+    const int m = std::min(32, n - 32 * s);
+    int slot[32], laneOf[32], copyOf[32];
+    for (int i = 0; i < m; ++i) slot[i] = weightSlotOf(k, step[i].rowPhase & 1023);
+    dealLanes(k, copies, m, slot, laneOf, copyOf);
+    uint32_t* words = &j.words[static_cast<size_t>(s) * kCapStepBytes / 4];
+    for (int lane = m; lane < 32; ++lane) words[2 * lane] = kRecordSkip;
+    for (int i = 0; i < m; ++i) {
+      const int off = (step[i].row() - boxY) * pitch + (step[i].col0 - boxX);
+      words[2 * laneOf[i]] = static_cast<uint32_t>(off) | (slotField(k, step[i].rowPhase & 1023, copyOf[i]) << 17);
+      words[2 * laneOf[i] + 1] = static_cast<uint32_t>(step[i].x) | (static_cast<uint32_t>(step[i].y) << 16);
+    }
+  }
+  return j;
+}
+
+PixelJob borderJob(const HostPlan& h, const CapPixel* px, int n) {
+  PixelJob j;
+  j.job = GatherJob{n, kJobBorder << kJobKindShift, 0, 0};
+  j.needRows = 0;
+  j.rect = JobRect{INT32_MAX, INT32_MAX, INT32_MIN, INT32_MIN};
+  j.words.assign(static_cast<size_t>(n) * kBorderPixelBytes / 4, 0u);
+  for (int i = 0; i < n; ++i) {
+    j.words[4 * i] = static_cast<uint32_t>(px[i].col0);
+    j.words[4 * i + 1] = static_cast<uint32_t>(px[i].rowPhase);
+    j.words[4 * i + 2] = static_cast<uint32_t>(px[i].x) | (static_cast<uint32_t>(px[i].y) << 16);
+    j.needRows = std::max(j.needRows, px[i].row() >= 0 && px[i].row() + h.kernelSize <= h.inH ? px[i].row() + h.kernelSize : h.inH);
+    j.rect = JobRect{std::min(j.rect.x0, px[i].x), std::min(j.rect.y0, px[i].y), std::max(j.rect.x1, px[i].x + 1), std::max(j.rect.y1, px[i].y + 1)};
+  }
+  return j;
+}
+
+void coverPoleCaps(const HostPlan& h, const std::vector<TileClass>& cls, int tilesX, int tilesY, std::vector<PixelJob>& out) {
+  const int k = h.kernelSize, boxW = stageBoxW(k, 0), boxH = stageBoxH(k, 0);
+  std::vector<CapPixel> cap, border;
+  std::vector<size_t> tileBorderStart;
+  for (int ty = 0; ty < tilesY; ++ty)
+    for (int tx = 0; tx < tilesX; ++tx) {
+      if (cls[static_cast<size_t>(ty) * tilesX + tx].kind != kJobGeneral) continue;
+      tileBorderStart.push_back(border.size());
+      for (int y = ty * kFrameTileH; y < std::min(h.mapH, (ty + 1) * kFrameTileH); ++y)
+        for (int x = tx * kGatherTileW; x < std::min(h.mapW, (tx + 1) * kGatherTileW); ++x) {
+          const SamplePoint& sp = h.samples[static_cast<size_t>(y) * h.mapW + x];
+          const CapPixel p{x, y, sp.col0, sp.rowPhase};
+          const bool inside = p.col0 >= 0 && p.row() >= 0 && p.col0 + k <= h.inW && p.row() + k <= h.inH;
+          (inside ? cap : border).push_back(p);
+        }
+    }
+  if (cap.empty() && border.empty()) return;
+  if (h.mapW > 65536 || h.mapH > 65536) throw std::invalid_argument("gather plan: pole-cap records hold 16-bit output positions");
+  auto outputOrder = [](const CapPixel& a, const CapPixel& b) { return a.y != b.y ? a.y < b.y : a.x < b.x; };
+  std::sort(cap.begin(), cap.end(), [](const CapPixel& a, const CapPixel& b) {
+    return a.row() != b.row() ? a.row() < b.row() : (a.y != b.y ? a.y < b.y : a.x < b.x);
+  });
+  for (size_t b0 = 0; b0 < cap.size();) {
+    size_t b1 = b0;
+    while (b1 < cap.size() && cap[b1].row() + k - cap[b0].row() <= boxH) ++b1;
+    std::sort(cap.begin() + b0, cap.begin() + b1, [](const CapPixel& a, const CapPixel& b) {
+      return a.col0 != b.col0 ? a.col0 < b.col0 : (a.y != b.y ? a.y < b.y : a.x < b.x);
+    });
+    for (size_t c0 = b0; c0 < b1;) {
+      const int boxX = cap[c0].col0 & ~15;
+      size_t c1 = c0;
+      while (c1 < b1 && cap[c1].col0 + k - boxX <= boxW) ++c1;
+      std::sort(cap.begin() + c0, cap.begin() + c1, outputOrder);
+      const int n = static_cast<int>(c1 - c0), jobs = ((n + 31) / 32 + capJobMaxSteps(k) - 1) / capJobMaxSteps(k);
+      const int per = ((n + jobs - 1) / jobs + 31) / 32 * 32;
+      for (int i = 0; i < n; i += per) out.push_back(capJob(h, &cap[c0 + i], std::min(per, n - i)));
+      c0 = c1;
+    }
+    b0 = b1;
+  }
+  tileBorderStart.push_back(border.size());
+  for (size_t t = 0; t + 1 < tileBorderStart.size(); ++t)
+    for (size_t i = tileBorderStart[t]; i < tileBorderStart[t + 1]; i += borderJobMaxPixels(k))
+      out.push_back(borderJob(h, &border[i], static_cast<int>(std::min(tileBorderStart[t + 1] - i, static_cast<size_t>(borderJobMaxPixels(k))))));
+}
+
 }
 
 struct PassDealer {
@@ -414,21 +534,6 @@
   return wavefronts;
 }
 
-void spreadGeneralJobs(std::vector<GatherJob>& jobs) {
-  std::vector<GatherJob> general, staged;
-  for (const GatherJob& j : jobs)
-    (((j.outY >> kJobKindShift) & kJobKindMask) == kJobGeneral ? general : staged).push_back(j);
-  if (general.empty() || staged.empty()) return;
-  const size_t span = staged.size() / 2 + 1;
-  jobs.clear();
-  size_t g = 0;
-  for (size_t i = 0; i < staged.size(); ++i) {
-    while (g < general.size() && g * span / general.size() <= i) jobs.push_back(general[g++]);
-    jobs.push_back(staged[i]);
-  }
-  while (g < general.size()) jobs.push_back(general[g++]);
-}
-
 std::vector<uint8_t> buildWeightImage(int k, const int16_t* table) {
   const int copies = weightCopies(k);
   std::vector<uint8_t> img(static_cast<size_t>(weightImageBytes(k, copies)), 0);
@@ -471,52 +576,78 @@
             classifyTile(h, t * 32, ty * kFrameTileH, seamPossible, cls[static_cast<size_t>(ty) * tilesX + t]);
       }
   });
-  const int order[7] = {kJobGeneral, kJobSeam, kJobClass1, kJobShareStay, kJobShare, kJobClass0, kJobClass0};
+
+  for (int ty = 0; ty < tilesY; ++ty)
+    for (int tx = 0; tx < tilesX; ++tx) {
+      const TileClass& c = cls[static_cast<size_t>(ty) * tilesX + tx];
+      const int kind = c.kind;
+      if (kind < 0) continue;
+      for (int q = 0; q < (c.quads ? 4 : 1); ++q) {
+        GatherJob job{tx * 32, ty * kFrameTileH | (kind << kJobKindShift),
+                      kind == kJobGeneral ? 0 : jobBoxField(c.boxX, c.boxY, boxVariantFor(k, boxClassOf(kind), c.boxRows)), 0};
+        if (c.quads) {
+          job.outX |= q + 1;
+          job.boxXY = jobBoxField(c.quadBoxX[q], c.quadBoxY[q], boxVariantFor(k, 0, c.quadBoxRows[q]));
+        }
+        g.jobs.push_back(job);
+      }
+      switch (kind) {
+        case kJobGeneral: ++g.numGeneral; break;
+        case kJobSeam: ++g.numSeam; break;
+        case kJobShare: case kJobShareStay: ++g.numShare; break;
+        default: g.numStaged[kind] += c.quads ? 4 : 1; break;
+      }
+    }
+  std::stable_sort(g.jobs.begin(), g.jobs.end(), [](const GatherJob& a, const GatherJob& b) { return jobLaunchRank(a) < jobLaunchRank(b); });
   size_t offset = 0;
-  for (int step = 0; step < 7; ++step)
-    for (int ty = 0; ty < tilesY; ++ty)
-      for (int tx = 0; tx < tilesX; ++tx) {
-        const int kind = order[step];
-        const TileClass& c = cls[static_cast<size_t>(ty) * tilesX + tx];
-        if (c.kind != kind || (kind == kJobClass0 && c.quads != (step == 6))) continue;
-        for (int q = 0; q < (c.quads ? 4 : 1); ++q) {
-          GatherJob job{tx * 32, ty * kFrameTileH | (kind << kJobKindShift),
-                        kind == kJobGeneral ? 0 : jobBoxField(c.boxX, c.boxY, boxVariantFor(k, boxClassOf(kind), c.boxRows)), 0};
-          if (c.quads) {
-            job.outX |= q + 1;
-            job.boxXY = jobBoxField(c.quadBoxX[q], c.quadBoxY[q], boxVariantFor(k, 0, c.quadBoxRows[q]));
-          }
-          if (kind != kJobGeneral) {
-            job.recordOffset = static_cast<int>(offset / 16);
-            offset += boxClassOf(kind) == 2 ? shareJobRecordBytes(k) : tileJobRecordBytes(job.outX);
-          }
-          g.jobs.push_back(job);
-        }
-        switch (kind) {
-          case kJobGeneral: ++g.numGeneral; break;
-          case kJobSeam: ++g.numSeam; break;
-          case kJobShare: case kJobShareStay: ++g.numShare; break;
-          default: g.numStaged[kind] += c.quads ? 4 : 1; break;
-        }
-      }
+  for (GatherJob& job : g.jobs) {
+    const int kind = (job.outY >> kJobKindShift) & kJobKindMask;
+    if (kind == kJobGeneral) continue;
+    job.recordOffset = static_cast<int>(offset / 16);
+    offset += jobRecordBytes(k, kind, job.outX);
+  }
   g.compact.assign(offset / 4, 0u);
-  g.jobNeedRows.assign(g.jobs.size(), h.inH);
+  std::vector<int> needRows(g.jobs.size(), h.inH);
+  std::vector<JobRect> rects(g.jobs.size());
   parallelRanges(static_cast<int>(g.jobs.size()), 2048, [&](int begin, int end) {
     for (int i = begin; i < end; ++i) {
       const GatherJob& job = g.jobs[i];
-      {
-        int rect[4];
-        jobOutputRect(job, k, rect);
-        const Extent e = extentOf(h, rect[0], rect[1], std::min(rect[2], h.mapW), std::min(rect[3], h.mapH));
-        if (e.minR >= 0 && e.maxR + k <= h.inH) g.jobNeedRows[i] = e.maxR + k;
-      }
+      JobRect& r = rects[i];
+      r = tileRect(job, k);
+      r.x1 = std::min(r.x1, h.mapW);
+      r.y1 = std::min(r.y1, h.mapH);
       const int kind = (job.outY >> kJobKindShift) & kJobKindMask;
       if (kind == kJobGeneral) continue;
+      const Extent e = extentOf(h, r.x0, r.y0, r.x1, r.y1);
+      if (e.minR >= 0 && e.maxR + k <= h.inH) needRows[i] = e.maxR + k;
       uint32_t* out = g.compact.data() + static_cast<size_t>(job.recordOffset) * 4;
       if (boxClassOf(kind) == 2) writeShareRecords(h, job, out);
       else writeTileRecords(h, job, out);
     }
   });
-}
-
-}
+
+  std::vector<PixelJob> pixelJobs;
+  coverPoleCaps(h, cls, tilesX, tilesY, pixelJobs);
+  for (PixelJob& pj : pixelJobs) {
+    const int kind = (pj.job.outY >> kJobKindShift) & kJobKindMask;
+    pj.job.recordOffset = static_cast<int>(offset / 16);
+    offset += jobRecordBytes(k, kind, pj.job.outX);
+    g.capJobs.push_back(pj.job);
+    g.capRecords.insert(g.capRecords.end(), pj.words.begin(), pj.words.end());
+    ++(kind == kJobCap ? g.numCap : g.numBorder);
+  }
+
+  std::vector<int> launch;
+  for (size_t i = 0; i < g.jobs.size(); ++i)
+    if (((g.jobs[i].outY >> kJobKindShift) & kJobKindMask) != kJobGeneral) launch.push_back(static_cast<int>(i));
+  for (size_t i = 0; i < g.capJobs.size(); ++i) launch.push_back(-1 - static_cast<int>(i));
+  auto jobOf = [&](int i) -> const GatherJob& { return i >= 0 ? g.jobs[i] : g.capJobs[-1 - i]; };
+  std::stable_sort(launch.begin(), launch.end(), [&](int a, int b) { return jobLaunchRank(jobOf(a)) < jobLaunchRank(jobOf(b)); });
+  for (int i : launch) {
+    g.launchJobs.push_back(jobOf(i));
+    g.launchNeedRows.push_back(i >= 0 ? needRows[i] : pixelJobs[-1 - i].needRows);
+    g.launchRects.push_back(i >= 0 ? rects[i] : pixelJobs[-1 - i].rect);
+  }
+}
+
+}
diff --git a/transform360_b200/csrc/gather_plan.h b/transform360_b200/csrc/gather_plan.h
--- a/transform360_b200/csrc/gather_plan.h
+++ b/transform360_b200/csrc/gather_plan.h
@@ -8,29 +8,37 @@
 
 namespace t360 {
 
+struct JobRect {
+  int x0, y0, x1, y1;
+};
+
 struct GatherPlan {
   int tilesPerRow = 0, tileRows = 0, tileH = 0;
   std::vector<int2> records;
   std::vector<GatherJob> jobs;
   std::vector<uint32_t> compact;
-  std::vector<int> jobNeedRows;
-  int numStaged[2] = {}, numSeam = 0, numGeneral = 0, numShare = 0;
-  int totalStaged() const { return numSeam + numShare + numStaged[0] + numStaged[1]; }
+  std::vector<GatherJob> capJobs;
+  std::vector<uint32_t> capRecords;
+  std::vector<GatherJob> launchJobs;
+  std::vector<int> launchNeedRows;
+  std::vector<JobRect> launchRects;
+  int numStaged[2] = {}, numSeam = 0, numGeneral = 0, numShare = 0, numCap = 0, numBorder = 0;
+  int totalStaged() const { return numSeam + numShare + numStaged[0] + numStaged[1] + numCap; }
 };
 
 void buildGatherPlan(const HostPlan& h, bool stageTiles, GatherPlan& g);
 
-inline void jobOutputRect(const GatherJob& job, int k, int rect[4]) {
-  const int kind = (job.outY >> kJobKindShift) & kJobKindMask, quad = (job.outX & kJobQuadMask) - 1;
-  rect[0] = job.outX & ~kJobQuadMask;
-  rect[1] = job.outY & kJobRowMask;
-  if (quad >= 0) { rect[0] += 16 * (quad & 1); rect[1] += 16 * (quad >> 1); }
-  const bool share = kind == kJobShare || kind == kJobShareStay;
-  rect[2] = rect[0] + (quad >= 0 ? 16 : (share ? kShareW : kGatherTileW));
-  rect[3] = rect[1] + (quad >= 0 ? 16 : (share ? shareH(k) : kFrameTileH));
+inline int jobLaunchRank(const GatherJob& job) {
+  switch ((job.outY >> kJobKindShift) & kJobKindMask) {
+    case kJobBorder: case kJobGeneral: return 0;
+    case kJobSeam: return 1;
+    case kJobClass1: return 2;
+    case kJobCap: return 3;
+    case kJobShareStay: return 4;
+    case kJobShare: return 5;
+    default: return (job.outX & kJobQuadMask) ? 7 : 6;
+  }
 }
-
-void spreadGeneralJobs(std::vector<GatherJob>& jobs);
 
 
 int dealLanes(int k, int copies, int n, const int* slot, int* laneOf, int* copyOf);
diff --git a/transform360_b200/csrc/kernels.cuh b/transform360_b200/csrc/kernels.cuh
--- a/transform360_b200/csrc/kernels.cuh
+++ b/transform360_b200/csrc/kernels.cuh
@@ -29,7 +29,8 @@
 __host__ __device__ constexpr int jobBoxY(int boxXY) { return (int)((unsigned)boxXY >> 16); }
 __host__ __device__ constexpr int jobBoxVariant(int boxXY) { return boxXY & 15; }
 using StagedTile = GatherJob;
-constexpr int kJobClass0 = 0, kJobClass1 = 1, kJobGeneral = 2, kJobShareStay = 3, kJobShare = 4, kJobNop = 5, kJobExit = 6, kJobSeam = 7;
+constexpr int kJobClass0 = 0, kJobClass1 = 1, kJobGeneral = 2, kJobShareStay = 3, kJobShare = 4, kJobNop = 5, kJobExit = 6, kJobSeam = 7,
+              kJobCap = 8, kJobBorder = 9;
 constexpr int kJobQuadMask = 7;
 constexpr uint32_t kRecordSkip = 0x8000u;
 constexpr int kJobKindShift = 24, kJobRowMask = (1 << kJobKindShift) - 1;
@@ -94,18 +95,24 @@
 __host__ __device__ constexpr int stageRecordBytes(int k) {
   return 128 + (shareJobRecordBytes(k) > kTileJobRecordBytes ? shareJobRecordBytes(k) : kTileJobRecordBytes);
 }
+constexpr int kCapStepBytes = 32 * 8, kBorderPixelBytes = 16;
+__host__ __device__ constexpr int capJobMaxSteps(int k) { return (stageRecordBytes(k) - 128) / kCapStepBytes; }
+__host__ __device__ constexpr int borderJobMaxPixels(int k) { return (stageRecordBytes(k) - 128) / kBorderPixelBytes; }
+__host__ __device__ constexpr int jobRecordBytes(int k, int kind, int outXField) {
+  return kind == kJobShare || kind == kJobShareStay ? shareJobRecordBytes(k)
+         : kind == kJobCap                          ? outXField * kCapStepBytes
+         : kind == kJobBorder                       ? outXField * kBorderPixelBytes
+                                                    : tileJobRecordBytes(outXField);
+}
 constexpr int kRecordColumnShift = 27;
 
 constexpr int kMaxFramePlanes = 3;
 struct PlaneView {
   const uint8_t* src;
   uint8_t* dst;
-  const int2* samples;
   const uint4* records;
   int srcW, srcH, srcPitch;
   int dstW, dstH, dstPitch;
-  int tilesPerRow;
-  int reserved;
 };
 struct FrameGatherParams {
   PlaneView plane[kMaxFramePlanes];
diff --git a/transform360_b200/csrc/video_frame_transform.cpp b/transform360_b200/csrc/video_frame_transform.cpp
--- a/transform360_b200/csrc/video_frame_transform.cpp
+++ b/transform360_b200/csrc/video_frame_transform.cpp
@@ -75,8 +75,8 @@
   DeviceBuffer<GatherJob> gatherJobs;
   std::vector<GatherJob> hostJobs;
   std::vector<int> jobNeedRows;
-  int numJobs = 0, numStaged[2] = {}, numSeam = 0, numShare = 0, numFallback = 0;
-  int totalStaged() const { return numSeam + numShare + numStaged[0] + numStaged[1]; }
+  std::vector<t360::JobRect> jobRects;
+  int numJobs = 0, numStaged = 0, numBorder = 0;
   struct BlurSet {
     DeviceBuffer<StripJob> stripJobs[t360::kStripMaxHy];
     int numStripJobs[t360::kStripMaxHy] = {};
@@ -326,7 +326,7 @@
   }
 
   bool pipelineEligible(const DevicePlan& plan, int inW, int inH, int outW, int outH) const {
-    return plan.totalStaged() > 0 && !plan.transparent && !plan.lowPass && inW == plan.inW && inH == plan.inH &&
+    return plan.numJobs > 0 && !plan.transparent && !plan.lowPass && inW == plan.inW && inH == plan.inH &&
            outW == plan.mapW && outH == plan.mapH && static_cast<long long>(inW) * inH >= pipelineMinBytes_ && inH >= 64;
   }
 
@@ -353,17 +353,16 @@
     for (size_t i = 0; i < plan.hostJobs.size(); ++i) {
       const int c = waveOf(plan.jobNeedRows[i]);
       byWave[c].push_back(plan.hostJobs[i]);
-      int rect[4];
-      t360::jobOutputRect(plan.hostJobs[i], plan.kernelSize, rect);
-      for (int band = rect[1] / 32; band <= (std::min(rect[3], plan.mapH) - 1) / 32; ++band) {
-        int& slot = complete[static_cast<size_t>(band) * blocks + rect[0] / blockW];
-        slot = std::max(slot, c);
-      }
+      const t360::JobRect& r = plan.jobRects[i];
+      for (int band = r.y0 / 32; band <= (r.y1 - 1) / 32; ++band)
+        for (int b = r.x0 / blockW; b <= (r.x1 - 1) / blockW; ++b) {
+          int& slot = complete[static_cast<size_t>(band) * blocks + b];
+          slot = std::max(slot, c);
+        }
     }
     std::vector<GatherJob> all;
     w.waveStart.assign(chunks + 1, 0);
     for (int c = 0; c < chunks; ++c) {
-      t360::spreadGeneralJobs(byWave[c]);
       w.waveStart[c] = static_cast<int>(all.size());
       all.insert(all.end(), byWave[c].begin(), byWave[c].end());
     }
@@ -712,7 +711,7 @@
     std::lock_guard<std::mutex> lock(mu_);
     auto it = plans_.find(planIndex);
     if (it == plans_.end()) return false;
-    counts[0] = it->second.totalStaged(); counts[1] = it->second.numFallback;
+    counts[0] = it->second.numStaged; counts[1] = it->second.numBorder;
     counts[2] = it->second.blur.numStripJobs[0] + it->second.blur.numStripJobs[1] + it->second.blur.numStripJobs[2];
     counts[3] = it->second.blur.numTileJobs + it->second.blur.numDirectJobs;
     return true;
@@ -834,23 +833,23 @@
       d.tilesPerRow = g.tilesPerRow;
       d.samples.reserve(g.records.size());
       CU(cudaMemcpy(d.samples.ptr, g.records.data(), g.records.size() * sizeof(int2), cudaMemcpyHostToDevice));
-      d.numFallback = g.numGeneral;
-      d.numSeam = g.numSeam;
-      d.numShare = g.numShare;
-      for (int c = 0; c < 2; ++c) d.numStaged[c] = g.numStaged[c];
-      d.numJobs = static_cast<int>(g.jobs.size());
-      if (!g.jobs.empty()) {
-        std::vector<GatherJob> launchOrder = g.jobs;
-        t360::spreadGeneralJobs(launchOrder);
-        d.gatherJobs.reserve(launchOrder.size());
-        CU(cudaMemcpy(d.gatherJobs.ptr, launchOrder.data(), launchOrder.size() * sizeof(GatherJob), cudaMemcpyHostToDevice));
-      }
-      if (!g.compact.empty()) {
-        d.records.reserve(g.compact.size());
-        CU(cudaMemcpy(d.records.ptr, g.compact.data(), g.compact.size() * sizeof(uint32_t), cudaMemcpyHostToDevice));
-      }
-      d.hostJobs = std::move(g.jobs);
-      d.jobNeedRows = std::move(g.jobNeedRows);
+      d.numStaged = g.totalStaged();
+      d.numBorder = g.numBorder;
+      d.numJobs = static_cast<int>(g.launchJobs.size());
+      if (!g.launchJobs.empty()) {
+        d.gatherJobs.reserve(g.launchJobs.size());
+        CU(cudaMemcpy(d.gatherJobs.ptr, g.launchJobs.data(), g.launchJobs.size() * sizeof(GatherJob), cudaMemcpyHostToDevice));
+      }
+      if (!g.compact.empty() || !g.capRecords.empty()) {
+        d.records.reserve(g.compact.size() + g.capRecords.size());
+        if (!g.compact.empty())
+          CU(cudaMemcpy(d.records.ptr, g.compact.data(), g.compact.size() * sizeof(uint32_t), cudaMemcpyHostToDevice));
+        if (!g.capRecords.empty())
+          CU(cudaMemcpy(d.records.ptr + g.compact.size(), g.capRecords.data(), g.capRecords.size() * sizeof(uint32_t), cudaMemcpyHostToDevice));
+      }
+      d.hostJobs = std::move(g.launchJobs);
+      d.jobNeedRows = std::move(g.launchNeedRows);
+      d.jobRects = std::move(g.launchRects);
     }
     d.lowPass = ctx_.enable_low_pass_filter != 0;
     if (d.lowPass) {
@@ -1114,9 +1113,8 @@
       src = lane.blurred.ptr;
       srcPitch = bp;
     }
-    w.view = t360::PlaneView{src, dOut, plan.samples.ptr, reinterpret_cast<const uint4*>(plan.records.ptr), inW, inH, srcPitch,
-                             outW, outH, outPitch, plan.tilesPerRow, 0};
-    w.staged = plan.totalStaged() > 0 && !plan.transparent && inW == plan.inW && inH == plan.inH;
+    w.view = t360::PlaneView{src, dOut, reinterpret_cast<const uint4*>(plan.records.ptr), inW, inH, srcPitch, outW, outH, outPitch};
+    w.staged = plan.numJobs > 0 && !plan.transparent && inW == plan.inW && inH == plan.inH;
     if (w.staged) w.staged = planeMaps(lane, src, inW, inH, srcPitch, plan.kernelSize, w.maps);
     return true;
   }
@@ -1140,7 +1138,7 @@
       CU(t360::launchGatherFrame(fp, jobs, w.maps, numSMs_, s));
     } else {
       const t360::PlaneView& v = w.view;
-      t360::GatherParams gp{v.src, v.srcW, v.srcH, v.srcPitch, v.dst, v.dstW, v.dstH, v.dstPitch, v.samples, v.tilesPerRow,
+      t360::GatherParams gp{v.src, v.srcW, v.srcH, v.srcPitch, v.dst, v.dstW, v.dstH, v.dstPitch, plan.samples.ptr, plan.tilesPerRow,
                             weights_[plan.kernelSize].ptr, plan.kernelSize, plan.transparent ? 1 : 0};
       CU(t360::launchGather(gp, numSMs_, s));
     }
@@ -1210,17 +1208,13 @@
     std::unique_lock<std::mutex> listLock(frameJobsMu_);
     if (f.generation != planGeneration_ || f.numPlanes != numPlanes) {
       std::vector<GatherJob> merged;
-      const int order[7] = {t360::kJobGeneral, t360::kJobSeam, t360::kJobClass1, t360::kJobShareStay, t360::kJobShare, t360::kJobClass0, t360::kJobClass0};
-      for (int step = 0; step < 7; ++step)
-        for (int p = 0; p < numPlanes; ++p)
-          for (GatherJob t : work[p].plan->hostJobs) {
-            const int kind = order[step];
-            if (((t.outY >> t360::kJobKindShift) & t360::kJobKindMask) != kind) continue;
-            if (kind == t360::kJobClass0 && ((t.outX & t360::kJobQuadMask) != 0) != (step == 6)) continue;
-            t.outY |= p << t360::kJobPlaneShift;
-            merged.push_back(t);
-          }
-      t360::spreadGeneralJobs(merged);
+      for (int p = 0; p < numPlanes; ++p)
+        for (GatherJob t : work[p].plan->hostJobs) {
+          t.outY |= p << t360::kJobPlaneShift;
+          merged.push_back(t);
+        }
+      std::stable_sort(merged.begin(), merged.end(),
+                       [](const GatherJob& a, const GatherJob& b) { return t360::jobLaunchRank(a) < t360::jobLaunchRank(b); });
       CU(cudaDeviceSynchronize());
       f.tiles.reserve(merged.size());
       CU(cudaMemcpy(f.tiles.ptr, merged.data(), merged.size() * sizeof(GatherJob), cudaMemcpyHostToDevice));
@@ -1380,6 +1374,18 @@
   if (compact) *compact = g.compact.empty() ? nullptr : g.compact.data();
   return 1;
 }
+T360_API int T360B200_hostPlanPoleCaps(T360HostPlan* plan, int info[4], const int32_t** capJobs, const uint32_t** capRecords,
+                                       const int32_t** launchJobs) {
+  int gatherInfo[10];
+  if (!plan || !info || !T360B200_hostPlanGather(plan, gatherInfo, nullptr, nullptr, nullptr)) return 0;
+  const t360::GatherPlan& g = plan->gather;
+  info[0] = g.numCap; info[1] = g.numBorder; info[2] = static_cast<int>(g.capRecords.size());
+  info[3] = static_cast<int>(g.launchJobs.size());
+  if (capJobs) *capJobs = g.capJobs.empty() ? nullptr : reinterpret_cast<const int32_t*>(g.capJobs.data());
+  if (capRecords) *capRecords = g.capRecords.empty() ? nullptr : g.capRecords.data();
+  if (launchJobs) *launchJobs = g.launchJobs.empty() ? nullptr : reinterpret_cast<const int32_t*>(g.launchJobs.data());
+  return 1;
+}
 T360_API int T360B200_hostPlanSegment(const T360HostPlan* plan, int i, int rect[4], int numTaps[2], const float** kx,
                                       const float** ky) {
   if (!plan || i < 0 || i >= static_cast<int>(plan->plan.segments.size())) return 0;
diff --git a/transform360_b200/handler.py b/transform360_b200/handler.py
--- a/transform360_b200/handler.py
+++ b/transform360_b200/handler.py
@@ -87,6 +87,8 @@
     L.T360B200_hostPlanSegment.argtypes = [vp, ci, C.POINTER(ci), C.POINTER(ci), C.POINTER(vp), C.POINTER(vp)]
     L.T360B200_hostPlanGather.restype = ci
     L.T360B200_hostPlanGather.argtypes = [vp, C.POINTER(ci), C.POINTER(vp), C.POINTER(vp), C.POINTER(vp)]
+    L.T360B200_hostPlanPoleCaps.restype = ci
+    L.T360B200_hostPlanPoleCaps.argtypes = [vp, C.POINTER(ci), C.POINTER(vp), C.POINTER(vp), C.POINTER(vp)]
     L.T360B200_weightImage.restype = ci
     L.T360B200_weightImage.argtypes = [ci, C.POINTER(vp)]
     L.T360B200_remapTable.restype = ci
@@ -123,7 +125,7 @@
     "VideoFrameTransform_new", "VideoFrameTransform_delete", "VideoFrameTransform_generateMapForPlane",
     "VideoFrameTransform_transformFramePlane", "T360B200_hostPlanCreate", "T360B200_hostPlanDestroy",
     "T360B200_hostPlanInfo", "T360B200_hostPlanMap", "T360B200_hostPlanSamples", "T360B200_hostPlanSegment",
-    "T360B200_hostPlanGather", "T360B200_weightImage", "T360B200_dealLanes",
+    "T360B200_hostPlanGather", "T360B200_hostPlanPoleCaps", "T360B200_weightImage", "T360B200_dealLanes",
     "T360B200_remapTable", "T360B200_transformFramePlaneAsync", "T360B200_transformFrameAsync",
     "T360B200_lowPassPlaneAsync",
     "T360B200_setPinHostPlanes", "T360B200_debugTrace", "T360B200_debugTraceRead", "T360B200_synchronize", "T360B200_stream", "T360B200_kernelLaunchCount", "T360B200_planDeviceBytes",
@@ -274,6 +276,16 @@
         return dict(tiles_per_row=tpr, tile_rows=trows, tile_h=th, jobs=j, records=records, compact=compact,
                     counts=dict(class0=info[4], class1=info[5], seam=info[6], general=info[7], share=info[8]))
 
+    def pole_caps(self):
+        info = (C.c_int * 4)()
+        jobs, recs, launch = C.c_void_p(), C.c_void_p(), C.c_void_p()
+        if not self._lib.T360B200_hostPlanPoleCaps(self._h, info, C.byref(jobs), C.byref(recs), C.byref(launch)):
+            raise ValueError("T360B200_hostPlanPoleCaps failed")
+        n, m = info[0] + info[1], info[3]
+        as_jobs = lambda p, k: np.frombuffer((C.c_int32 * (k * 4)).from_address(p.value), np.int32).reshape(k, 4).copy() if k and p.value else np.zeros((0, 4), np.int32)
+        records = np.frombuffer((C.c_uint32 * info[2]).from_address(recs.value), np.uint32).copy() if info[2] and recs.value else np.zeros(0, np.uint32)
+        return dict(counts=dict(cap=info[0], border=info[1]), jobs=as_jobs(jobs, n), records=records, launch=as_jobs(launch, m))
+
     def segments(self):
         out = []
         rect, nk = (C.c_int * 4)(), (C.c_int * 2)()
```

Result: faster. 691,000, median of 6 (+10.2%).
